# opensensor/thingino-accel

Hardware: AMD Instinct MI355X
Metric: images/sec yolov5s_int8 640x640 batch256 (higher is better)
Workload: dtype int8

## Files before the change

thingino-accel_amd/csrc/hip/conv_i8.hip:

```cpp
#include "conv_i8_common.hpp"

#ifndef I8M_ABL
#define I8M_ABL 0
#endif
template <int BPX, int BN, int STAGES, int KS = 1, int NW = 4>
__global__ __launch_bounds__(NW * 64) void conv_i8_mfma(const mhip_conv_i8_t p, const long total_pix, const int k64,
                                                         const int8_t *__restrict__ zeros, const unsigned noc,
                                                         const unsigned nblk, const int lg_inc, const unsigned kw_magic,
                                                         const fastdiv_t dhw, const fastdiv_t dow, const int bufmode,
                                                         const unsigned in_bytes) {
    ANAT_BEGIN();
    const bool POW2 = lg_inc >= 0;
    const bool masked = p.kh * p.kw <= 32;
    constexpr int SLICE = (BPX + BN) * BK;
    constexpr int STAGE = KS * SLICE;
    constexpr int NWN = BN == 128 ? 2 : 1;
    constexpr int NWM = NW / NWN;
    constexpr int WPX = BPX / NWM / 16;
    constexpr int WOC = BN / NWN / 16;
    constexpr int XROWS = BPX / NW;
    constexpr int XI = XROWS / 16;
    constexpr int LW = (BN / 16 + NW - 1) / NW;
    constexpr int L = XI + LW;
    static_assert(XI >= 1 && XROWS % 16 == 0, "every wave fetches whole 16-row pieces of the pixel tile");
// ... 240 lines not shown
    const int taps = p.kh * p.kw;
    const int nst = k128 / 128;
    auto issue = [&](int st, int buf) {
        int8_t *sb = lds + buf * STAGE;
        const int utap = (st * 128) >> lg_inc, urc = (st * 128) & ((1 << lg_inc) - 1);
        const int uky = (int)(((unsigned)utap * kw_magic) >> 16), ukx = utap - uky * p.kw;
        const int ukoff = (uky * p.in_w + ukx) * p.in_c + urc;
        const bool uvalid = utap < taps;
#pragma unroll
        for (int j = 0; j < XI; j++) {
            const bool ok = uvalid & (((tapmask[j] >> utap) & 1u) != 0u);
            blds16(xrs, ok ? xvoff[j] + ukoff : -1, 0, sb + (wv * XI + j) * 1024);
        }
#pragma unroll
        for (int j = 0; j < WI; j++) blds16(wrs, wvoff[j], st * 128, sb + BPX * 128 + (wv * WI + j) * 1024);
    };

    issue(0, 0);
    const int frow = lane & 15, fchunk = lane >> 4;
    for (int st = 0; st < nst; st++) {
        wait_vmcnt<0>();
        __builtin_amdgcn_s_barrier();
        asm volatile("" ::: "memory");
        const int8_t *xs = lds + (st & 1) * STAGE, *ws = xs + BPX * 128;
        v4i xb[2][WPX], wa[2][WOC];
#pragma unroll
        for (int h = 0; h < 2; h++) {
#pragma unroll
            for (int t = 0; t < WPX; t++) xb[h][t] = *(const v4i *)(xs + lds_off128(pxw + t * 16 + frow, h * 4 + fchunk));
#pragma unroll
            for (int q = 0; q < WOC; q++) wa[h][q] = *(const v4i *)(ws + lds_off128(ocw + q * 16 + frow, h * 4 + fchunk));
        }
        if (st + 1 < nst) issue(st + 1, (st + 1) & 1);
#pragma unroll
        for (int h = 0; h < 2; h++)
#pragma unroll
            for (int q = 0; q < WOC; q++)
#pragma unroll
                for (int t = 0; t < WPX; t++) acc[q][t] = __builtin_amdgcn_mfma_i32_16x16x64_i8(wa[h][q], xb[h][t], acc[q][t], 0, 0, 0);
    }
    __syncthreads();
    epilogue<BPX, BN, WPX, WOC, true>(p, acc, lds, slut, rowoff, oc0, pxw, ocw, hw);
}

template <int A, int B>
__device__ __forceinline__ void wait_vmcnt_at_most(int n) {
    constexpr int HI = A > B ? A : B, LO = A > B ? B : A;
    if (n >= A + B) wait_vmcnt<A + B>();
    else if (n >= HI) wait_vmcnt<HI>();
    else if (n >= LO) wait_vmcnt<LO>();
    else wait_vmcnt<0>();
}

struct conv_out_side_t {
    int8_t *out;
    size_t out_stride;
    const int8_t *w;
    const int32_t *bias;
    const uint8_t *lut, *lut2;
    int out_c, relu, out_pix_stride, out_ch_off;
    float cs;
    unsigned out_bytes;
};
template <int BPX, int BN, int STAGES, bool HAS_LUT, bool SEG = false, bool PAIR = false>
__global__ __launch_bounds__(NTHREADS) void conv_i8_persist(const mhip_conv_i8_t pin, const unsigned total_pix, const int k64,
                                                            const int8_t *__restrict__ zeros, const unsigned noc,
                                                            const unsigned npt, const unsigned ngrp, const int lg_inc,
                                                            const unsigned kw_magic, const fastdiv_t dhw, const fastdiv_t dow,
                                                            const unsigned out_bytes_first, const conv_out_side_t alt,
                                                            const unsigned noc0, const int bufmode, const unsigned in_bytes,
                                                            const int wres) {
    ANAT_BEGIN();
    const int STAGE = wres ? BPX * BK : (BPX + BN) * BK;
    constexpr int NWN = BN == 128 ? 2 : 1;
    constexpr int NWM = 4 / NWN;
    constexpr int WPX = BPX / NWM / 16;
    constexpr int WOC = BN / NWN / 16;
    constexpr int XI = BPX / 64;
    constexpr int LW = BN >= 128 ? 2 : 1;
    constexpr int L = XI + LW;
    constexpr int NST = WPX;
    extern __shared__ __attribute__((aligned(16))) int8_t dynlds[];
    uint8_t *slut = (uint8_t *)dynlds;
    int8_t *lds = dynlds + LUTB;
    lds_base_must_be_zero(dynlds);

    const int tid = threadIdx.x, lane = tid & 63;
    const int wv = __builtin_amdgcn_readfirstlane(tid >> 6);
    const unsigned id = xcd_remap(blockIdx.x, noc * ngrp);
    const unsigned grp = id / noc;
    unsigned ot = id - grp * noc;
    mhip_conv_i8_t p = pin;
    unsigned out_bytes = out_bytes_first;
    if (PAIR && ot >= noc0) {
        ot -= noc0;
        p.lut2 = alt.lut2;
        p.out = alt.out; p.out_stride = alt.out_stride; p.w = alt.w; p.bias = alt.bias; p.lut = alt.lut;
        p.out_c = alt.out_c; p.relu = alt.relu; p.out_pix_stride = alt.out_pix_stride; p.out_ch_off = alt.out_ch_off;
        p.cs = alt.cs;
        out_bytes = alt.out_bytes;
    }
    const int oc0 = (int)ot * BN;
    const unsigned t0 = (unsigned)(((unsigned long long)grp * npt) / ngrp);
    const unsigned t1 = (unsigned)(((unsigned long long)(grp + 1) * npt) / ngrp);
    if (t0 >= t1) return;
    const unsigned hw = (unsigned)(p.out_h * p.out_w);
    const int wm = wv % NWM, wn = wv / NWM;
    const int pxw = wm * (WPX * 16), ocw = wn * (WOC * 16);

    auto packed_row16 = [](int c) { return ((c >> 2) & 1) * 16 + (c >> 3) * 4 + (c & 3); };
    v4i bias[WOC];
#pragma unroll
    for (int s = 0; s < WOC; s++)
        bias[s] = p.bias ? *(const v4i *)(p.bias + (BN == 16 ? packed_row16((lane >> 4) * 4) : oc0 + ocw + s * 16 + (lane >> 4) * 4)) : (v4i){0, 0, 0, 0};
    if (HAS_LUT) {
        if (p.lut2) { if (tid < 128) ((uint32_t *)slut)[tid] = ((const uint32_t *)p.lut2)[tid]; }
        else if (tid < 64) ((uint32_t *)slut)[tid] = ((const uint32_t *)p.lut)[tid];
        __syncthreads();
    }
    const __amdgpu_buffer_rsrc_t orsrc = __builtin_amdgcn_make_buffer_rsrc(p.out, 0, (int)out_bytes, 0x00020000);

    const int schunk = (lane & 3) ^ (((lane >> 4) & 1) << 1);
    const int8_t *xwin[XI];
    unsigned tapmask[XI];
    unsigned rowf[SEG ? XI : 1], rowrem[SEG ? XI : 1];
    unsigned rowrem_up[SEG ? XI : 1];
    int xvoff[XI];
    auto setup_rows = [&](unsigned tile) {
#pragma unroll
        for (int j = 0; j < XI; j++) {
            const unsigned pix = tile * BPX + wv * (BPX / 4) + j * 16 + (lane >> 2);
            const bool valid = pix < total_pix;
            const unsigned f = valid ? fdiv(pix, dhw) : 0u;
            const unsigned rem = valid ? pix - f * hw : 0u;
            if (SEG) {
                rowf[j] = f;
                rowrem[j] = rem;
                const unsigned oy = fdiv(rem, dow), ox = rem - oy * (unsigned)p.out_w;
                rowrem_up[j] = (oy >> 1) * ((unsigned)p.out_w >> 1) + (ox >> 1);
                tapmask[j] = valid ? 1u : 0u;
                continue;
            }
            const int oy = (int)fdiv(rem, dow), ox = (int)(rem - (unsigned)oy * (unsigned)p.out_w);
            const int iy0 = oy * p.stride_h - p.pad_top, ix0 = ox * p.stride_w - p.pad_left;
            xwin[j] = p.in + (size_t)f * p.in_stride + ((long)iy0 * p.in_w + ix0) * p.in_c;
            xvoff[j] = (int)(f * (unsigned)p.in_stride) + (iy0 * p.in_w + ix0) * p.in_c + schunk * 16;
            const int kx_lo = ix0 < 0 ? -ix0 : 0, kx_hi = p.in_w - ix0 < p.kw ? p.in_w - ix0 : p.kw;
            const unsigned colbits = kx_hi > kx_lo ? ((kx_hi >= 32 ? ~0u : (1u << kx_hi) - 1u) & ~((1u << kx_lo) - 1u)) : 0u;
            unsigned m = 0;
            for (int r = 0; r < p.kh; r++) {
                const int iy = iy0 + r;
                if (iy >= 0 && iy < p.in_h) m |= colbits << (r * p.kw);
            }
            tapmask[j] = valid ? m : 0u;
        }
    };
    const int8_t *wsrc[LW];
    int wq[LW], wvoff[LW];
#pragma unroll
    for (int j = 0; j < LW; j++) {
        wq[j] = BN >= 64 ? wv * LW + j : (BN == 16 ? 0 : (wv & 1));
        const int wrow = BN == 16 ? packed_row16(lane >> 2) : oc0 + wq[j] * 16 + (lane >> 2);
        wsrc[j] = p.w + (size_t)wrow * k64 + schunk * 16;
        wvoff[j] = wrow * k64 + schunk * 16;
    }
    const __amdgpu_buffer_rsrc_t xrs = __builtin_amdgcn_make_buffer_rsrc((void *)p.in, 0, (int)in_bytes, 0x00020000);
    const __amdgpu_buffer_rsrc_t wrs = __builtin_amdgcn_make_buffer_rsrc((void *)p.w, 0, p.oc_pad * k64, 0x00020000);
    const int taps = p.kh * p.kw;
    const int nks = k64 / BK;

    auto issue = [&](int ks, int stage) {
        int8_t *sb = lds + stage * STAGE;
        const unsigned pos = (unsigned)(ks * BK + schunk * 16);
        if (SEG) {
            auto owner = [&](int c) { return (c >= p.seg_c0[1]) + (c >= p.seg_c0[2]) + (c >= p.seg_c0[3]); };
            const int sa = owner(ks * BK), sb2 = owner(ks * BK + 32);
            const bool hi = schunk >= 2;
            const int8_t *base = hi ? p.seg_in[sb2] : p.seg_in[sa];
            const unsigned fstride = (unsigned)(hi ? p.seg_stride[sb2] : p.seg_stride[sa]);
            const unsigned segc = (unsigned)(hi ? p.seg_c[sb2] : p.seg_c[sa]);
            const unsigned coff = pos - (unsigned)(hi ? p.seg_c0[sb2] : p.seg_c0[sa]);
            const bool up = ((p.seg_up >> (hi ? sb2 : sa)) & 1) != 0;
            const bool kvalid = (int)pos < p.in_c;
#pragma unroll
            for (int j = 0; j < XI; j++) {
                const bool ok = kvalid & (tapmask[j] != 0u);
                const int8_t *src = base + (size_t)rowf[j] * fstride + (size_t)(up ? rowrem_up[j] : rowrem[j]) * segc + coff;
                glds16(ok ? src : zeros, sb + (wv * (BPX / 4) + j * 16) * BK);
            }
        } else if (bufmode) {
            const int utap = (ks * BK) >> lg_inc, urc = (ks * BK) & ((1 << lg_inc) - 1);
            const int uky = (int)(((unsigned)utap * kw_magic) >> 16), ukx = utap - uky * p.kw;
            const int ukoff = (uky * p.in_w + ukx) * p.in_c + urc;
            const bool uvalid = utap < taps;
#pragma unroll
            for (int j = 0; j < XI; j++) {
                const bool ok = uvalid & (((tapmask[j] >> utap) & 1u) != 0u);
                blds16(xrs, ok ? xvoff[j] + ukoff : -1, 0, sb + (wv * (BPX / 4) + j * 16) * BK);
            }
            if (!wres)
#pragma unroll
                for (int j = 0; j < LW; j++) blds16(wrs, wvoff[j], ks * BK, sb + BPX * BK + wq[j] * 16 * BK);
            return;
        } else {
            const unsigned tap = pos >> lg_inc;
            const int rc = (int)(pos & ((1u << lg_inc) - 1u));
            const int ky = (int)((tap * kw_magic) >> 16);
            const int kx = (int)tap - ky * p.kw;
            const bool kvalid = (int)tap < taps;
            const long koff = ((long)ky * p.in_w + kx) * p.in_c + rc;
#pragma unroll
            for (int j = 0; j < XI; j++) {
                const bool ok = kvalid & ((tapmask[j] >> tap) & 1u);
                glds16(ok ? xwin[j] + koff : zeros, sb + (wv * (BPX / 4) + j * 16) * BK);
            }
        }
        if (!wres)
#pragma unroll
            for (int j = 0; j < LW; j++) glds16(wsrc[j] + ks * BK, sb + BPX * BK + wq[j] * 16 * BK);
    };

    int8_t *const wres_base = lds + STAGES * STAGE;
    if (wres)
        for (int ks = 0; ks < nks; ks++)
#pragma unroll
            for (int j = 0; j < LW; j++) glds16(wsrc[j] + ks * BK, wres_base + (ks * BN + wq[j] * 16) * BK);
    unsigned itile = t0;
    int iks = 0;
    int younger[STAGES - 1];
    setup_rows(t0);
    int nstage = 0;
#pragma unroll
    for (int s = 0; s < STAGES - 1; s++) {
        int n = 0;
        if (itile < t1) {
            issue(iks, nstage);
            n = wres ? XI : L;
            if (++iks == nks) {
                iks = 0;
                if (++itile < t1) setup_rows(itile);
            }
        }
#pragma unroll
        for (int i = 0; i < s; i++) younger[i] += n;
        younger[s] = 0;
        nstage++;
    }
    nstage = STAGES - 1;

    const int frow = lane & 15, fchunk = lane >> 4;
    const int chan = ocw + (lane >> 4) * (4 * WOC);
    const int pstride = p.out_pix_stride ? p.out_pix_stride : p.out_c;
    const int lo = p.relu ? 0 : -128;
    const uint8_t *lut128 = slut + 128;
    const bool ragged = (p.out_c % (WOC * 4)) != 0;
    int stage = 0;
    ANAT_NOW(1);
    for (unsigned tile = t0; tile < t1; tile++) {
        v4i acc[WOC][WPX];
        for (int ks = 0; ks < nks; ks++) {
            wait_vmcnt_at_most<(STAGES - 2) * L, NST>(younger[0]);
            __builtin_amdgcn_s_barrier();
            asm volatile("" ::: "memory");
            const int8_t *xs = lds + stage * STAGE, *ws = wres ? wres_base + ks * (BN * BK) : xs + BPX * BK;
            v4i xb[WPX], wa[WOC];
#pragma unroll
            for (int t = 0; t < WPX; t++) xb[t] = *(const v4i *)(xs + lds_off(pxw + t * 16 + frow, fchunk));
#pragma unroll
            for (int s = 0; s < WOC; s++) wa[s] = *(const v4i *)(ws + lds_off(ocw + s * 16 + frow, fchunk));
            int n = 0;
            if (itile < t1) {
                issue(iks, nstage);
                n = wres ? XI : L;
                if (++iks == nks) {
                    iks = 0;
                    if (++itile < t1) setup_rows(itile);
                }
            }
#pragma unroll
            for (int i = 0; i + 1 < STAGES - 1; i++) younger[i] = younger[i + 1] + n;
            younger[STAGES - 2] = 0;
            if (ks == 0) {
#pragma unroll
                for (int s = 0; s < WOC; s++)
#pragma unroll
                    for (int t = 0; t < WPX; t++) acc[s][t] = __builtin_amdgcn_mfma_i32_16x16x64_i8(wa[s], xb[t], bias[s], 0, 0, 0);
            } else {
#pragma unroll
                for (int s = 0; s < WOC; s++)
#pragma unroll
                    for (int t = 0; t < WPX; t++) acc[s][t] = __builtin_amdgcn_mfma_i32_16x16x64_i8(wa[s], xb[t], acc[s][t], 0, 0, 0);
            }
            stage = stage + 1 == STAGES ? 0 : stage + 1;
            nstage = nstage + 1 == STAGES ? 0 : nstage + 1;
        }
#ifdef ANATOMY
        if (tile + 1 == t1) ANAT_NOW(2);
#endif
#pragma unroll
        for (int t = 0; t < WPX; t++) {
            const unsigned pix = tile * BPX + pxw + t * 16 + (lane & 15);
            const unsigned f = fdiv(pix, dhw), rem = pix - f * hw;
            const unsigned off = f * (unsigned)p.out_stride + rem * (unsigned)pstride + (unsigned)(p.out_ch_off + oc0 + chan);
            const int nvalid = p.out_c - (oc0 + chan);
            const bool ok = pix < total_pix && nvalid >= WOC * 4;
            uint32_t pk[WOC];
            int a[WOC * 4];
#pragma unroll
            for (int s = 0; s < WOC; s++)
#pragma unroll
                for (int r = 0; r < 4; r++) a[s * 4 + r] = acc[s][t][r];
            if (HAS_LUT && p.lut2) requant_pack<WOC * 4, HAS_LUT, true, true, false, true>(a, p.cs, lo, lut128, pk);
            else requant_pack<WOC * 4, HAS_LUT, true, true>(a, p.cs, lo, lut128, pk);
            const int voff = ok ? (int)off : -1;
            if (WOC == 4)
                __builtin_amdgcn_raw_buffer_store_b128((v4i){(int)pk[0], (int)pk[1], (int)pk[2], (int)pk[3]}, orsrc, voff, 0, 0);
            else if (WOC == 2)
                __builtin_amdgcn_raw_buffer_store_b64((v2i){(int)pk[0], (int)pk[WOC > 1 ? 1 : 0]}, orsrc, voff, 0, 0);
            else
                __builtin_amdgcn_raw_buffer_store_b32((int)pk[0], orsrc, voff, 0, 0);
            if (ragged) {
                const bool part = pix < total_pix && nvalid > 0 && nvalid < WOC * 4;
                const int nv = part ? nvalid : 0;
                const int o4 = nv & 8, o2 = nv & 12, o1 = nv & 14;
                const uint32_t w4 = o4 ? pk[(WOC * 4 > 8) ? 2 : 0] : pk[0];
                const int i2 = o2 >> 2, i1 = o1 >> 2;
                uint32_t w2 = pk[0], w1 = pk[0];
#pragma unroll
                for (int q = 1; q < WOC; q++) {
                    w2 = i2 == q ? pk[q] : w2;
                    w1 = i1 == q ? pk[q] : w1;
                }
                w1 >>= (o1 & 2) * 8;
                if (WOC == 4)
                    __builtin_amdgcn_raw_buffer_store_b64((v2i){(int)pk[0], (int)pk[1]}, orsrc, (nv & 8) ? (int)off : -1, 0, 0);
                __builtin_amdgcn_raw_buffer_store_b32((int)w4, orsrc, (nv & 4) ? (int)off + o4 : -1, 0, 0);
                __builtin_amdgcn_raw_buffer_store_b16((short)w2, orsrc, (nv & 2) ? (int)off + o2 : -1, 0, 0);
                __builtin_amdgcn_raw_buffer_store_b8((char)w1, orsrc, (nv & 1) ? (int)off + o1 : -1, 0, 0);
            }
        }
#pragma unroll
        for (int i = 0; i < STAGES - 1; i++) younger[i] += ragged ? NST * (WOC == 4 ? 5 : 4) : NST;
    }
    ANAT_END(p);
}
ANAT_SETTER(mhip_anatomy_set_i8)
__device__ __forceinline__ bool mhip_small_c_dev(int in_c, int kw, int out_c) { return in_c <= 4 && kw <= 8 && out_c <= 64; }
template <int BN>
__global__ __launch_bounds__(NTHREADS) void conv_i8_generic(const mhip_conv_i8_t p, const long total_pix, const int k64,
                                                            const fastdiv_t dhw) {
    constexpr int STAGE = (BP + BN) * BK;
    constexpr int WPX = 2, WOC = BN / 16;
    constexpr int TILE_BYTES = BP * (BN + OPAD);
    constexpr int LDS_BYTES = (2 * STAGE > TILE_BYTES ? 2 * STAGE : TILE_BYTES) + 256;
    __shared__ __attribute__((aligned(16))) int8_t lds[LDS_BYTES];
    __shared__ long rowoff[BP];
    uint8_t *slut = (uint8_t *)lds + LDS_BYTES - 256;

    const int tid = threadIdx.x, lane = tid & 63, wv = tid >> 6;
    const long pix0 = (long)blockIdx.x * BP;
    const int oc0 = blockIdx.y * BN;
    const int hw = p.out_h * p.out_w;
    if (p.lut && tid < 64) ((uint32_t *)slut)[tid] = ((const uint32_t *)p.lut)[tid];
    fill_rowoff<BP>(p, rowoff, [=](int row) { long q = pix0 + row; return q < total_pix ? q : -1L; }, (unsigned)hw, dhw);

    const int cc = tid & 3;
    const int8_t *xbase[2];
    int iy0[2], ix0[2];
    bool rvalid[2];
#pragma unroll
    for (int j = 0; j < 2; j++) {
        long pix = pix0 + (tid >> 2) + j * 64;
        rvalid[j] = pix < total_pix;
        long f = rvalid[j] ? pix / hw : 0;
        int rem = rvalid[j] ? (int)(pix - f * hw) : 0;
        int oy = rem / p.out_w, ox = rem - oy * p.out_w;
        iy0[j] = oy * p.stride_h - p.pad_top;
        ix0[j] = ox * p.stride_w - p.pad_left;
        xbase[j] = p.in + (size_t)f * p.in_stride;
    }
    int ky = 0, rc = cc * 16;
    while (rc >= p.row_pad) { rc -= p.row_pad; ky++; }
    const int ceff = mhip_small_c_dev(p.in_c, p.kw, p.out_c) ? 4 : p.in_c;
    const int nks = k64 / BK;
    constexpr int WLOADS = (BN * 4 + NTHREADS - 1) / NTHREADS;
    v4i xreg[2], wreg[WLOADS];

    auto load_global = [&](int ks) {
#pragma unroll
        for (int j = 0; j < 2; j++) {
            v4i v = {0, 0, 0, 0};
            const int iy = iy0[j] + ky;
            if (rvalid[j] && ky < p.kh && iy >= 0 && iy < p.in_h) {
                const int8_t *rowp = xbase[j] + ((long)iy * p.in_w + ix0[j]) * p.in_c;
                int8_t b[16];
// ... 63 lines not shown
    return g * G + s * 16 + q * 4 + r;
}

extern "C" int mhip_conv_i8_is_safe(float cs) {
    return cs == cs && cs < 0.99f && cs > -0.99f;
}

extern "C" int mhip_conv_i8_lut2_ok(float cs) {
    if (!mhip_conv_i8_is_safe(cs)) return 0;
    const float a = cs < 0 ? -cs : cs;
    if (!(a >= 1e-6f)) return 0;
    const float quirk = 0.49999997f;
    const double a0 = (double)quirk / (double)a;
    for (int d = -3; d <= 3; d++) {
        const double c = (double)(long long)(a0 + 0.5) + d;
        if (c < 1.0 || c > 2147483647.0) continue;
        volatile float prod = (float)(int)c * a;
        if (prod == quirk) return 0;
    }
    return 1;
}

extern "C" int mhip_conv_i8_small_c(int in_c, int kw, int out_c) { return in_c <= 4 && kw <= 8 && out_c <= 64; }

extern "C" void mhip_conv_i8_pack_geom(int in_c, int kw, int out_c, int *row_pad, int *oc_pad, int *c_eff) {
    const int small = mhip_conv_i8_small_c(in_c, kw, out_c);
    if (row_pad) *row_pad = small ? 32 : (kw * in_c + 15) & ~15;
    if (oc_pad) *oc_pad = (out_c + 31) & ~31;
    if (c_eff) *c_eff = small ? 4 : in_c;
}

static tune_t g_tune;
static int env_int(const char *name, int dflt) {
    const char *e = getenv(name);
    return e ? atoi(e) : dflt;
}
const tune_t &conv_i8_tune_state() {
    if (!g_tune.init) {
        g_tune.persist = env_int("MARS_HIP_PERSIST", 1);
        g_tune.persist_stages = env_int("MARS_HIP_PSTAGES", 2);
        g_tune.persist_maxk = env_int("MARS_HIP_PERSIST_MAXK", 8);
        g_tune.persist_slots = env_int("MARS_HIP_PSLOTS", 0);
        g_tune.stages = env_int("MARS_HIP_STAGES", 0);
        g_tune.bpx = env_int("MARS_HIP_BPX", 0);
        g_tune.variant = env_int("MARS_HIP_VARIANT", 0);
        g_tune.bufmode = env_int("MARS_HIP_BUFMODE", 1);
        g_tune.wres = env_int("MARS_HIP_WRES", 3);
        g_tune.rgb_direct = env_int("MARS_HIP_RGB_DIRECT", 1);
        g_tune.small_batch = env_int("MARS_HIP_SMALL_BATCH", 1);
        g_tune.rows = env_int("MARS_HIP_ROWS", 1);
        g_tune.few_wgs = env_int("MARS_HIP_FEW_WGS", 256);
        g_tune.patch_ring = env_int("MARS_HIP_PATCH_RING", 0);
        g_tune.patch_lds_kb = env_int("MARS_HIP_PATCH_LDS_KB", 80);
        g_tune.init = 1;
    }
    return g_tune;
}
static inline const tune_t &tune() { return conv_i8_tune_state(); }
static int tune_access(const char *key, int value, int *get) {
    (void)conv_i8_tune_state();
    struct { const char *k; int *v; } tab[] = {{"persist", &g_tune.persist}, {"persist_stages", &g_tune.persist_stages},
                                               {"persist_maxk", &g_tune.persist_maxk}, {"persist_slots", &g_tune.persist_slots}, {"wres", &g_tune.wres}, {"rgb_direct", &g_tune.rgb_direct}, {"small_batch", &g_tune.small_batch},
                                               {"rows", &g_tune.rows}, {"few_wgs", &g_tune.few_wgs}, {"patch_ring", &g_tune.patch_ring}, {"patch_lds_kb", &g_tune.patch_lds_kb}, {"stages", &g_tune.stages}, {"bpx", &g_tune.bpx}, {"variant", &g_tune.variant}, {"bufmode", &g_tune.bufmode}};
    for (auto &e : tab)
        if (key && !strcmp(key, e.k)) {
            if (get) *get = *e.v;
            else *e.v = value;
            return 0;
        }
    return -1;
}
extern "C" int mhip_conv_i8_tune(const char *key, int value) { return tune_access(key, value, nullptr); }
extern "C" int mhip_conv_i8_tune_get(const char *key, int *value) { return value ? tune_access(key, 0, value) : -1; }

static int buf_mode(const mhip_conv_i8_t *p, int k64) {
    if (!tune().bufmode) return 0;
    return p->in_c >= 64 && (p->in_c & (p->in_c - 1)) == 0 && p->kh * p->kw <= 32 && (long)p->kh * p->kw * (p->kw - 1) < 65536 &&
           in_extent_bytes(p) <= 0x7fffffffL && (long)p->oc_pad * k64 <= 0x7fffffffL;
}

template <int BPX, int BN, int STAGES, int KS = 1, int NW = 4>
static int launch_mfma(const mhip_conv_i8_t *p, long total_pix, int k64) {
    const unsigned npt = (unsigned)((total_pix + BPX - 1) / BPX), noc = (unsigned)(p->oc_pad / BN);
    const unsigned nblk = npt * noc;
    const int nks = k64 / BK, nst = nks / KS, used = nst < STAGES ? nst : STAGES;
    if (KS > 1 && (nks % KS) != 0) return -1;
    size_t ring = (size_t)used * KS * (BPX + BN) * BK, tile = (size_t)BPX * (BN + OPAD);
    const size_t lds = BPX * 8 + LUTB + (ring > tile ? ring : tile);
    if (lds > 64 * 1024) {
        static bool attr = false;
        if (!attr && hipFuncSetAttribute((const void *)conv_i8_mfma<BPX, BN, STAGES, KS, NW>, hipFuncAttributeMaxDynamicSharedMemorySize,
                                         (int)(BPX * 8 + LUTB + (size_t)STAGES * KS * (BPX + BN) * BK)) != hipSuccess)
            return mhip_check(hipErrorUnknown, "conv_i8_mfma LDS attribute");
        attr = true;
    }
    int lg = -1;
    if ((p->in_c & (p->in_c - 1)) == 0 && (long)p->kh * p->kw * (p->kw - 1) < 65536) {
        lg = 0;
        while ((1 << lg) < p->in_c) lg++;
    }
    const unsigned magic = ((65536u + (unsigned)p->kw - 1u) / (unsigned)p->kw);
    hipLaunchKernelGGL((conv_i8_mfma<BPX, BN, STAGES, KS, NW>), dim3(nblk), dim3(NW * 64), lds, mhip_stream_native(), *p, total_pix,
                       k64, (const int8_t *)mhip_zero_page(), noc, nblk, lg, magic,
                       make_fastdiv((unsigned)(p->out_h * p->out_w)), make_fastdiv((unsigned)p->out_w),
                       lg >= 0 ? buf_mode(p, k64) : 0, (unsigned)in_extent_bytes(p));
    return mhip_check(hipGetLastError(), "conv_i8_mfma launch");
}


template <int BPX, int BN>
static size_t wres_lds(int k64) { return LUTB + 2 * (size_t)BPX * BK + (size_t)(k64 / BK) * BN * BK; }

template <int BPX, int BN, int STAGES, bool HAS_LUT, bool SEG = false, bool PAIR = false>
static int launch_persist_t(const mhip_conv_i8_t *p, long total_pix, int k64, int lg, unsigned magic,
                            const mhip_conv_i8_t *second = nullptr, int wres = 0) {
    if (BN == 16 && (p->out_c > 16 || p->oc_pad != 32 || (PAIR && (second->out_c > 16 || second->oc_pad != 32)))) return -1;
    const unsigned noc0 = BN == 16 ? 1u : (unsigned)(p->oc_pad / BN);
    const unsigned npt = (unsigned)((total_pix + BPX - 1) / BPX), noc = noc0 + (PAIR ? (BN == 16 ? 1u : (unsigned)(second->oc_pad / BN)) : 0u);
    conv_out_side_t alt;
    memset(&alt, 0, sizeof(alt));
    if (PAIR) {
        alt.out = second->out; alt.out_stride = second->out_stride; alt.w = second->w; alt.bias = second->bias;
        alt.lut = second->lut; alt.lut2 = second->lut2; alt.out_c = second->out_c; alt.relu = second->relu; alt.out_pix_stride = second->out_pix_stride;
        alt.out_ch_off = second->out_ch_off; alt.cs = second->cs;
    }
    if (PAIR) alt.out_bytes = (unsigned)persist_out_bytes(second);
    if (wres && STAGES != 2) return -1;
    const size_t lds = wres ? wres_lds<BPX, BN>(k64) : LUTB + (size_t)STAGES * (BPX + BN) * BK;
    if (wres) {
        static bool attr = false;
        if (!attr && hipFuncSetAttribute((const void *)conv_i8_persist<BPX, BN, STAGES, HAS_LUT, SEG, PAIR>,
                                         hipFuncAttributeMaxDynamicSharedMemorySize, 80 * 1024) != hipSuccess)
            return mhip_check(hipErrorUnknown, "conv_i8_persist LDS attribute");
        attr = true;
        int occ = 0, dev = 0;
        hipDeviceProp_t prop;
        if (hipOccupancyMaxActiveBlocksPerMultiprocessor(&occ, conv_i8_persist<BPX, BN, STAGES, HAS_LUT, SEG, PAIR>, NTHREADS, lds) != hipSuccess ||
            hipGetDevice(&dev) != hipSuccess || hipGetDeviceProperties(&prop, dev) != hipSuccess)
            return mhip_check(hipErrorUnknown, "conv_i8_persist occupancy query");
        unsigned g = (unsigned)((occ > 0 ? occ : 1) * prop.multiProcessorCount) / noc;
        if (tune().persist_slots > 0) g = (unsigned)tune().persist_slots / noc;
        if (g < 1) g = 1;
        if (g > npt) g = npt;
        hipLaunchKernelGGL((conv_i8_persist<BPX, BN, STAGES, HAS_LUT, SEG, PAIR>), dim3(noc * g), dim3(NTHREADS), lds,
                           mhip_stream_native(), *p, (unsigned)total_pix, k64, (const int8_t *)mhip_zero_page(), noc, npt, g, lg,
                           magic, make_fastdiv((unsigned)(p->out_h * p->out_w)), make_fastdiv((unsigned)p->out_w),
                           (unsigned)persist_out_bytes(p), alt, noc0, SEG ? 0 : buf_mode(p, k64), (unsigned)in_extent_bytes(p), 1);
        return mhip_check(hipGetLastError(), "conv_i8_persist (resident weights) launch");
    }
    static int slots = 0;
    if (!slots) {
        int occ = 0, dev = 0;
        hipDeviceProp_t prop;
        if (hipOccupancyMaxActiveBlocksPerMultiprocessor(&occ, conv_i8_persist<BPX, BN, STAGES, HAS_LUT, SEG, PAIR>, NTHREADS, lds) != hipSuccess ||
            hipGetDevice(&dev) != hipSuccess || hipGetDeviceProperties(&prop, dev) != hipSuccess)
            return mhip_check(hipErrorUnknown, "conv_i8_persist occupancy query");
        slots = (occ > 0 ? occ : 1) * prop.multiProcessorCount;
    }
    unsigned ngrp = (unsigned)(tune().persist_slots > 0 ? tune().persist_slots : 4 * slots) / noc;
    if (ngrp < 1) ngrp = 1;
    if (ngrp > npt) ngrp = npt;
    hipLaunchKernelGGL((conv_i8_persist<BPX, BN, STAGES, HAS_LUT, SEG, PAIR>), dim3(noc * ngrp), dim3(NTHREADS), lds,
                       mhip_stream_native(), *p, (unsigned)total_pix, k64, (const int8_t *)mhip_zero_page(), noc, npt, ngrp, lg,
                       magic, make_fastdiv((unsigned)(p->out_h * p->out_w)), make_fastdiv((unsigned)p->out_w),
                       (unsigned)persist_out_bytes(p), alt, noc0, SEG ? 0 : buf_mode(p, k64), (unsigned)in_extent_bytes(p), 0);
    return mhip_check(hipGetLastError(), "conv_i8_persist launch");
}

#define NVARIANTS 20
struct variant_t {
    int persist, bpx, stages, patch, ks2, w8, wres, r128, rows;
};
static int variant_code(const variant_t &v) {
    if (v.rows) return 20;
    if (v.r128) return 17 + v.r128;
    if (v.wres) return v.bpx == 256 ? 15 : 14;
    if (v.w8) return 13;
    if (v.ks2) return 12;
    if (v.patch) return v.patch == 16 ? 10 : (v.patch == 8 ? 9 : 11);
    return 1 + (v.persist ? 1 : 0) + (v.bpx == 256 ? 2 : 0) + (v.stages == 3 ? 4 : 0);
}
static variant_t variant_of(int code) {
    if (code == 20) return variant_t{0, 0, 0, 0, 0, 0, 0, 0, 1};
    if (code == 18 || code == 19) return variant_t{0, 0, 0, 0, 0, 0, 0, code - 17, 0};
    if (code == 14 || code == 15) return variant_t{1, code == 15 ? 256 : 128, 2, 0, 0, 0, 1, 0, 0};
    if (code == 13) return variant_t{0, 256, 3, 0, 0, 1, 0, 0, 0};
    if (code == 12) return variant_t{0, 128, 2, 0, 1, 0, 0, 0, 0};
    if (code >= 9 && code <= 11) return variant_t{0, 0, 0, code == 10 ? 16 : (code == 9 ? 8 : 4), 0, 0, 0, 0, 0};
    if (code > 8 || code == 6 || code == 8) return variant_t{-1, 0, 0, 0, 0, 0, 0, 0, 0};
    const int c = code - 1;
    return variant_t{c & 1, (c & 2) ? 256 : 128, (c & 4) ? 3 : 2, 0, 0, 0, 0, 0, 0};
}

static bool r128_ok(const mhip_conv_i8_t *p) {
    const int C = p->in_c;
    return C >= 128 && (C & (C - 1)) == 0 && p->oc_pad % 128 == 0 && p->kh * p->kw <= 32 && (long)p->kh * p->kw * (p->kw - 1) < 65536 &&
           p->row_pad == p->kw * C && p->nseg <= 1 && in_extent_bytes(p) <= 0x7fffffffL && (long)p->oc_pad * p->kh * p->row_pad <= 0x7fffffffL;
}
template <int BPX, int BN, int NW>
static int launch_r128_t(const mhip_conv_i8_t *p, long total_pix) {
    const int k128 = p->kh * p->row_pad;
    const unsigned npt = (unsigned)((total_pix + BPX - 1) / BPX), noc = (unsigned)(p->oc_pad / BN);
    size_t ring = 2 * (size_t)(BPX + BN) * 128, tile = (size_t)BPX * (BN + OPAD);
    const size_t lds = BPX * 8 + LUTB + (ring > tile ? ring : tile);
    static bool attr = false;
    if (!attr && hipFuncSetAttribute((const void *)conv_i8_r128<BPX, BN, NW>, hipFuncAttributeMaxDynamicSharedMemorySize, (int)lds) != hipSuccess)
        return mhip_check(hipErrorUnknown, "conv_i8_r128 LDS attribute");
    attr = true;
    int lg = 0;
    while ((1 << lg) < p->in_c) lg++;
    const unsigned magic = ((65536u + (unsigned)p->kw - 1u) / (unsigned)p->kw);
    hipLaunchKernelGGL((conv_i8_r128<BPX, BN, NW>), dim3(npt * noc), dim3(NW * 64), lds, mhip_stream_native(), *p, total_pix, k128, noc,
                       npt * noc, lg, magic, make_fastdiv((unsigned)(p->out_h * p->out_w)), make_fastdiv((unsigned)p->out_w),
                       (unsigned)in_extent_bytes(p));
    return mhip_check(hipGetLastError(), "conv_i8_r128 launch");
}
static int launch_r128(const mhip_conv_i8_t *p, long total_pix, int form) {
    if (!r128_ok(p)) return -1;
// ... 129 lines not shown
        if (b16) return launch_variant_t<256, 16>(p, total_pix, k64, v);
        return launch_variant_t<256, 32>(p, total_pix, k64, v);
    }
    if (bn == 128) return launch_variant_t<128, 128>(p, total_pix, k64, v);
    if (bn == 64) return launch_variant_t<128, 64>(p, total_pix, k64, v);
    if (b16) return launch_variant_t<128, 16>(p, total_pix, k64, v);
    return launch_variant_t<128, 32>(p, total_pix, k64, v);
}

template <int BPX, int BN>
static int launch_pair_t(const mhip_conv_i8_t *a, const mhip_conv_i8_t *b, long total_pix, int k64, int lg, unsigned magic,
                         int wres) {
    if (a->nseg > 1) return -2;
    return launch_persist_t<BPX, BN, 2, true, false, true>(a, total_pix, k64, lg, magic, b, wres);
}
extern "C" int mhip_conv_i8_pair(const mhip_conv_i8_t *a, const mhip_conv_i8_t *b) {
    if (!a || !b || !tune().persist || tune().variant) return -2;
    if (a->in != b->in || a->in_stride != b->in_stride || a->frames != b->frames || a->in_h != b->in_h || a->in_w != b->in_w ||
        a->in_c != b->in_c || a->out_h != b->out_h || a->out_w != b->out_w || a->kh != b->kh || a->kw != b->kw ||
        a->stride_h != b->stride_h || a->stride_w != b->stride_w || a->pad_top != b->pad_top || a->pad_left != b->pad_left ||
        a->row_pad != b->row_pad || a->nseg != b->nseg || a->seg_up != b->seg_up || !a->lut || !b->lut || a->add || b->add ||
        a->out_nchw || b->out_nchw)
        return -2;
    for (int i = 0; i < a->nseg; i++)
        if (a->seg_in[i] != b->seg_in[i] || a->seg_c[i] != b->seg_c[i] || a->seg_stride[i] != b->seg_stride[i]) return -2;
    if ((a->in_c % 16) != 0 || mhip_conv_i8_small_c(a->in_c, a->kw, a->out_c) || mhip_conv_i8_small_c(b->in_c, b->kw, b->out_c))
        return -2;
    if (a->nseg > 1 && (!seg_valid(a) || !seg_valid(b))) return -2;
    if (!persist_eligible(a) || !persist_eligible(b)) return -2;
    const int bn = a->oc_pad % 128 == 0 ? 128 : (a->oc_pad % 64 == 0 ? 64 : 32);
    const int bnb = b->oc_pad % 128 == 0 ? 128 : (b->oc_pad % 64 == 0 ? 64 : 32);
    if (bn != bnb || !mhip_zero_page()) return -2;
    const long total_pix = (long)a->frames * a->out_h * a->out_w;
    const int k64 = (a->kh * a->row_pad + BK - 1) / BK * BK, nks = k64 / BK;
    if (total_pix <= 0 || total_pix > 0x7fffffffL) return -2;
    int lg = 0;
    while ((1 << lg) < a->in_c) lg++;
    const unsigned magic = ((65536u + (unsigned)a->kw - 1u) / (unsigned)a->kw);
    const variant_t dv = default_variant(a, nks);
    const int bpx = dv.bpx ? dv.bpx : 128, wres = dv.persist && dv.wres && (tune().wres & 2);
    const bool b16 = bn16_ok(a) && bn16_ok(b);
    if (bpx == 256) {
        if (bn == 128) return launch_pair_t<256, 128>(a, b, total_pix, k64, lg, magic, wres);
        if (bn == 64) return launch_pair_t<256, 64>(a, b, total_pix, k64, lg, magic, wres);
        if (b16) return launch_pair_t<256, 16>(a, b, total_pix, k64, lg, magic, wres);
        return launch_pair_t<256, 32>(a, b, total_pix, k64, lg, magic, wres);
    }
    if (bn == 128) return launch_pair_t<128, 128>(a, b, total_pix, k64, lg, magic, wres);
    if (bn == 64) return launch_pair_t<128, 64>(a, b, total_pix, k64, lg, magic, wres);
    if (b16) return launch_pair_t<128, 16>(a, b, total_pix, k64, lg, magic, wres);
    return launch_pair_t<128, 32>(a, b, total_pix, k64, lg, magic, wres);
}

extern "C" int mhip_conv_i8_seg_ok(const mhip_conv_i8_t *p) {
    return p && (p->in_c % 16) == 0 && !mhip_conv_i8_small_c(p->in_c, p->kw, p->out_c) && seg_valid(p) && persist_eligible(p);
}

extern "C" int mhip_conv_i8_variants(const mhip_conv_i8_t *p, int *codes, int max) {
    if (!p || (p->in_c % 16) != 0 || mhip_conv_i8_small_c(p->in_c, p->kw, p->out_c)) return 0;
    const int k64 = (p->kh * p->row_pad + BK - 1) / BK * BK, nks = k64 / BK;
    int n = 0;
    if (p->pre_w) {
        const int first = conv_i8_pre_tile_rows(p);
        for (int th : {first, 16, 8, 4})
            if (th && n < max && conv_i8_patch_ok(p, th, nullptr)) {
                const int code = th == 16 ? 10 : (th == 8 ? 9 : 11);
                bool seen = false;
                for (int i = 0; i < n; i++) seen |= codes[i] == code;
                if (!seen) codes[n++] = code;
            }
        return n;
    }
    if (p->post_w) {
        for (int th : {16, 8, 4})
            if (n < max && conv_i8_patch_ok(p, th, nullptr)) codes[n++] = th == 16 ? 10 : (th == 8 ? 9 : 11);
        return n;
    }
    if (p->split_w) {
        for (int th : {16, 8, 4})
            if (n < max && conv_i8_patch_ok(p, th, nullptr)) codes[n++] = th == 16 ? 10 : (th == 8 ? 9 : 11);
        return n;
    }
    if (p->nseg > 1) {
        const int bn = p->oc_pad % 128 == 0 ? 128 : (p->oc_pad % 64 == 0 ? 64 : 32);
        const variant_t dv = default_variant(p, nks);
        const int dflt = dv.persist && dv.wres ? (dv.bpx == 256 ? 15 : 14) : (dv.bpx == 256 ? 4 : 2);
        if (n < max) codes[n++] = dflt;
        if (n < max && dflt != 2) codes[n++] = 2;
        if (n < max && dflt != 4) codes[n++] = 4;
        if (n < max && dflt != 14 && LUTB + 2 * (size_t)128 * BK + (size_t)nks * bn * BK <= 80 * 1024) codes[n++] = 14;
        if (n < max && dflt != 15 && LUTB + 2 * (size_t)256 * BK + (size_t)nks * bn * BK <= 80 * 1024) codes[n++] = 15;
        return n;
    }
    const int dflt = variant_code(default_variant(p, nks));
    if (n < max) codes[n++] = dflt;
    for (int code = 1; code <= NVARIANTS; code++) {
        const variant_t v = variant_of(code);
        if (code == dflt) continue;
        if (v.patch && !conv_i8_patch_ok(p, v.patch, nullptr)) continue;
        if (v.persist && !persist_eligible(p)) continue;
        if (v.ks2 && ((nks & 1) || nks < 4 || p->oc_pad % 64 != 0)) continue;
        if (v.w8 && (p->oc_pad % 128 != 0 || nks < 3)) continue;
        if (v.persist < 0) continue;
        if (v.r128 && !r128_ok(p)) continue;
        if (v.rows && !conv_i8_rows_ok(p)) continue;
        if (v.wres) {
// ... 123 lines not shown
```

thingino-accel_amd/csrc/hip/conv_i8_common.hpp:

```cpp
#pragma once
#include <hip/hip_runtime.h>
#include <stdint.h>
#include <stdlib.h>
#include <string.h>
#include <type_traits>

#include "../mhip.h"

extern "C" hipStream_t mhip_stream_native(void);
extern "C" int mhip_check(hipError_t e, const char *what);
extern "C" const void *mhip_zero_page(void);

typedef int v4i __attribute__((ext_vector_type(4)));
typedef int v2i __attribute__((ext_vector_type(2)));

#ifdef ANATOMY
struct anat_rec_t {
    unsigned key, wg, hwid, xcc;
    unsigned long long t[4];
};
static __device__ anat_rec_t *g_anat_buf;
static __device__ unsigned g_anat_cap;
#define ANAT_SETTER(NAME)                                                                                                    \
    extern "C" int NAME(void *buf, unsigned cap) {                                                                          \
// ... 64 lines not shown
    asm("v_med3_i32 %0, %1, %2, %3" : "=v"(m) : "v"(r), "v"(lo), "v"(hi));
    return m;
}
template <int NV>
__device__ __forceinline__ void wait_lds_values(int (&v)[NV]) {
    static_assert(NV == 4 || NV == 8 || NV == 16, "values per lane");
    if constexpr (NV == 16)
        asm volatile("s_waitcnt lgkmcnt(0)"
                     : "+v"(v[0]), "+v"(v[1]), "+v"(v[2]), "+v"(v[3]), "+v"(v[4]), "+v"(v[5]), "+v"(v[6]), "+v"(v[7]), "+v"(v[8]), "+v"(v[9]),
                       "+v"(v[10]), "+v"(v[11]), "+v"(v[12]), "+v"(v[13]), "+v"(v[14]), "+v"(v[15]));
    else if constexpr (NV == 8)
        asm volatile("s_waitcnt lgkmcnt(0)" : "+v"(v[0]), "+v"(v[1]), "+v"(v[2]), "+v"(v[3]), "+v"(v[4]), "+v"(v[5]), "+v"(v[6]), "+v"(v[7]));
    else
        asm volatile("s_waitcnt lgkmcnt(0)" : "+v"(v[0]), "+v"(v[1]), "+v"(v[2]), "+v"(v[3]));
}

__device__ __forceinline__ uint32_t pack4(int q0, int q1, int q2, int q3) {
    const uint32_t a = __builtin_amdgcn_perm((uint32_t)q1, (uint32_t)q0, 0x0c0c0400u);
    const uint32_t b = __builtin_amdgcn_perm((uint32_t)q3, (uint32_t)q2, 0x0c0c0400u);
    return (b << 16) | a;
}
__device__ __forceinline__ void lut4_at0(int q0, int q1, int q2, int q3, int &v0, int &v1, int &v2, int &v3) {
    asm volatile("ds_read_i8 %0, %4 offset:128\n\tds_read_i8 %1, %5 offset:128\n\t"
                 "ds_read_i8 %2, %6 offset:128\n\tds_read_i8 %3, %7 offset:128"
                 : "=&v"(v0), "=&v"(v1), "=&v"(v2), "=&v"(v3)
                 : "v"(q0), "v"(q1), "v"(q2), "v"(q3)
                 : "memory");
}
__device__ __forceinline__ void lds_base_must_be_zero(const void *dynamic_lds) {
    __builtin_amdgcn_s_setprio(3);
    unsigned a = (unsigned)(size_t)(const __attribute__((address_space(3))) void *)dynamic_lds;
    asm volatile("" : "+s"(a));
    if (a != 0u) __builtin_trap();
}
struct add_args_t {
    float s_conv, s_other, inv;
};
__device__ __forceinline__ int add_one(int v, uint32_t xword, int k, const add_args_t &g, int lo8, int hi8) {
    const int x = __builtin_amdgcn_sbfe((int)xword, 8 * k, 8);
    const float y = (float)v * g.s_conv + (float)x * g.s_other;
    const float t = y * g.inv;
    const int r = (int)(t + 0.5f);
    int m;
    asm("v_med3_i32 %0, %1, %2, %3" : "=v"(m) : "v"(r), "v"(lo8), "v"(hi8));
    return m;
}
__device__ __forceinline__ void lut4_fast(int q0, int q1, int q2, int q3, int &v0, int &v1, int &v2, int &v3) {
    asm volatile("ds_read_i8 %0, %4 offset:256\n\tds_read_i8 %1, %5 offset:256\n\t"
                 "ds_read_i8 %2, %6 offset:256\n\tds_read_i8 %3, %7 offset:256"
                 : "=&v"(v0), "=&v"(v1), "=&v"(v2), "=&v"(v3)
                 : "v"(q0), "v"(q1), "v"(q2), "v"(q3)
                 : "memory");
}
template <int NV>
__device__ __forceinline__ void requant_pack_pre(const int (&a)[NV], float cs, uint32_t (&pk)[NV / 4]) {
    const float cs2 = cs * 2.0f;
    const int klo = -256, khi = 255;
    int q[NV], v[NV];
#pragma unroll
    for (int i = 0; i < NV; i++) {
        const int k = (int)((float)a[i] * cs2);
        asm("v_med3_i32 %0, %1, %2, %3" : "=v"(q[i]) : "v"(k), "v"(klo), "v"(khi));
    }
#pragma unroll
    for (int g = 0; g < NV / 4; g++)
        asm volatile("ds_read_i8 %0, %4 offset:768\n\tds_read_i8 %1, %5 offset:768\n\t"
                     "ds_read_i8 %2, %6 offset:768\n\tds_read_i8 %3, %7 offset:768"
                     : "=&v"(v[4 * g]), "=&v"(v[4 * g + 1]), "=&v"(v[4 * g + 2]), "=&v"(v[4 * g + 3])
                     : "v"(q[4 * g]), "v"(q[4 * g + 1]), "v"(q[4 * g + 2]), "v"(q[4 * g + 3])
                     : "memory");
    wait_lds_values<NV>(v);
#pragma unroll
    for (int g = 0; g < NV / 4; g++) pk[g] = pack4(v[4 * g], v[4 * g + 1], v[4 * g + 2], v[4 * g + 3]);
}
__device__ __forceinline__ void requant_pack_two(const int (&a)[16], float cs0, float cs1, uint32_t (&pk)[4]) {
    const float c0 = cs0 * 2.0f, c1 = cs1 * 2.0f;
    const int klo = -256, khi = 255;
    int q[16], v[16];
#pragma unroll
    for (int i = 0; i < 16; i++) {
        const int k = (int)((float)a[i] * (i < 8 ? c0 : c1));
        asm("v_med3_i32 %0, %1, %2, %3" : "=v"(q[i]) : "v"(k), "v"(klo), "v"(khi));
    }
#pragma unroll
    for (int g = 0; g < 2; g++)
        asm volatile("ds_read_i8 %0, %4 offset:768\n\tds_read_i8 %1, %5 offset:768\n\t"
                     "ds_read_i8 %2, %6 offset:768\n\tds_read_i8 %3, %7 offset:768"
                     : "=&v"(v[4 * g]), "=&v"(v[4 * g + 1]), "=&v"(v[4 * g + 2]), "=&v"(v[4 * g + 3])
                     : "v"(q[4 * g]), "v"(q[4 * g + 1]), "v"(q[4 * g + 2]), "v"(q[4 * g + 3])
                     : "memory");
#pragma unroll
    for (int g = 2; g < 4; g++)
        asm volatile("ds_read_i8 %0, %4 offset:1280\n\tds_read_i8 %1, %5 offset:1280\n\t"
                     "ds_read_i8 %2, %6 offset:1280\n\tds_read_i8 %3, %7 offset:1280"
                     : "=&v"(v[4 * g]), "=&v"(v[4 * g + 1]), "=&v"(v[4 * g + 2]), "=&v"(v[4 * g + 3])
                     : "v"(q[4 * g]), "v"(q[4 * g + 1]), "v"(q[4 * g + 2]), "v"(q[4 * g + 3])
                     : "memory");
    wait_lds_values<16>(v);
#pragma unroll
    for (int g = 0; g < 4; g++) pk[g] = pack4(v[4 * g], v[4 * g + 1], v[4 * g + 2], v[4 * g + 3]);
}
__device__ __forceinline__ void requant_pack_chain(const int (&a)[8], float cs, uint32_t (&pk)[2]) {
    const float cs2 = cs * 2.0f;
    const int klo = -256, khi = 255;
    int q[8], v[8];
#pragma unroll
    for (int i = 0; i < 8; i++) {
        const int k = (int)((float)a[i] * cs2);
        asm("v_med3_i32 %0, %1, %2, %3" : "=v"(q[i]) : "v"(k), "v"(klo), "v"(khi));
    }
#pragma unroll
    for (int g = 0; g < 2; g++)
        asm volatile("ds_read_i8 %0, %4 offset:1792\n\tds_read_i8 %1, %5 offset:1792\n\t"
                     "ds_read_i8 %2, %6 offset:1792\n\tds_read_i8 %3, %7 offset:1792"
                     : "=&v"(v[4 * g]), "=&v"(v[4 * g + 1]), "=&v"(v[4 * g + 2]), "=&v"(v[4 * g + 3])
                     : "v"(q[4 * g]), "v"(q[4 * g + 1]), "v"(q[4 * g + 2]), "v"(q[4 * g + 3])
                     : "memory");
    wait_lds_values<8>(v);
#pragma unroll
    for (int g = 0; g < 2; g++) pk[g] = pack4(v[4 * g], v[4 * g + 1], v[4 * g + 2], v[4 * g + 3]);
}
template <int NV, bool HAS_LUT, bool SAFE, bool LUT0, bool ADD = false, bool FAST = false>
__device__ __forceinline__ void requant_pack(const int (&a)[NV], float cs, int lo, const uint8_t *lut128, uint32_t (&pk)[NV / 4],
                                             const uint32_t *xw = nullptr, const add_args_t *ga = nullptr) {
    int q[NV];
    const int hi = 127;
    if (FAST && HAS_LUT && LUT0 && SAFE) {
        const float cs2 = cs * 2.0f;
        const int klo = -256, khi = 255;
        int v[NV];
#pragma unroll
        for (int i = 0; i < NV; i++) {
            const int k = (int)((float)a[i] * cs2);
            asm("v_med3_i32 %0, %1, %2, %3" : "=v"(q[i]) : "v"(k), "v"(klo), "v"(khi));
        }
#pragma unroll
        for (int g = 0; g < NV / 4; g++)
            lut4_fast(q[4 * g], q[4 * g + 1], q[4 * g + 2], q[4 * g + 3], v[4 * g], v[4 * g + 1], v[4 * g + 2], v[4 * g + 3]);
        wait_lds_values<NV>(v);
        if (ADD) {
            const int lo8 = -128;
#pragma unroll
            for (int i = 0; i < NV; i++) v[i] = add_one(v[i], xw[i >> 2], i & 3, *ga, lo8, hi);
        }
#pragma unroll
        for (int g = 0; g < NV / 4; g++) pk[g] = pack4(v[4 * g], v[4 * g + 1], v[4 * g + 2], v[4 * g + 3]);
        return;
    }
#pragma unroll
    for (int i = 0; i < NV; i++) q[i] = SAFE ? requant_safe(a[i], cs, lo, hi) : requant<false>(a[i], cs, lo);
    if (HAS_LUT && LUT0) {
        int v[NV];
#pragma unroll
        for (int g = 0; g < NV / 4; g++)
            lut4_at0(q[4 * g], q[4 * g + 1], q[4 * g + 2], q[4 * g + 3], v[4 * g], v[4 * g + 1], v[4 * g + 2], v[4 * g + 3]);
        wait_lds_values<NV>(v);
        if (ADD) {
            const int lo8 = -128;
#pragma unroll
            for (int i = 0; i < NV; i++) v[i] = add_one(v[i], xw[i >> 2], i & 3, *ga, lo8, hi);
        }
#pragma unroll
        for (int g = 0; g < NV / 4; g++) pk[g] = pack4(v[4 * g], v[4 * g + 1], v[4 * g + 2], v[4 * g + 3]);
    } else {
        if (HAS_LUT) {
#pragma unroll
            for (int i = 0; i < NV; i++) q[i] = (int8_t)lut128[q[i]];
        }
        if (ADD) {
            const int lo8 = -128;
#pragma unroll
            for (int i = 0; i < NV; i++) q[i] = add_one(q[i], xw[i >> 2], i & 3, *ga, lo8, hi);
        }
#pragma unroll
// ... 138 lines not shown
        for (int id = tid; id < BPX * BN; id += (int)blockDim.x) {
            const int c = id / BPX, row = id - c * BPX;
            const long off = rowoff[row];
            if (off < 0 || c >= ncols) continue;
            p.out[off + (size_t)(oc0 + c) * hw] = tile[row * ROW + c];
        }
    }
}

template <int BPX, int BN, int WPX, int WOC, bool LUT0 = false>
__device__ __forceinline__ void epilogue(const mhip_conv_i8_t &p, v4i (&acc)[WOC][WPX], int8_t *tile, const uint8_t *slut,
                                         const long *rowoff, int oc0, int pxw, int ocw, int hw) {
    const bool direct = !p.out_nchw && ((p.out_c | p.out_pix_stride | p.out_ch_off) & 15) == 0;
#define EPI(L, S, D) epilogue_t<BPX, BN, WPX, WOC, L, S, D, LUT0>(p, acc, tile, slut, rowoff, oc0, pxw, ocw, hw)
    if (direct) {
        if (p.lut) { if (p.safe) EPI(true, true, true); else EPI(true, false, true); }
        else { if (p.safe) EPI(false, true, true); else EPI(false, false, true); }
    } else {
        if (p.lut) { if (p.safe) EPI(true, true, false); else EPI(true, false, false); }
        else { if (p.safe) EPI(false, true, false); else EPI(false, false, false); }
    }
#undef EPI
}

template <int WPX, int WOC>
__device__ __forceinline__ void init_acc(const mhip_conv_i8_t &p, v4i (&acc)[WOC][WPX], int ocbase) {
    const int lane = threadIdx.x & 63;
#pragma unroll
    for (int s = 0; s < WOC; s++) {
        const v4i b = p.bias ? *(const v4i *)(p.bias + ocbase + s * 16 + (lane >> 4) * 4) : (v4i){0, 0, 0, 0};
#pragma unroll
        for (int t = 0; t < WPX; t++) acc[s][t] = b;
    }
}


struct tune_t {
    int init;
    int persist;
    int persist_stages;
    int persist_maxk;
    int persist_slots;
    int stages;
    int bpx;
    int variant;
    int bufmode;
    int small_batch;
    int rgb_direct;
    int wres;
    int few_wgs;
    int rows;
    int patch_ring;
    int patch_lds_kb;
};
const tune_t &conv_i8_tune_state();

extern "C" int mhip_conv_i8_small_c(int in_c, int kw, int out_c);

static inline long in_extent_bytes(const mhip_conv_i8_t *p) {
    return (long)(p->frames - 1) * (long)p->in_stride + (long)p->in_h * p->in_w * p->in_c;
}
static inline long persist_out_bytes(const mhip_conv_i8_t *p) {
    const long pstride = p->out_pix_stride ? p->out_pix_stride : p->out_c;
    return (long)(p->frames - 1) * (long)p->out_stride + (long)p->out_h * p->out_w * pstride;
}
static inline bool conv_i8_direct_rows(const mhip_conv_i8_t *p) {
    return !p->out_nchw && ((p->out_c | p->out_pix_stride | p->out_ch_off) & 15) == 0;
}

bool conv_i8_patch_ok(const mhip_conv_i8_t *p, int th, int *ring);
int conv_i8_launch_patch(const mhip_conv_i8_t *p, int k64, int th);
int conv_i8_pre_tile_rows(const mhip_conv_i8_t *p);
int conv_i8_post_tile_rows(const mhip_conv_i8_t *p);
int conv_i8_split_tile_rows(const mhip_conv_i8_t *p);
bool conv_i8_rows_ok(const mhip_conv_i8_t *p);
int conv_i8_launch_rows(const mhip_conv_i8_t *p);
int conv_i8_try_rgb(const mhip_conv_i8_t *p, int k64);
int conv_i8_try_smallc(const mhip_conv_i8_t *p, int k64);
```

thingino-accel_amd/csrc/host/mars_internal.h:

```cpp
#ifndef MARS_INTERNAL_H
#define MARS_INTERNAL_H

#include <stddef.h>
#include <stdint.h>

#include "../mhip.h"
#include "mars_hip.h"
#include "mars_runtime.h"

enum {
    OP_CONV_I8 = 0,
    OP_CONV_F32,
    OP_RELU_BYTES,
    OP_LUT_I8,
    OP_BINARY_I8,
    OP_SIGMOID_F32,
    OP_BINARY_F32,
    OP_RELU_F32,
    OP_BN,
    OP_MAXPOOL,
    OP_CONCAT_SLICE,
    OP_UPSAMPLE,
    OP_UPSAMPLE_Q, OP_MAXPOOL_Q,
    OP_CONCAT_Q,
    OP_CONV_F32_VHEAD,
    OP_FAIL,
};

#define NO_OFF ((size_t)-1)
#define MARS_MAX_IO 4
#define MARS_MAX_MODEL_TUNE 16

typedef struct {
    size_t bytes;
    size_t extent;
    size_t stride;
    uint8_t *dev;
    int is_weight;
    int needed;
    int io_in, io_out;
    uint8_t *host;
    uint8_t *dense_dev;
    int pix_c, pix_stride;
    int rec_c, rec_hw;
    int nhwc_c, nhwc_hw;
    size_t zero_from;
    int partial;
    int nhwc_pitch;
    int tail_read;
} mtensor_t;

typedef struct {
    int kind, layer, err;
    int t_in[4], n_in, t_out;
    int in_h, in_w, in_c, out_h, out_w, out_c, kh, kw, sh, sw, pt, pl;
    int nchw, relu, is_mul, is_f32, leaky, safe;
    size_t in_byte_off, out_byte_off;
    int k_limit;
    int vc_n, vc_t[3], vc_run, vc_shift;
    int rows_only;
    int out_nchw;
    int silu_f32;
    int f32_exact;
    int variant;
    int add_t; float add_s_conv, add_s_other, add_inv;
    int nseg, seg_t[4], seg_c[4], seg_up;
    int chain_n, chain_out[3];
    int pair_next;
    int row_pad, oc_pad, c_pad;
    int ch_off, scale_h, scale_w, bn_n;
    int out_pix_stride, out_ch_off;
    int store_c;
    float cs, f0, f1, f2;
    size_t n;
    size_t w_off, b_off, lut_off, s_off;
    int pre;
    size_t pre_w_off, pre_b_off, pre_lut2_off;
    float pre_cs;
    int post_next;
    size_t post_w_off;
    int split_next;
    size_t split_w_off;
    int split_chain;
    size_t chain_w_off;
    size_t w2_off;
    int w2_rows;
    int w2_planes;
    size_t w3_off;
    int w3_stem;
    int in_rec, out_rec;
    size_t lut2_off;
    size_t w_blob_off[2];
    double macs, bytes;
    int prof_kind;
    float last_ms;
    void *ev0, *ev1;
    int prof_rec;
    void *ev_start;
} mars_op_t;

typedef struct {
    int fusion;
    unsigned no_fuse_lut : 1, no_nhwc_internal : 1, no_vconcat_q : 1, no_pair_f32 : 1, no_rec : 1, no_zero_tail : 1, no_vconcat_f32 : 1,
        no_rowpad : 1, no_post : 1, no_split : 1, no_chain : 1;
    size_t rec_limit;
    size_t vconcat_limit;
    size_t bottleneck_limit;
} plan_switches_t;

typedef struct mars_model_ext {
    mars_model_t pub;
    plan_switches_t sw;
    int batch, profiling, deferred;
    int plan_err;
    int no_vconcat;
    int no_download;
    int no_bottleneck;
    int no_post;
    int no_split;
    int no_chain;
    int rec_frames;
    int rec_skipped;
    size_t rec_max_frames;
    mtensor_t *mt;
    mars_op_t *ops;
    int n_ops, cap_ops;
    uint8_t *arena_host;
    size_t arena_size, arena_cap;
    uint8_t *arena_dev;
    size_t blob_mirror_bytes;
    uint8_t *act_dev;
    size_t act_bytes;
    uint8_t *scratch_dev;
    size_t scratch_per_frame;
    int scratch_t, scratch_cpad, scratch_f0, scratch_n;
    void *det_dev;
    int *det_counts_dev;
    float *det_lut_dev;
    int det_cap;
    float det_lut_scale[4];
    int det_lut_n;
    int det_lut_mono[4];
    float *heads_lut_dev;
    float heads_lut_scale[4];
    int heads_lut_n;
    float *dfl_lut_dev;
    float dfl_lut_scale[4][2];
    int dfl_lut_n;
    void *ev_graph_done, *ev_tail_done;
    int tail_pending;
    int frame0, run_frames;
    void *ev_fork, *ev_join[3];
    void *ev_chunk[2][8];
    void *graph_exec;
    unsigned graph_gen;
    int ran_plain;
    void *pipe;
    struct { char key[28]; int value, saved; } tune[MARS_MAX_MODEL_TUNE];
    int n_tune, tune_depth;
    int plan_f32_mode;
    unsigned char *layer_noop;
    void *roi_dev;
    int roi_cap_slots, roi_cap_frames;
    int roi_slots;
    struct mars_model_ext *roi_from;
    void *cls_dev;
    size_t cls_bytes, cls_sums_off, cls_top_off;
    int cls_frames, cls_c, cls_top_k;
    void *ev_label_done;
    int label_pending;
    void *label_dev;
    int label_cap, label_frames;
    void *match_dev;
// ... 4 lines not shown
    void *track_dev;
    int track_cap, track_frames;
    void *seg_dev;
    size_t seg_bytes, seg_rec_off, seg_word_off;
    int seg_frames, seg_max, seg_ph, seg_pw;
    void *ev_seg[2];
    void *pose_dev;
    size_t pose_bytes, pose_rec_off, pose_kpt_off;
    int pose_frames, pose_max, pose_k;
    float pose_lut_scale[4];
    int pose_lut_n;
    void *ev_pose[2];
    void *obb_dev;
    size_t obb_bytes, obb_cnt_off, obb_out_off;
    int obb_frames;
    float obb_lut_scale[4];
    int obb_lut_n;
    void *ev_obb[2];
    int det_mapped;
    void *tile_roi_dev;
    int tile_roi_cap;
    void *tile_dev;
    int tile_cap, tile_cams;
    void *ev_tile[2];
    struct mars_model_ext *live_next;
} mars_model_ext_t;


#define MARS_INTERNAL __attribute__((visibility("hidden")))
#define ALIGN_UP(x, a) (((x) + (size_t)(a) - 1) & ~((size_t)(a) - 1))
#define NO_TENSOR 0xFFFFFFFFu
#define MAX_DIM_PRODUCT ((size_t)1 << 40)
#define ARENA_MAX ((size_t)1 << 40)
#define MAX_CHANNELS 65536
MARS_INTERNAL int mars_verbose(void);
#define VLOG(...) do { if (mars_verbose()) fprintf(stderr, "Mars: " __VA_ARGS__); } while (0)
MARS_INTERNAL void drop_graph(mars_model_ext_t *m);
MARS_INTERNAL mars_model_ext_t *mars_live_models(void);
MARS_INTERNAL void plan_switches_read(plan_switches_t *sw, int at_load);
MARS_INTERNAL mars_error_t build_plan(mars_model_ext_t *m);
MARS_INTERNAL mars_error_t upload_params(mars_model_ext_t *m);
MARS_INTERNAL mars_error_t alloc_batch(mars_model_ext_t *m, int n);
MARS_INTERNAL size_t elem_size(uint32_t dtype);
MARS_INTERNAL size_t shape_numel(const mars_tensor_t *d);
MARS_INTERNAL size_t reference_buffer_size(const mars_model_ext_t *m);
MARS_INTERNAL size_t arena_reserve(mars_model_ext_t *m, size_t bytes);
MARS_INTERNAL void blob_read(const mars_model_ext_t *m, size_t off, size_t n, void *dst);
MARS_INTERNAL int op_reads(const mars_op_t *o, int t);
MARS_INTERNAL int op_writes(const mars_op_t *o, int t);
MARS_INTERNAL size_t planned_stride(const mtensor_t *t);
MARS_INTERNAL void conv_i8_geometry(const mars_op_t *op, int frames, mhip_conv_i8_t *p);
MARS_INTERNAL int conv_i8_pre_fits(const mars_op_t *op, int frames, size_t in_stride, size_t out_stride);
MARS_INTERNAL int conv_i8_post_fits(const mars_model_ext_t *m, const mars_op_t *a, const mars_op_t *b, int frames);
MARS_INTERNAL int conv_i8_split_fits(const mars_model_ext_t *m, const mars_op_t *a, const mars_op_t *b, const mars_op_t *c, int frames);
MARS_INTERNAL int conv_i8_chain_fits(const mars_model_ext_t *m, const mars_op_t *a, const mars_op_t *b, const mars_op_t *c, const mars_op_t *d, int side, int frames);
MARS_INTERNAL void plan_layer(mars_model_ext_t *m, int li);
MARS_INTERNAL void fold_silu(mars_model_ext_t *m, int f32);
MARS_INTERNAL void fuse_lut(mars_model_ext_t *m);
MARS_INTERNAL void nhwc_internal(mars_model_ext_t *m);
MARS_INTERNAL void fold_add(mars_model_ext_t *m, int f32);
MARS_INTERNAL void virtual_concat(mars_model_ext_t *m);
MARS_INTERNAL void elide_concat(mars_model_ext_t *m);
MARS_INTERNAL void trim_concat(mars_model_ext_t *m);
MARS_INTERNAL void fuse_pool_chains(mars_model_ext_t *m);
MARS_INTERNAL void pair_convs(mars_model_ext_t *m);
MARS_INTERNAL void fuse_bottleneck(mars_model_ext_t *m);
MARS_INTERNAL void fuse_post(mars_model_ext_t *m);
MARS_INTERNAL void fuse_split(mars_model_ext_t *m);
MARS_INTERNAL void fuse_split_chain(mars_model_ext_t *m);
MARS_INTERNAL void pad_output_rows(mars_model_ext_t *m);
MARS_INTERNAL void virtual_concat_q(mars_model_ext_t *m);
MARS_INTERNAL void f32_policy(mars_model_ext_t *m);
MARS_INTERNAL void zero_tail_f32(mars_model_ext_t *m);
MARS_INTERNAL void pair_convs_f32(mars_model_ext_t *m);
MARS_INTERNAL void rec_pairs(mars_model_ext_t *m);
MARS_INTERNAL void virtual_concat_f32(mars_model_ext_t *m);
MARS_INTERNAL void plan_check(mars_model_ext_t *m);
MARS_INTERNAL void conv_i8_params(const mars_model_ext_t *m, const mars_op_t *op, mhip_conv_i8_t *p);
MARS_INTERNAL int mars_preproc_prepare(int w, int h, int tw, int th);
MARS_INTERNAL int mars_preproc_prepare_nv12(int w, int h, int tw, int th, int frames);

MARS_INTERNAL void mars_roi_release(mars_model_ext_t *m);

MARS_INTERNAL void mars_cls_release(mars_model_ext_t *m);

MARS_INTERNAL void mars_match_release(mars_model_ext_t *m);

MARS_INTERNAL void mars_track_release(mars_model_ext_t *m);

MARS_INTERNAL void mars_seg_release(mars_model_ext_t *m);

MARS_INTERNAL void mars_pose_release(mars_model_ext_t *m);

MARS_INTERNAL void mars_obb_release(mars_model_ext_t *m);

MARS_INTERNAL void mars_tile_release(mars_model_ext_t *m);

MARS_INTERNAL int mars_tensor_chw(const mars_tensor_t *d, int *c, int *h, int *w);
MARS_INTERNAL int mars_locate_i8(const mars_model_ext_t *m, int T, int ch, int hh, int ww, int any_writer, int *buf, int *off, int *pix_step, int *ch_step);
MARS_INTERNAL mars_error_t mars_own_det_buffers(mars_model_ext_t *m);
MARS_INTERNAL mars_error_t mars_tail_on_aux(mars_model_ext_t *m, int (*launch)(struct mars_model_ext *, const void *, void *, int *), const void *cfg);

mars_error_t mars_detect_prepare(mars_model_ext_t *m, const int *output_indices, int n_outputs);
int mars_detect_launch(mars_model_ext_t *m, const int *output_indices, int n_outputs, float nms_thresh, void *dets_dev,
                       int *counts_dev);

// ... 36 lines not shown
```

thingino-accel_amd/csrc/host/mars_model.c:

```c
#include <math.h>
#include <stdio.h>
#include <stdlib.h>
#include <string.h>
#include <sys/types.h>
#include <time.h>

#include "mars_internal.h"
#include "nna.h"


int mars_verbose(void) {
    static int v = -1;
    if (v < 0) v = getenv("MARS_VERBOSE") ? 1 : 0;
    return v;
}

void plan_switches_read(plan_switches_t *sw, int at_load) {
    const char *e;
    if (at_load) sw->fusion = (e = getenv("MARS_HIP_FUSION")) ? atoi(e) : 1;
    sw->no_fuse_lut = getenv("MARS_HIP_NO_FUSE_LUT") != NULL;
    sw->no_nhwc_internal = getenv("MARS_HIP_NO_NHWC_INTERNAL") != NULL;
    sw->no_vconcat_q = getenv("MARS_HIP_NO_VCONCAT_Q") != NULL;
    sw->no_pair_f32 = getenv("MARS_HIP_NO_PAIR_F32") != NULL;
    sw->no_rec = getenv("MARS_HIP_NO_REC") != NULL;
    sw->no_zero_tail = getenv("MARS_HIP_NO_ZERO_TAIL") != NULL;
    sw->no_vconcat_f32 = getenv("MARS_HIP_NO_VCONCAT_F32") != NULL;
    sw->no_rowpad = getenv("MARS_HIP_NO_ROWPAD") != NULL;
    sw->no_post = getenv("MARS_HIP_NO_POST") != NULL;
    sw->no_split = getenv("MARS_HIP_NO_SPLIT") != NULL;
    sw->no_chain = getenv("MARS_HIP_NO_CHAIN") != NULL;
    sw->rec_limit = (e = getenv("MARS_HIP_REC_LIMIT")) ? (size_t)strtoull(e, NULL, 0) : (size_t)0xfffffff0u;
    sw->vconcat_limit = (e = getenv("MARS_HIP_VCONCAT_LIMIT")) ? (size_t)strtoull(e, NULL, 0) : (size_t)0x7fffffffu;
    sw->bottleneck_limit = (e = getenv("MARS_HIP_BOTTLENECK_LIMIT")) ? (size_t)strtoull(e, NULL, 0) : 0;
}

void drop_graph(mars_model_ext_t *m) {
    if (m->graph_exec) {
        mhip_sync();
        mhip_graph_destroy(m->graph_exec);
    }
    m->graph_exec = NULL;
    m->ran_plain = 0;
}

static const char *const k_err[] = {
    "OK", "Invalid magic number", "Version mismatch", "Memory allocation failed",
    "Invalid file format", "NNA initialization failed", "Layer execution failed",
    "Invalid tensor", "Invalid layer",
};

const char *mars_get_error_string(mars_error_t err) {
    int i = -(int)err;
    if (i >= 0 && i < (int)(sizeof(k_err) / sizeof(k_err[0]))) return k_err[i];
    return "Unknown error";
}

static void free_device_state(mars_model_ext_t *m) {
    drop_graph(m);
    if (m->act_dev) mhip_free(m->act_dev);
    if (m->scratch_dev) mhip_free(m->scratch_dev);
    m->act_dev = m->scratch_dev = NULL;
    for (uint32_t i = 0; m->mt && i < m->pub.header.num_tensors; i++) {
        if (m->mt[i].host) mhip_host_free(m->mt[i].host);
        m->mt[i].host = NULL;
        if (m->mt[i].dense_dev) mhip_free(m->mt[i].dense_dev);
        m->mt[i].dense_dev = NULL;
        if (!m->mt[i].is_weight) m->mt[i].dev = NULL;
    }
    if (m->det_dev) mhip_free(m->det_dev);
    if (m->det_counts_dev) mhip_free(m->det_counts_dev);
    m->det_dev = NULL;
    m->det_counts_dev = NULL;
    m->det_cap = 0;
    m->tail_pending = 0;
    mars_roi_release(m);
    mars_cls_release(m);
    mars_track_release(m);
    mars_seg_release(m);
    mars_pose_release(m);
    mars_obb_release(m);
    mars_tile_release(m);
}

// ... 33 lines not shown
    for (int k = 0; k < 3; k++)
        if (m->ev_join[k]) mhip_event_destroy(m->ev_join[k]);
    for (int k = 0; k < 2; k++)
        for (int c = 0; c < 8; c++)
            if (m->ev_chunk[k][c]) mhip_event_destroy(m->ev_chunk[k][c]);
    free(m->arena_host);
    free(m->layer_noop);
    free(m->mt);
    free(m->pub.weights);
    free(m->pub.layers);
    free(m->pub.tensors);
    free(m);
}

mars_error_t build_plan(mars_model_ext_t *m) {
    const uint32_t nt = m->pub.header.num_tensors, nl = m->pub.header.num_layers;
    plan_switches_read(&m->sw, 0);
    free_ops(m);
    m->arena_size = 0;
    if (m->arena_host) memset(m->arena_host, 0, m->arena_cap);
    m->scratch_per_frame = 0;
    m->plan_err = MARS_OK;
    m->plan_f32_mode = mhip_conv_f32_mode(-1);
    m->blob_mirror_bytes = m->pub.weights_size;
    for (uint32_t i = 0; i < nt; i++) {
        m->mt[i].extent = m->mt[i].bytes;
        m->mt[i].pix_c = m->mt[i].pix_stride = 0;
        m->mt[i].needed = (m->mt[i].io_in || m->mt[i].io_out) ? 1 : 0;
    }
    for (uint32_t i = 0; i < nl && m->plan_err == MARS_OK; i++) {
        const int n0 = m->n_ops;
        plan_layer(m, (int)i);
        m->layer_noop[i] = m->n_ops == n0;
    }
    if (m->plan_err != MARS_OK) return (mars_error_t)m->plan_err;
    if (m->sw.fusion >= 1) {
        fold_silu(m, 0);
        fuse_lut(m);
        fold_silu(m, 1);
        nhwc_internal(m);
        fold_add(m, 0);
        fold_add(m, 1);
        if (!m->no_vconcat) virtual_concat(m);
        elide_concat(m);
        trim_concat(m);
        fuse_pool_chains(m);
        pair_convs(m);
        if (m->sw.fusion >= 2 && !m->no_bottleneck) fuse_bottleneck(m);
        fuse_post(m);
        fuse_split(m);
        fuse_split_chain(m);
        pad_output_rows(m);
        virtual_concat_q(m);
    } else {
        nhwc_internal(m);
    }
    f32_policy(m);
    zero_tail_f32(m);
    if (m->sw.fusion >= 1) pair_convs_f32(m);
    rec_pairs(m);
    virtual_concat_f32(m);
    if (m->plan_err == MARS_OK) plan_check(m);
    return (mars_error_t)m->plan_err;
}

mars_error_t upload_params(mars_model_ext_t *m) {
    size_t mirror_off = arena_reserve(m, m->blob_mirror_bytes + 64);
    if (mirror_off == NO_OFF) return MARS_ERR_ALLOC_FAILED;
    if (!m->deferred) blob_read(m, 0, m->blob_mirror_bytes, m->arena_host + mirror_off);
    if (m->arena_dev) mhip_free(m->arena_dev);
    m->arena_dev = (uint8_t *)mhip_malloc(m->arena_size);
    if (!m->arena_dev) return MARS_ERR_ALLOC_FAILED;
    if (mhip_h2d_async(m->arena_dev, m->arena_host, m->arena_size) || mhip_sync()) return MARS_ERR_NNA_INIT_FAILED;
    for (uint32_t i = 0; i < m->pub.header.num_tensors; i++) {
        if (!m->mt[i].is_weight) continue;
        m->mt[i].dev = m->arena_dev + mirror_off + (size_t)m->pub.tensors[i].desc.data_offset;
        m->mt[i].stride = 0;
        m->pub.tensors[i].paddr = m->mt[i].dev;
    }
    m->pub.ddr_paddr = m->arena_dev;
    m->pub.ddr_size = m->arena_size;
    return MARS_OK;
}

mars_error_t alloc_batch(mars_model_ext_t *m, int n) {
    const uint32_t nt = m->pub.header.num_tensors;
    if (m->pipe) mars_hip_pipe_close(&m->pub);
    if (mhip_sync()) return MARS_ERR_LAYER_FAILED;
    plan_switches_read(&m->sw, 0);
    const size_t vlim = m->sw.vconcat_limit, blim = m->sw.bottleneck_limit;
    const int rec_replan = (size_t)n > m->rec_max_frames || (m->rec_skipped && n < m->rec_frames);
    m->rec_frames = n;
    if (m->no_vconcat || m->no_bottleneck || m->no_post || m->no_split || m->no_chain || rec_replan) {
        m->no_vconcat = m->no_bottleneck = m->no_post = m->no_split = m->no_chain = 0;
        mars_error_t e = build_plan(m);
        if (e == MARS_OK) e = upload_params(m);
        if (e != MARS_OK) return e;
    }
    if (!m->no_vconcat)
        for (int i = 0; i < m->n_ops; i++) {
            const mars_op_t *op = &m->ops[i];
            if (op->kind != OP_CONV_I8 || op->nseg < 2 || op->t_out < 0) continue;
            if (planned_stride(&m->mt[op->t_out]) * (size_t)n > vlim) {
                m->no_vconcat = 1;
                mars_error_t e = build_plan(m);
                if (e == MARS_OK) e = upload_params(m);
                if (e != MARS_OK) return e;
                break;
            }
        }
    if (m->sw.fusion >= 2 && !m->no_bottleneck)
        for (int i = 0; i < m->n_ops; i++) {
            const mars_op_t *op = &m->ops[i];
            if (op->kind != OP_CONV_I8 || !op->pre || op->t_out < 0) continue;
            const size_t in_stride = op->t_in[0] >= 0 ? planned_stride(&m->mt[op->t_in[0]]) : 0;
            if (!conv_i8_pre_fits(op, n, in_stride, planned_stride(&m->mt[op->t_out])) || (blim && (size_t)n > blim)) {
                m->no_bottleneck = 1;
                mars_error_t e = build_plan(m);
                if (e == MARS_OK) e = upload_params(m);
                if (e != MARS_OK) return e;
                break;
            }
        }
    if (!m->no_post)
        for (int i = 0; i + 1 < m->n_ops; i++) {
            const mars_op_t *op = &m->ops[i];
            if (op->kind != OP_CONV_I8 || !op->post_next) continue;
            if (!conv_i8_post_fits(m, op, op + 1, n)) {
                m->no_post = 1;
                mars_error_t e = build_plan(m);
                if (e == MARS_OK) e = upload_params(m);
                if (e != MARS_OK) return e;
                break;
            }
        }
    if (!m->no_chain)
        for (int i = 0; i + 3 < m->n_ops; i++) {
            const mars_op_t *op = &m->ops[i];
            if (op->kind != OP_CONV_I8 || !op->split_next || !op->split_chain) continue;
            if (!conv_i8_chain_fits(m, op, op + 1, op + 2, op + 3, op->split_chain, n)) {
                m->no_chain = 1;
                mars_error_t e = build_plan(m);
                if (e == MARS_OK) e = upload_params(m);
                if (e != MARS_OK) return e;
                break;
            }
        }
    if (!m->no_split)
        for (int i = 0; i + 2 < m->n_ops; i++) {
            const mars_op_t *op = &m->ops[i];
            if (op->kind != OP_CONV_I8 || !op->split_next) continue;
            if (!conv_i8_split_fits(m, op, op + 1, op + 2, n)) {
                m->no_split = 1;
                mars_error_t e = build_plan(m);
                if (e == MARS_OK) e = upload_params(m);
                if (e != MARS_OK) return e;
                break;
            }
        }
    free_device_state(m);
    size_t per_frame = 0;
    for (uint32_t i = 0; i < nt; i++) {
        mtensor_t *t = &m->mt[i];
        if (t->is_weight || !t->needed) continue;
        t->stride = planned_stride(t);
        per_frame += t->stride;
    }
    m->act_bytes = per_frame * (size_t)n;
    m->act_dev = (uint8_t *)mhip_malloc(m->act_bytes + 512);
    if (!m->act_dev) return MARS_ERR_ALLOC_FAILED;
    if (mhip_memset_async(m->act_dev, 0, m->act_bytes + 256)) return MARS_ERR_ALLOC_FAILED;
    size_t off = 256;
    for (uint32_t i = 0; i < nt; i++) {
        mtensor_t *t = &m->mt[i];
        mars_runtime_tensor_t *rt = &m->pub.tensors[i];
        if (t->is_weight) continue;
        rt->vaddr = NULL; rt->paddr = NULL; rt->alloc_size = 0;
        if (!t->needed) continue;
        t->dev = m->act_dev + off;
        off += t->stride * (size_t)n;
        rt->paddr = t->dev;
        rt->alloc_size = t->stride * (size_t)n;
        if (t->io_in || t->io_out) {
            const size_t hb = t->bytes * (size_t)n, ref = reference_buffer_size(m);
            size_t cap = hb > ref ? hb : ref;
            if (ref > ((size_t)8 << 20)) cap = hb;
            t->host = (uint8_t *)mhip_host_alloc(cap ? cap : 64);
            if (!t->host) return MARS_ERR_ALLOC_FAILED;
            memset(t->host, 0, cap);
            rt->vaddr = t->host;
            rt->alloc_size = n == 1 && cap >= ref ? ref : hb;
        }
        if (t->pix_stride) {
            t->dense_dev = (uint8_t *)mhip_malloc(t->bytes * (size_t)n);
            if (!t->dense_dev) return MARS_ERR_ALLOC_FAILED;
        }
    }
    if (m->scratch_per_frame) {
        m->scratch_dev = (uint8_t *)mhip_malloc(ALIGN_UP(m->scratch_per_frame, 256) * (size_t)n + 256);
        if (!m->scratch_dev) return MARS_ERR_ALLOC_FAILED;
    }
    m->batch = n;
    m->frame0 = 0;
    m->run_frames = n;
    return mhip_sync() ? MARS_ERR_ALLOC_FAILED : MARS_OK;
}
// ... 56 lines not shown
        uint32_t id = h.output_tensor_ids[i];
        if (id < h.num_tensors && !m->mt[id].is_weight) m->mt[id].io_out = (int)i + 1;
    }

    mars_error_t err = build_plan(m);
    if (err != MARS_OK) { mars_free(&m->pub); return err; }
    VLOG("%u layers -> %d launches, parameter arena %zu bytes\n", h.num_layers, m->n_ops, m->arena_size);
    *out_m = m;
    return MARS_OK;
}

mars_error_t mars_hip_load_memory_ex(const void *data, size_t size, unsigned flags, mars_model_t **out_model) {
    if (!out_model) return MARS_ERR_INVALID_FILE;
    mars_model_ext_t *m = NULL;
    mars_error_t err = load_host(data, size, flags, &m);
    if (err != MARS_OK) return err;
    if (!nna_is_ready() || !mhip_ready()) {
        fprintf(stderr, "Mars: no initialised MI355X device (call nna_init first); refusing to load\n");
        mars_free(&m->pub);
        return MARS_ERR_NNA_INIT_FAILED;
    }
    err = upload_params(m);
    if (err == MARS_OK) err = alloc_batch(m, 1);
    if (err != MARS_OK) { mars_free(&m->pub); return err; }
    m->live_next = g_live_models;
    g_live_models = m;
    *out_model = &m->pub;
    return MARS_OK;
}

static int describe_op_full(const mars_op_t *o, char *line, size_t cap, int k) {
#define ADD(...) k += snprintf(line + k, cap - (size_t)k, __VA_ARGS__)
    ADD(" | err %d in %dx%dx%d out %dx%dx%d k %dx%d s %dx%d p %d,%d", o->err, o->in_h, o->in_w, o->in_c, o->out_h, o->out_w, o->out_c, o->kh, o->kw, o->sh, o->sw, o->pt, o->pl);
    ADD(" nchw %d out_nchw %d relu %d is_mul %d is_f32 %d leaky %d safe %d silu %d f32_exact %d variant %d", o->nchw, o->out_nchw, o->relu, o->is_mul, o->is_f32, o->leaky,
        o->safe, o->silu_f32, o->f32_exact, o->variant);
    ADD(" row_pad %d oc_pad %d c_pad %d store_c %d ch_off %d out_ch_off %d out_pix_stride %d in_byte_off %zu out_byte_off %zu scale %dx%d bn_n %d n %zu", o->row_pad,
        o->oc_pad, o->c_pad, o->store_c, o->ch_off, o->out_ch_off, o->out_pix_stride, o->in_byte_off, o->out_byte_off, o->scale_h, o->scale_w, o->bn_n, o->n);
    ADD(" k_limit %d rows_only %d pair_next %d in_rec %d out_rec %d vc %d,%d,%d:", o->k_limit, o->rows_only, o->pair_next, o->in_rec, o->out_rec, o->vc_n, o->vc_run, o->vc_shift);
    for (int q = 0; q < o->vc_n && q < 3; q++) ADD(" %d", o->vc_t[q]);
    ADD(" add %d %a %a %a seg %d up %d:", o->add_t, (double)o->add_s_conv, (double)o->add_s_other, (double)o->add_inv, o->nseg, o->seg_up);
    for (int q = 0; q < o->nseg && q < 4; q++) ADD(" %d/%d", o->seg_t[q], o->seg_c[q]);
    ADD(" chain %d:", o->chain_n);
    for (int q = 0; q < o->chain_n && q < 3; q++) ADD(" %d", o->chain_out[q]);
    ADD(" cs %a f %a %a %a", (double)o->cs, (double)o->f0, (double)o->f1, (double)o->f2);
    ADD(" w_off %zd b_off %zd lut_off %zd lut2_off %zd s_off %zd w2_off %zd rows %d planes %d w3_off %zd stem %d blob %zd %zd", (ssize_t)o->w_off, (ssize_t)o->b_off,
        (ssize_t)o->lut_off, (ssize_t)o->lut2_off, (ssize_t)o->s_off, (ssize_t)o->w2_off, o->w2_rows, o->w2_planes, (ssize_t)o->w3_off, o->w3_stem, (ssize_t)o->w_blob_off[0],
        (ssize_t)o->w_blob_off[1]);
    ADD(" post_next %d", o->post_next);
    if (o->post_next) ADD(" %zd", (ssize_t)o->post_w_off);
    ADD(" split_next %d", o->split_next);
    if (o->split_next) ADD(" %zd", (ssize_t)o->split_w_off);
    ADD(" split_chain %d", o->split_chain);
    if (o->split_chain) ADD(" %zd", (ssize_t)o->chain_w_off);
    ADD(" pre %d", o->pre);
    if (o->pre) ADD(" %zd %zd %zd %a", (ssize_t)o->pre_w_off, (ssize_t)o->pre_b_off, (ssize_t)o->pre_lut2_off, (double)o->pre_cs);
    ADD(" macs %a bytes %a prof_kind %d", o->macs, o->bytes, o->prof_kind);
#undef ADD
    return k;
}

size_t mars_hip_describe_plan(const void *data, size_t size, unsigned flags, char *out, size_t cap) {
    static const char *const kinds[] = {"conv_i8", "conv_f32", "relu_bytes", "lut_i8", "binary_i8", "sigmoid_f32", "binary_f32", "relu_f32", "bn",
                                        "maxpool", "concat_slice", "upsample", "upsample_q", "maxpool_q", "concat_q", "conv_f32_vhead", "fail"};
    mars_model_ext_t *m = NULL;
    const int full = (flags & MARS_HIP_DESCRIBE_FULL) != 0;
    if (load_host(data, size, flags & ~MARS_HIP_DESCRIBE_FULL, &m) != MARS_OK) return 0;
    size_t n = 0;
    char line[4096];
#define EMIT() do { const size_t l = strlen(line); if (out && n < cap) memcpy(out + n, line, n + l <= cap ? l : cap - n); n += l; } while (0)
    for (int i = 0; i < m->n_ops; i++) {
        const mars_op_t *o = &m->ops[i];
        int k = snprintf(line, sizeof line, "op %d layer %d %s in", i, o->layer, o->kind >= 0 && o->kind <= OP_FAIL ? kinds[o->kind] : "?");
        for (int q = 0; q < o->n_in && q < 4; q++) k += snprintf(line + k, sizeof line - (size_t)k, " %d", o->t_in[q]);
        k += snprintf(line + k, sizeof line - (size_t)k, " out %d", o->t_out);
#define FLAG(cond, ...) if (cond) k += snprintf(line + k, sizeof line - (size_t)k, __VA_ARGS__)
        FLAG(o->kind == OP_CONV_I8 || o->kind == OP_CONV_F32 || o->kind == OP_CONV_F32_VHEAD, " k%dx%d s%d c%d->%d", o->kh, o->kw, o->sw, o->in_c, o->out_c);
        FLAG(o->nchw, " relayout"); FLAG(o->out_nchw, " planar_store"); FLAG(o->lut_off != NO_OFF, " lut"); FLAG(o->add_t, " add=%d", o->add_t - 1);
        FLAG(o->nseg, " seg=%d", o->nseg); FLAG(o->pair_next, " pair_next"); FLAG(o->post_next, " post_next"); FLAG(o->split_next, " split_next"); FLAG(o->pre, " pre"); FLAG(o->silu_f32, " silu");
        FLAG(o->k_limit, " k_limit=%d", o->k_limit); FLAG(o->in_rec, " in_rec=%d", o->in_rec); FLAG(o->out_rec, " out_rec");
        FLAG(o->vc_shift, " view=-%d", o->vc_shift); FLAG(o->vc_n, " vcat=%dx%d", o->vc_n, o->vc_run);
        FLAG(o->rows_only, " rows_only=%d", o->rows_only); FLAG(o->out_byte_off, " out_off=%zu", o->out_byte_off); FLAG(o->chain_n, " chain=%d", o->chain_n);
        FLAG(o->out_pix_stride, " pix_stride=%d", o->out_pix_stride); FLAG(o->kind == OP_FAIL, " err=%d", o->err);
#undef FLAG
        if (full) k = describe_op_full(o, line, sizeof line, k);
        snprintf(line + k, sizeof line - (size_t)k, "\n");
        EMIT();
    }
    for (uint32_t t = 0; t < m->pub.header.num_tensors; t++) {
        const mtensor_t *mt = &m->mt[t];
        const int listed = mt->nhwc_c || mt->partial || mt->zero_from || mt->rec_c || mt->pix_stride;
        if (!listed && !(full && mt->needed)) continue;
        int k = listed ? snprintf(line, sizeof line, "tensor %u nhwc_c %d pitch %d partial %d zero_from %zu rec_c %d pix_stride %d", t, mt->nhwc_c, mt->nhwc_pitch,
                                  mt->partial, mt->zero_from, mt->rec_c, mt->pix_stride)
                       : snprintf(line, sizeof line, "+tensor %u", t);
        if (full)
            k += snprintf(line + k, sizeof line - (size_t)k, " | bytes %zu extent %zu needed %d tail_read %d weight %d io %d,%d pix_c %d rec_hw %d nhwc_hw %d", mt->bytes,
                          mt->extent, mt->needed, mt->tail_read, mt->is_weight, mt->io_in, mt->io_out, mt->pix_c, mt->rec_hw, mt->nhwc_hw);
        snprintf(line + k, sizeof line - (size_t)k, "\n");
        EMIT();
    }
    if (full) {
        const plan_switches_t *w = &m->sw;
        snprintf(line, sizeof line, "+plan n_ops %d arena_size %zu scratch_per_frame %zu blob_mirror_bytes %zu rec_max_frames %zu rec_skipped %d f32_mode %d | fusion %d"
                 " no_fuse_lut %d no_nhwc_internal %d no_vconcat_q %d no_pair_f32 %d no_rec %d no_zero_tail %d no_vconcat_f32 %d no_rowpad %d no_post %d no_split %d no_chain %d rec_limit %zu"
                 " vconcat_limit %zu bottleneck_limit %zu\n", m->n_ops, m->arena_size, m->scratch_per_frame, m->blob_mirror_bytes, m->rec_max_frames, m->rec_skipped,
                 m->plan_f32_mode, w->fusion, w->no_fuse_lut, w->no_nhwc_internal, w->no_vconcat_q, w->no_pair_f32, w->no_rec, w->no_zero_tail, w->no_vconcat_f32,
                 w->no_rowpad, w->no_post, w->no_split, w->no_chain, w->rec_limit, w->vconcat_limit, w->bottleneck_limit);
        EMIT();
    }
#undef EMIT
    if (out && cap) out[n < cap ? n : cap - 1] = 0;
    mars_free(&m->pub);
    return n;
}

int mars_yolo_find_heads(const void *data, size_t size, int *tensor_ids, int *strides, int *num_classes, int cap) {
    mars_model_ext_t *m = NULL;
    if (load_host(data, size, 0, &m) != MARS_OK) return -1;
    const int n = mars_find_heads(m, tensor_ids, strides, num_classes, cap);
    mars_free(&m->pub);
    return n;
}

int mars_yolo_find_dfl_heads(const void *data, size_t size, int *box_ids, int *cls_ids, int *strides, int *num_classes, int *reg_max, int cap) {
    mars_model_ext_t *m = NULL;
    if (load_host(data, size, 0, &m) != MARS_OK) return -1;
    const int n = mars_find_dfl_heads(m, box_ids, cls_ids, strides, num_classes, reg_max, cap);
    mars_free(&m->pub);
    return n;
}

mars_error_t mars_load_memory(const void *data, size_t size, mars_model_t **model) {
    return mars_hip_load_memory_ex(data, size, 0, model);
}

mars_error_t mars_load_file(const char *path, mars_model_t **model) {
    if (!path || !model) return MARS_ERR_INVALID_FILE;
    FILE *fp = fopen(path, "rb");
    if (!fp) {
        fprintf(stderr, "Mars: Cannot open %s\n", path);
        return MARS_ERR_INVALID_FILE;
    }
    fseek(fp, 0, SEEK_END);
    long size = ftell(fp);
    fseek(fp, 0, SEEK_SET);
    if (size <= 0) { fclose(fp); return MARS_ERR_INVALID_FILE; }
    void *buf = malloc((size_t)size);
    if (!buf) { fclose(fp); return MARS_ERR_ALLOC_FAILED; }
    if (fread(buf, 1, (size_t)size, fp) != (size_t)size) { free(buf); fclose(fp); return MARS_ERR_INVALID_FILE; }
    fclose(fp);
    mars_error_t err = mars_load_memory(buf, (size_t)size, model);
    free(buf);
    return err;
}

mars_runtime_tensor_t *mars_get_input(mars_model_t *model, int index) {
    if (!model || index < 0 || (uint32_t)index >= model->header.num_inputs) return NULL;
    uint32_t tid = model->header.input_tensor_ids[index];
    if (tid >= model->header.num_tensors) return NULL;
    return &model->tensors[tid];
// ... 26 lines not shown
```

thingino-accel_amd/csrc/host/mars_plan.c:

```c
#include <math.h>
#include <stdio.h>
#include <stdlib.h>
#include <string.h>
#include <time.h>

#include "mars_internal.h"
#include "nna.h"

int32_t mars_trunc_x86(float x) {
    if (x >= -2147483648.0f && x < 2147483648.0f) return (int32_t)x;
    return INT32_MIN;
}
static int sat8(int32_t v) { return v > 127 ? 127 : (v < -128 ? -128 : v); }
static int q_half_up(float v) { return sat8(mars_trunc_x86(v + 0.5f)); }

size_t elem_size(uint32_t dtype) {
    switch (dtype) {
        case MARS_DTYPE_FLOAT32: case MARS_DTYPE_INT32: return 4;
        case MARS_DTYPE_INT16: return 2;
        default: return 1;
    }
}

size_t shape_numel(const mars_tensor_t *d) {
// ... 554 lines not shown
    int w = 0;
    for (int i = 0; i < m->n_ops; i++)
        if (m->ops[i].kind != -1) m->ops[w++] = m->ops[i];
    m->n_ops = w;
}

size_t planned_stride(const mtensor_t *t) {
    size_t s = ALIGN_UP(t->extent > t->bytes ? t->extent : t->bytes, 256);
    return s ? s : 256;
}

static void lut2_from_lut(mars_model_ext_t *m, mars_op_t *c, const int8_t *tab) {
    if (!mhip_conv_i8_lut2_ok(c->cs)) return;
    int8_t tab2[512];
    for (int k = -256; k < 256; k++) {
        int r = k >= 0 ? (k + 1) >> 1 : -((1 - k) >> 1);
        const int lo = c->relu ? 0 : -128;
        r = r < lo ? lo : (r > 127 ? 127 : r);
        tab2[k + 256] = tab[r + 128];
    }
    c->lut2_off = arena_reserve(m, 512);
    if (c->lut2_off != NO_OFF) memcpy(m->arena_host + c->lut2_off, tab2, 512);
}

void conv_i8_geometry(const mars_op_t *op, int frames, mhip_conv_i8_t *p) {
    memset(p, 0, sizeof(*p));
    p->frames = frames;
    p->in_c = op->in_c; p->in_h = op->in_h; p->in_w = op->in_w;
    p->out_h = op->out_h; p->out_w = op->out_w; p->out_c = op->store_c ? op->store_c : op->out_c;
    p->kh = op->kh; p->kw = op->kw; p->stride_h = op->sh; p->stride_w = op->sw; p->pad_top = op->pt; p->pad_left = op->pl;
    p->row_pad = op->row_pad; p->oc_pad = op->oc_pad; p->safe = op->safe;
    p->out_pix_stride = op->out_pix_stride; p->out_ch_off = op->out_ch_off;
}
int conv_i8_pre_fits(const mars_op_t *op, int frames, size_t in_stride, size_t out_stride) {
    mhip_conv_i8_t p;
    conv_i8_geometry(op, frames, &p);
    p.in_stride = in_stride; p.out_stride = out_stride;
    p.pre_w = (const int8_t *)op; p.pre_bias = (const int32_t *)op; p.pre_lut2 = (const uint8_t *)op; p.lut2 = (const uint8_t *)op;
    p.lut = (const uint8_t *)op;
    return mhip_conv_i8_pre_ok(&p);
}

int conv_i8_post_fits(const mars_model_ext_t *m, const mars_op_t *a, const mars_op_t *b, int frames) {
    mhip_conv_i8_t p;
    if (a->t_in[0] < 0 || a->t_out < 0 || b->t_out < 0) return 0;
    conv_i8_geometry(a, frames, &p);
    p.in_stride = planned_stride(&m->mt[a->t_in[0]]); p.out_stride = planned_stride(&m->mt[a->t_out]);
    p.lut = p.lut2 = p.post_lut2 = (const uint8_t *)a;
    p.post_w = p.post_in = (const int8_t *)a; p.post_out = (int8_t *)m;
    if (a->add_t) p.add = (const int8_t *)a;
    p.post_out_stride = planned_stride(&m->mt[b->t_out]);
    p.post_out_pix_stride = b->out_pix_stride; p.post_out_ch_off = b->out_ch_off;
    return mhip_conv_i8_post_ok(&p);
}

int conv_i8_split_fits(const mars_model_ext_t *m, const mars_op_t *a, const mars_op_t *b, const mars_op_t *c, int frames) {
    mhip_conv_i8_t p;
    if (a->t_in[0] < 0 || a->t_out < 0 || b->t_out < 0 || c->t_out < 0) return 0;
    conv_i8_geometry(a, frames, &p);
    p.in_stride = planned_stride(&m->mt[a->t_in[0]]); p.out_stride = planned_stride(&m->mt[a->t_out]);
    p.lut = p.lut2 = p.split_lut2[0] = p.split_lut2[1] = (const uint8_t *)a;
    p.split_w = (const int8_t *)a; p.split_out[0] = p.split_out[1] = (int8_t *)m;
    p.split_out_stride[0] = planned_stride(&m->mt[b->t_out]); p.split_out_stride[1] = planned_stride(&m->mt[c->t_out]);
    return mhip_conv_i8_split_ok(&p);
}

int conv_i8_chain_fits(const mars_model_ext_t *m, const mars_op_t *a, const mars_op_t *b, const mars_op_t *c, const mars_op_t *d, int side, int frames) {
    mhip_conv_i8_t p;
    if (a->t_in[0] < 0 || a->t_out < 0 || b->t_out < 0 || c->t_out < 0 || d->t_out < 0 || (side != 1 && side != 2)) return 0;
    conv_i8_geometry(a, frames, &p);
    p.in_stride = planned_stride(&m->mt[a->t_in[0]]); p.out_stride = planned_stride(&m->mt[a->t_out]);
    p.lut = p.lut2 = p.split_lut2[0] = p.split_lut2[1] = p.chain_lut2 = (const uint8_t *)a;
    p.split_w = p.chain_w = (const int8_t *)a;
    p.split_out[0] = (int8_t *)m; p.split_out[1] = (int8_t *)m + 1; p.chain_out = (int8_t *)m + 2;
    p.split_out_stride[0] = planned_stride(&m->mt[b->t_out]); p.split_out_stride[1] = planned_stride(&m->mt[c->t_out]);
    p.chain_side = side; p.chain_out_stride = planned_stride(&m->mt[d->t_out]);
    return mhip_conv_i8_split_ok(&p);
}

static int match_silu(const mars_model_ext_t *m, int i, int f32, const int *readers, const int *writers, int q[3], int *fwd) {
    const mars_op_t *c = &m->ops[i], *s = c + 1, *mu = c + 2;
    if (c->kind != (f32 ? OP_CONV_F32 : OP_CONV_I8) || s->kind != (f32 ? OP_SIGMOID_F32 : OP_LUT_I8) || mu->kind != (f32 ? OP_BINARY_F32 : OP_BINARY_I8) || !mu->is_mul)
        return 0;
    if (!f32 && m->pub.layers[s->layer].desc.type != MARS_LAYER_SIGMOID) return 0;
    const int q1 = q[0] = c->t_out, q2 = q[1] = s->t_out, q3 = q[2] = mu->t_out;
    if (s->t_in[0] != q1 || q1 == q2 || q2 == q3 || q1 == q3) return 0;
    *fwd = mu->t_in[0] == q1 && mu->t_in[1] == q2;
    if (!*fwd && !(mu->t_in[0] == q2 && mu->t_in[1] == q1)) return 0;
    if (f32 ? q3 == c->t_in[0] || m->mt[q3].is_weight : op_reads(c, q3)) return 0;
    if (readers[q1] != 2 || readers[q2] != 1 || writers[q1] != 1 || writers[q2] != 1 || writers[q3] != 1) return 0;
    if (m->mt[q1].io_out || m->mt[q2].io_out || m->mt[q1].io_in || m->mt[q2].io_in) return 0;
    const size_t n1 = (size_t)c->out_h * c->out_w * c->out_c;
    return s->n == n1 && mu->n == n1;
}

void fold_silu(mars_model_ext_t *m, int f32) {
    int *readers, *writers;
    if (!use_counts(m, &readers, &writers)) return;
    for (int i = 0; i + 2 < m->n_ops; i++) {
        mars_op_t *c = &m->ops[i];
        int q[3], fwd;
        if (!match_silu(m, i, f32, readers, writers, q, &fwd)) continue;
        const size_t n1 = (size_t)c->out_h * c->out_w * c->out_c;
        if (f32) {
            c->silu_f32 = 1;
        } else {
// ... 476 lines not shown
                                (int8_t *)(m->arena_host + off));
        a->split_next = 1;
        a->split_w_off = off;
        m->mt[T].needed = 0;
        i += 2;
    }
    free(readers);
}

static int chain_mate_ok(const mars_op_t *d, const mars_op_t *a) {
    return d->kind == OP_CONV_I8 && d->kh == 1 && d->kw == 1 && d->sh == 1 && d->sw == 1 && !d->pt && !d->pl && d->safe && !d->nchw && !d->out_nchw && !d->add_t &&
           !d->chain_n && !d->store_c && !d->in_byte_off && !d->out_byte_off && !d->out_pix_stride && !d->out_ch_off && d->lut_off != NO_OFF &&
           d->lut2_off != NO_OFF && !d->nseg && !d->pre && !d->pair_next && !d->post_next && !d->split_next && d->n_in == 1 && d->in_c == 32 && d->out_c == 32 &&
           d->oc_pad == 32 && d->row_pad == 32 && d->in_h == a->out_h && d->in_w == a->out_w && d->out_h == a->out_h && d->out_w == a->out_w;
}
void fuse_split_chain(mars_model_ext_t *m) {
    if (m->sw.no_chain || m->no_chain || m->sw.no_split || m->no_split) return;
    int *readers, *writers;
    if (!use_counts(m, &readers, &writers)) return;
    for (int i = 0; i + 3 < m->n_ops; i++) {
        mars_op_t *a = &m->ops[i];
        if (a->kind != OP_CONV_I8 || !a->split_next || a->split_chain) continue;
        const int O0 = a[1].t_out, O1 = a[2].t_out;
        for (int j = i + 3; j < m->n_ops && j <= i + 48; j++) {
            const mars_op_t *d = &m->ops[j];
            if (!chain_mate_ok(d, a) || m->ops[j - 1].pair_next || m->ops[j - 1].post_next || m->ops[j - 1].split_next ||
                (j >= 2 && m->ops[j - 2].split_next))
                continue;
            const int side = d->t_in[0] == O0 ? 1 : (d->t_in[0] == O1 ? 2 : 0), O = d->t_out;
            if (!side || O < 0 || O == O0 || O == O1 || O == a->t_out || writers[O] != 1 || m->mt[O].io_in || m->mt[O].is_weight || m->mt[O].pix_stride ||
                op_reads(a, O) || op_reads(d, O))
                continue;
            if (touched_between(m, i + 3, j, O, USE_READ | USE_WRITE) || touched_between(m, i + 3, j, d->t_in[0], USE_WRITE)) continue;
            if (!conv_i8_chain_fits(m, a, a + 1, a + 2, d, side, 1)) continue;
            const size_t bytes = mhip_conv_i8_chain_pack(NULL, NULL, NULL);
            const size_t off = arena_reserve(m, bytes);
            if (off == NO_OFF) { free(readers); return; }
            mhip_conv_i8_chain_pack((const int8_t *)(m->arena_host + d->w_off), d->b_off != NO_OFF ? (const int32_t *)(m->arena_host + d->b_off) : NULL,
                                    (int8_t *)(m->arena_host + off));
            if (j > i + 3) {
                const mars_op_t moved = *d;
                memmove(&m->ops[i + 4], &m->ops[i + 3], sizeof(mars_op_t) * (size_t)(j - i - 3));
                m->ops[i + 3] = moved;
            }
            a->split_chain = side;
            a->chain_w_off = off;
            break;
        }
        i += 2;
    }
    free(readers);
}

void pad_output_rows(mars_model_ext_t *m) {
    for (uint32_t i = 0; i < m->pub.header.num_tensors; i++) m->mt[i].pix_c = m->mt[i].pix_stride = 0;
    if (m->sw.no_rowpad) return;
    for (int i = 0; i < m->n_ops; i++) {
        mars_op_t *o = &m->ops[i];
        if (o->kind != OP_CONV_I8 || o->out_nchw || o->out_pix_stride || o->out_ch_off || o->add_t || o->t_out < 0 ||
            (o->out_c & 15) == 0 || (o->in_c & 15) != 0)
            continue;
        mtensor_t *t = &m->mt[o->t_out];
        const int P = (o->out_c + 15) & ~15;
        const size_t px = (size_t)o->out_h * o->out_w;
        if (!t->io_out || t->io_in || P > o->oc_pad || t->bytes != px * (size_t)o->out_c || (px * P) % 256 != 0) continue;
        if (touched_by_other(m, o->t_out, i, i)) continue;
        o->out_pix_stride = P;
        o->store_c = P;
        t->pix_c = o->out_c;
        t->pix_stride = P;
        if (px * P > t->extent) t->extent = px * P;
    }
}

void virtual_concat(mars_model_ext_t *m) {
    const int nt = (int)m->pub.header.num_tensors;
    for (int T = 0; T < nt; T++) {
        const mtensor_t *mt = &m->mt[T];
        if (mt->is_weight || mt->io_in || mt->io_out) continue;
        int sl[4], ns = 0, bad = 0, first_reader = -1, last_reader = -1, last_slice = -1;
        for (int i = 0; i < m->n_ops && !bad; i++) {
            const mars_op_t *o = &m->ops[i];
            if (o->t_out == T) {
                if (o->kind != OP_CONCAT_SLICE || ns >= 4) bad = 1;
                else { sl[ns++] = i; last_slice = i; }
            }
            for (int k = 0; k < o->n_in; k++)
                if (o->t_in[k] == T) {
                    if (o->kind != OP_CONV_I8 || k != 0 || o->n_in != 1 || o->nchw || o->kh != 1 || o->kw != 1 || o->sh != 1 ||
                        o->sw != 1 || o->pt || o->pl || !o->safe || o->nseg || (o->out_c & 15) || o->in_h != o->out_h ||
                        o->in_w != o->out_w || (o->in_c & (o->in_c - 1)) != 0 || o->add_t)
                        bad = 1;
                    if (first_reader < 0) first_reader = i;
                    last_reader = i;
                }
        }
        if (bad || ns < 2 || first_reader < 0 || last_slice > first_reader) continue;
        for (int a = 0; a < ns; a++)
            for (int b = a + 1; b < ns; b++)
                if (m->ops[sl[b]].ch_off < m->ops[sl[a]].ch_off) { int t = sl[a]; sl[a] = sl[b]; sl[b] = t; }
        int c = 0;
        const mars_op_t *s0 = &m->ops[sl[0]];
        for (int a = 0; a < ns && !bad; a++) {
            const mars_op_t *o = &m->ops[sl[a]];
            if (o->ch_off != c || (o->in_c & 31) || o->out_h != s0->out_h || o->out_w != s0->out_w || o->out_c != s0->out_c ||
                o->t_in[0] == T || o->t_in[0] < 0)
// ... 19 lines not shown
                o->seg_c[a] = m->ops[sl[a]].in_c;
            }
        }
        for (int a = 0; a < ns; a++) m->ops[sl[a]].kind = -1;
        m->mt[T].needed = 0;
        for (int a = 0; a < ns; a++) {
            const int S = m->ops[sl[a]].t_in[0];
            int up = -1, nread = 0, nwrite = 0, ok = 1;
            for (int i = 0; i < m->n_ops; i++) {
                const mars_op_t *o = &m->ops[i];
                if (o->kind == -1) continue;
                if (o->t_out == S) { nwrite++; up = i; }
                for (int k = 0; k < o->n_in; k++)
                    if (o->t_in[k] == S && !(o->kind == OP_CONV_I8 && o->nseg == ns && o->seg_t[a] == S)) nread++;
            }
            if (nwrite != 1 || nread != 0 || up < 0 || m->mt[S].io_out || m->mt[S].io_in || m->mt[S].is_weight) continue;
            const mars_op_t *u = &m->ops[up];
            if (u->kind != OP_UPSAMPLE || u->out_pix_stride || u->scale_h != 2 || u->scale_w != 2 || u->out_h != 2 * u->in_h ||
                u->out_w != 2 * u->in_w || u->in_c != m->ops[sl[a]].in_c || u->out_h != s0->out_h || u->out_w != s0->out_w)
                continue;
            const int U = u->t_in[0];
            if (U < 0 || U == S) continue;
            int last = -1;
            for (int i = 0; i < m->n_ops; i++)
                if (m->ops[i].kind == OP_CONV_I8 && m->ops[i].nseg == ns && m->ops[i].seg_t[a] == S) last = i;
            for (int i = up; i <= last && ok; i++)
                if (m->ops[i].kind != -1 && m->ops[i].t_out == U) ok = 0;
            if (!ok) continue;
            for (int i = 0; i < m->n_ops; i++) {
                mars_op_t *o = &m->ops[i];
                if (o->kind == OP_CONV_I8 && o->nseg == ns && o->seg_t[a] == S) {
                    o->seg_t[a] = o->t_in[a] = U;
                    o->seg_up |= 1 << a;
                }
            }
            m->ops[up].kind = -1;
            m->mt[S].needed = 0;
        }
    }
    drop_dead_ops(m);
}

static int same_conv_input(const mars_op_t *a, const mars_op_t *b) {
    if (a->n_in != b->n_in || a->nseg != b->nseg || a->seg_up != b->seg_up) return 0;
    for (int k = 0; k < a->n_in; k++)
        if (a->t_in[k] != b->t_in[k]) return 0;
    for (int k = 0; k < a->nseg; k++)
        if (a->seg_t[k] != b->seg_t[k] || a->seg_c[k] != b->seg_c[k]) return 0;
    return a->in_h == b->in_h && a->in_w == b->in_w && a->in_c == b->in_c && a->out_h == b->out_h && a->out_w == b->out_w &&
           a->kh == b->kh && a->kw == b->kw && a->sh == b->sh && a->sw == b->sw && a->pt == b->pt && a->pl == b->pl &&
           a->row_pad == b->row_pad && a->oc_pad == b->oc_pad;
}
static int pairable(const mars_op_t *o) {
    return o->kind == OP_CONV_I8 && !o->nchw && !o->out_nchw && !o->add_t && !o->nseg && o->safe && o->lut_off != NO_OFF && !o->pair_next &&
           (o->in_c & 15) == 0 && o->in_c > 4 && (o->out_c & 15) == 0 && !o->out_pix_stride;
}
static int pair_up(mars_model_ext_t *m, int i, int j) {
    const mars_op_t *b = &m->ops[j];
    if (touched_between(m, i + 1, j, b->t_out, USE_READ | USE_WRITE)) return 0;
    for (int k = 0; k < b->n_in; k++)
        if (touched_between(m, i + 1, j, b->t_in[k], USE_WRITE)) return 0;
    const mars_op_t moved = *b;
    memmove(&m->ops[i + 2], &m->ops[i + 1], sizeof(mars_op_t) * (size_t)(j - i - 1));
    m->ops[i + 1] = moved;
    m->ops[i].pair_next = 1;
    return 1;
}
void pair_convs(mars_model_ext_t *m) {
    for (int i = 0; i + 1 < m->n_ops; i++) {
        mars_op_t *a = &m->ops[i];
        if (!pairable(a) || (i > 0 && m->ops[i - 1].pair_next)) continue;
        for (int j = i + 1; j < m->n_ops && j <= i + 48; j++) {
            mars_op_t *b = &m->ops[j];
            if (!pairable(b) || !same_conv_input(a, b) || b->t_out == a->t_out) continue;
            if (op_reads(b, b->t_out) || op_reads(b, a->t_out)) continue;
            if (pair_up(m, i, j)) break;
        }
    }
}

static int pairable_f32(const mars_op_t *o) {
    return o->kind == OP_CONV_F32 && !o->add_t && o->n_in == 1 && o->w2_off != NO_OFF && o->w3_off == NO_OFF && !o->pair_next && !o->in_rec && !o->out_rec &&
           o->kh == 1 && o->kw == 1;
}
void pair_convs_f32(mars_model_ext_t *m) {
    if (m->sw.no_pair_f32) return;
    for (int i = 0; i + 1 < m->n_ops; i++) {
        mars_op_t *a = &m->ops[i];
        if (!pairable_f32(a) || (i > 0 && m->ops[i - 1].pair_next)) continue;
        for (int j = i + 1; j < m->n_ops && j <= i + 48; j++) {
            mars_op_t *b = &m->ops[j];
            if (!pairable_f32(b) || b->t_in[0] != a->t_in[0] || b->t_out == a->t_out || b->t_out < 0 || a->t_out < 0) continue;
            if (a->in_h != b->in_h || a->in_w != b->in_w || a->in_c != b->in_c || a->out_h != b->out_h || a->out_w != b->out_w || a->out_c != b->out_c ||
                a->sh != b->sh || a->sw != b->sw || a->pt != b->pt || a->pl != b->pl || a->silu_f32 != b->silu_f32 || a->f32_exact != b->f32_exact)
                continue;
            if (planned_stride(&m->mt[a->t_out]) != planned_stride(&m->mt[b->t_out])) continue;
            if (a->w2_planes != b->w2_planes) continue;
            int ok = b->t_in[0] != b->t_out && b->t_in[0] != a->t_out;
            for (int q = i + 1; q < j && ok; q++)
                if (m->ops[q].pair_next) ok = 0;
            if (ok && pair_up(m, i, j)) break;
        }
    }
}

void fuse_pool_chains(mars_model_ext_t *m) {
    for (int i = 0; i + 1 < m->n_ops; i++) {
        mars_op_t *a = &m->ops[i];
        if (a->kind != OP_MAXPOOL || a->chain_n || a->sh != 1 || a->sw != 1 || a->out_pix_stride || (a->in_c & 15) ||
            a->out_h != a->in_h || a->out_w != a->in_w || a->kh <= 0 || a->kw <= 0 || (size_t)a->in_h * a->in_w * 64 > 60 * 1024 ||
            a->t_out < 0 || m->mt[a->t_out].io_out)
            continue;
        int n = 1;
        a->chain_out[0] = a->t_out;
        while (n < 3 && i + n < m->n_ops) {
            const mars_op_t *b = &m->ops[i + n];
            if (b->kind != OP_MAXPOOL || b->t_in[0] != a->chain_out[n - 1] || b->sh != 1 || b->sw != 1 || b->out_pix_stride ||
                b->in_c != a->in_c || b->in_h != a->in_h || b->in_w != a->in_w || b->out_h != a->in_h || b->out_w != a->in_w ||
                b->kh != a->kh || b->kw != a->kw || b->t_out < 0 || m->mt[b->t_out].io_out || b->t_out == a->t_in[0])
                break;
            a->chain_out[n] = b->t_out;
            n++;
        }
        if (n < 2) continue;
        a->chain_n = n;
        for (int k = 1; k < n; k++) {
            a->bytes += m->ops[i + k].bytes - (double)a->in_h * a->in_w * a->in_c;
            m->ops[i + k].kind = -1;
        }
// ... 214 lines not shown
            h->vc_n = N - 1; h->vc_run = Wb / 4;
            h->n_in = N;
            for (int k = 0; k < N - 1; k++) { h->vc_t[k] = firsts[k]; h->t_in[1 + k] = firsts[k]; }
            h->macs = (double)(sB / 4) * x->out_c * (double)(km + 1);
            h->bytes = ((double)(sB / 4) * (double)(km + 1) + (double)(sB / 4) * x->out_c) * 4.0;
            h->variant = 0;
            h->w3_off = wt_off[q]; h->w3_stem = 0;
            h->w2_off = NO_OFF; h->w2_planes = 0;
        }
        memmove(&m->ops[first_op], &m->ops[e + 1], sizeof(mars_op_t) * (size_t)(m->n_ops - e - 1));
        m->n_ops -= N;
        m->mt[T].needed = 0;
        m->mt[T].partial = 1;
        m->mt[T].zero_from = 0;
        i = first_op - 1;
    }
}

void f32_policy(mars_model_ext_t *m) {
    const int nt = (int)m->pub.header.num_tensors;
    unsigned char *hot = (unsigned char *)calloc((size_t)nt + 1, 1);
    if (!hot) {
        for (int i = 0; i < m->n_ops; i++) m->ops[i].f32_exact = 1;
        return;
    }
    for (int i = m->n_ops - 1; i >= 0; i--) {
        mars_op_t *o = &m->ops[i];
        int reach = 0;
        if (o->kind == OP_MAXPOOL && o->t_in[0] >= 0 && m->pub.tensors[o->t_in[0]].desc.dtype == MARS_DTYPE_FLOAT32) reach = 1;
        if (o->kind == OP_RELU_BYTES && o->t_out >= 0) {
            hot[o->t_out] = 1;
            continue;
        }
        if (o->t_out >= 0 && hot[o->t_out]) reach = 1;
        for (int k = 0; k < o->chain_n; k++)
            if (o->chain_out[k] >= 0 && hot[o->chain_out[k]]) reach = 1;
        if (!reach) continue;
        for (int k = 0; k < o->n_in; k++)
            if (o->t_in[k] >= 0) hot[o->t_in[k]] = 1;
        if (o->kind == OP_CONV_F32) o->f32_exact = 1;
    }
    free(hot);
}

void plan_check(mars_model_ext_t *m) {
    for (int i = 0; i < m->n_ops; i++) {
        const mars_op_t *o = &m->ops[i];
        const char *why = NULL;
        if (o->kind == -1) why = "a dead op is left";
        else if (o->n_in < 0 || o->n_in > 4 || o->nseg < 0 || o->nseg > 4 || o->chain_n < 0 || o->chain_n > 3 || o->vc_n < 0 || o->vc_n > 3) why = "an operand count is out of range";
        else if (o->add_t && !op_reads(o, o->add_t - 1)) why = "add_t is not among t_in";
        else if (o->chain_n && o->t_out != o->chain_out[o->chain_n - 1]) why = "t_out is not the chain's last stage";
        else if (o->pair_next && (i + 1 >= m->n_ops || m->ops[i + 1].kind != o->kind)) why = "pair_next without a mate of its kind";
        else if (o->post_next && (o->kind != OP_CONV_I8 || i + 1 >= m->n_ops || m->ops[i + 1].kind != OP_CONV_I8 || m->ops[i + 1].nseg != 2 ||
                                  m->ops[i + 1].seg_t[0] != o->t_out || !op_reads(o, m->ops[i + 1].seg_t[1])))
            why = "post_next without its 1x1 behind it, or y2 is not among t_in";
        else if (o->split_next && (o->kind != OP_CONV_I8 || i + 2 >= m->n_ops || m->ops[i + 1].kind != OP_CONV_I8 || m->ops[i + 2].kind != OP_CONV_I8 ||
                                   !m->ops[i + 1].pair_next || m->ops[i + 2].pair_next || m->ops[i + 1].n_in != 1 || m->ops[i + 2].n_in != 1 ||
                                   m->ops[i + 1].t_in[0] != o->t_out || m->ops[i + 2].t_in[0] != o->t_out || o->post_next || o->pair_next || o->pre || o->add_t))
            why = "split_next without its pair of 1x1s behind it";
        else if (o->split_chain && (!o->split_next || i + 3 >= m->n_ops || !chain_mate_ok(&m->ops[i + 3], o) || (o->split_chain != 1 && o->split_chain != 2) ||
                                    m->ops[i + 3].t_in[0] != m->ops[i + o->split_chain].t_out || m->ops[i + 3].t_out < 0 ||
                                    m->ops[i + 3].t_out == m->ops[i + 1].t_out || m->ops[i + 3].t_out == m->ops[i + 2].t_out || m->ops[i + 3].t_out == o->t_out ||
                                    m->mt[m->ops[i + 3].t_out].pix_stride || o->chain_w_off == NO_OFF))
            why = "split_chain without its 1x1 behind the pair";
        for (int k = 0; !why && k < o->nseg; k++)
            if (!op_reads(o, o->seg_t[k])) why = "a seg_t is not among t_in";
        for (int k = 0; !why && k < o->vc_n; k++)
            if (!op_reads(o, o->vc_t[k])) why = "a vc_t is not among t_in";
        if (!why) continue;
        VLOG("plan_check: op %d (layer %d, kind %d): %s\n", i, o->layer, o->kind, why);
        m->plan_err = MARS_ERR_LAYER_FAILED;
        return;
    }
}
```

thingino-accel_amd/csrc/host/mars_run.c:

```c
#include <math.h>
#include <stdio.h>
#include <stdlib.h>
#include <string.h>
#include <time.h>

#include "mars_internal.h"
#include "nna.h"

static int g_graph_max_batch = 8;
static unsigned g_tune_gen = 1;
static int g_dual_min_batch = 64;
static int g_dual_ways = 2;
static uint8_t *tdev(const mars_model_ext_t *m, int ti) {
    if (ti < 0 || !m->mt[ti].dev) return NULL;
    return m->mt[ti].dev + (m->mt[ti].is_weight ? 0 : (size_t)m->frame0 * m->mt[ti].stride);
}
static size_t tstride(const mars_model_ext_t *m, int ti) { return ti >= 0 ? m->mt[ti].stride : 0; }

void conv_i8_params(const mars_model_ext_t *m, const mars_op_t *op, mhip_conv_i8_t *p) {
    uint8_t *A = m->arena_dev;
    conv_i8_geometry(op, m->run_frames, p);
    p->in = (const int8_t *)tdev(m, op->t_in[0]); p->in_stride = tstride(m, op->t_in[0]);
    p->out = (int8_t *)tdev(m, op->t_out); p->out_stride = tstride(m, op->t_out);
    if (p->in) p->in += op->in_byte_off;
// ... 261 lines not shown
    if (!m->act_dev || !m->arena_dev) return MARS_ERR_NNA_INIT_FAILED;
    int graphable = g_graph_max_batch > 0 && m->batch <= g_graph_max_batch && !m->profiling && !m->pipe;
    for (int i = 0; i < m->n_ops && graphable; i++)
        if (m->ops[i].kind == OP_FAIL) graphable = 0;
    if (!graphable) return enqueue_plan(model);
    if (m->graph_exec && m->graph_gen != g_tune_gen) {
        drop_graph(m);
        m->ran_plain = 0;
    }
    if (!m->graph_exec) {
        if (!m->ran_plain) {
            mars_error_t e = enqueue_plan(model);
            if (e == MARS_OK) m->ran_plain = 1;
            return e;
        }
        if (m->tail_pending) {
            mhip_select_stream(0);
            if (mhip_stream_wait(0, m->ev_tail_done)) return MARS_ERR_LAYER_FAILED;
            m->tail_pending = 0;
        }
        if (mhip_graph_begin() == 0) {
            mars_error_t e = enqueue_plan(model);
            m->graph_exec = mhip_graph_end(e == MARS_OK);
            m->graph_gen = g_tune_gen;
            if (e != MARS_OK) { m->graph_exec = NULL; return e; }
        }
        VLOG("plan of %d launches at batch %d %s\n", m->n_ops, m->batch, m->graph_exec ? "captured into a HIP graph" : "could not be captured");
        if (!m->graph_exec) {
            g_graph_max_batch = 0;
            return enqueue_plan(model);
        }
    }
    if (m->tail_pending) {
        mhip_select_stream(0);
        if (mhip_stream_wait(0, m->ev_tail_done)) return MARS_ERR_LAYER_FAILED;
        m->tail_pending = 0;
    }
    if (mhip_graph_launch(m->graph_exec)) return MARS_ERR_LAYER_FAILED;
    for (uint32_t i = 0; i < model->header.num_layers; i++) model->layers[i].is_executed = true;
    return MARS_OK;
}

static mars_error_t enqueue_range(mars_model_ext_t *m, int sid, int wait_tail) {
    void *prof_last = NULL;
    mhip_select_stream(sid);
    m->scratch_t = -1;
    for (int i = 0; i < m->n_ops; i++) {
        mars_op_t *op = &m->ops[i];
        if (op->kind == OP_FAIL) {
            fprintf(stderr, "Mars: Layer %d execution failed\n", op->layer);
            return (mars_error_t)op->err;
        }
        mars_op_t *mate = (op->pair_next || op->post_next || op->split_next) && i + 1 < m->n_ops ? &m->ops[i + 1] : NULL;
        mars_op_t *mate2 = op->split_next && i + 2 < m->n_ops ? &m->ops[i + 2] : NULL;
        mars_op_t *mate3 = op->split_next && op->split_chain && i + 3 < m->n_ops ? &m->ops[i + 3] : NULL;
        if (wait_tail && ((op->t_out >= 0 && (m->mt[op->t_out].io_out || m->mt[op->t_out].tail_read)) ||
                          (mate && mate->t_out >= 0 && (m->mt[mate->t_out].io_out || m->mt[mate->t_out].tail_read)) ||
                          (mate2 && mate2->t_out >= 0 && (m->mt[mate2->t_out].io_out || m->mt[mate2->t_out].tail_read)) ||
                          (mate3 && mate3->t_out >= 0 && (m->mt[mate3->t_out].io_out || m->mt[mate3->t_out].tail_read)))) {
            mhip_stream_wait(sid, m->ev_tail_done);
            wait_tail = 0;
        }
        if (m->profiling) {
            if (!op->ev1) op->ev1 = mhip_event_create();
            if (!prof_last) {
                if (!op->ev0) op->ev0 = mhip_event_create();
                mhip_event_record(op->ev0);
                prof_last = op->ev0;
            }
            op->ev_start = prof_last;
        }
        int rc;
        if (op->split_next) {
            mhip_conv_i8_t pa;
            rc = -1;
            if (mate && mate2 && (mate3 || !op->split_chain)) {
                conv_i8_split_params(m, op, mate, mate2, &pa);
                if (mate3) conv_i8_chain_params(m, op, mate3, &pa);
                rc = mhip_conv_i8(&pa);
            }
            i += mate3 ? 3 : 2;
        } else if (mate && op->post_next) {
            mhip_conv_i8_t pa;
            conv_i8_post_params(m, op, mate, &pa);
            rc = mhip_conv_i8(&pa);
            i++;
        } else if (mate && op->kind == OP_CONV_F32) {
            mhip_conv_f32_t pa, pb;
            conv_f32_params(m, op, &pa);
            conv_f32_params(m, mate, &pb);
            rc = mhip_conv_f32_pair(&pa, &pb);
            if (rc == -2) {
                rc = launch_op(m, op);
                if (!rc) rc = launch_op(m, mate);
            }
            i++;
        } else if (mate) {
            mhip_conv_i8_t pa, pb;
            conv_i8_params(m, op, &pa);
            conv_i8_params(m, mate, &pb);
            rc = mhip_conv_i8_pair(&pa, &pb);
            if (rc == -2) {
                rc = launch_op(m, op);
                if (!rc) rc = launch_op(m, mate);
            }
            i++;
        } else {
            rc = launch_op(m, op);
        }
        {
            const mars_op_t *w2[4] = {op, mate, mate2, mate3};
            for (int q = 0; q < 4; q++)
                if (w2[q] && op_writes(w2[q], m->scratch_t)) m->scratch_t = -1;
        }
        if (m->profiling) {
            const int nx = i + 1;
            const int end = m->profiling != 2 || nx >= m->n_ops || m->ops[nx].prof_kind != op->prof_kind;
            op->prof_rec = end;
            if (end) {
                mhip_event_record(op->ev1);
                prof_last = op->ev1;
            }
        }
        if (rc != 0) {
            fprintf(stderr, "Mars: Layer %d launch failed: %s\n", op->layer, mhip_last_error());
            return MARS_ERR_LAYER_FAILED;
        }
    }
    return MARS_OK;
}

static mars_error_t enqueue_plan(mars_model_t *model) {
    mars_model_ext_t *m = (mars_model_ext_t *)model;
    for (uint32_t i = 0; i < model->header.num_layers; i++) model->layers[i].is_executed = false;
    const int B = m->batch;
    int dual = g_dual_min_batch > 0 && B >= g_dual_min_batch && B >= 2 && !m->profiling &&
               !(g_graph_max_batch > 0 && B <= g_graph_max_batch);
    if (dual) {
        if (!m->ev_fork) m->ev_fork = mhip_event_create_sync();
        for (int k = 0; k < 3; k++) {
            if (!m->ev_join[k]) m->ev_join[k] = mhip_event_create_sync();
            if (!m->ev_join[k]) dual = 0;
        }
        if (!m->ev_fork) dual = 0;
    }
    mars_error_t e;
    if (!dual) {
        m->frame0 = 0; m->run_frames = B;
        e = enqueue_range(m, 0, m->tail_pending);
    } else {
        const int ways = g_dual_ways < B ? g_dual_ways : B;
        mhip_select_stream(0);
        int rc = mhip_event_record(m->ev_fork);
        for (int k = 1; k < ways && !rc; k++) rc = mhip_stream_wait(3 + k, m->ev_fork);
// ... 247 lines not shown

int mars_hip_get_tuning(const char *key, int *value) { return value ? tune_raw(key, 0, value) : -1; }

int mars_hip_model_set_tuning(mars_model_t *model, const char *key, int value) {
    mars_model_ext_t *m = (mars_model_ext_t *)model;
    int cur;
    if (!m || !key || strlen(key) >= sizeof m->tune[0].key || tune_raw(key, 0, &cur)) return -1;
    if (tune_raw(key, value, NULL)) return -1;
    tune_raw(key, cur, NULL);
    int i = 0;
    while (i < m->n_tune && strcmp(m->tune[i].key, key)) i++;
    if (i == m->n_tune) {
        if (m->n_tune == MARS_MAX_MODEL_TUNE) return -1;
        strcpy(m->tune[m->n_tune++].key, key);
    }
    m->tune[i].value = value;
    drop_graph(m);
    if (!strcmp(key, "f32_mfma") && replan_for_f32_mode(m) != MARS_OK) return -1;
    return 0;
}

int mars_hip_model_get_tuning(mars_model_t *model, const char *key, int *value) {
    mars_model_ext_t *m = (mars_model_ext_t *)model;
    if (!m || !key || !value) return -1;
    for (int i = 0; i < m->n_tune; i++)
        if (!strcmp(m->tune[i].key, key)) { *value = m->tune[i].value; return 0; }
    return tune_raw(key, 0, value);
}

static mars_error_t autotune_model(mars_model_t *model, int reps);
mars_error_t mars_hip_autotune(mars_model_t *model, int reps) {
    if (!model) return MARS_ERR_INVALID_FILE;
    tune_push((mars_model_ext_t *)model);
    mars_error_t e = autotune_model(model, reps);
    tune_pop((mars_model_ext_t *)model);
    return e;
}
static mars_error_t autotune_model(mars_model_t *model, int reps) {
    mars_model_ext_t *m = (mars_model_ext_t *)model;
    if (!m->act_dev || !m->arena_dev) return MARS_ERR_NNA_INIT_FAILED;
    drop_graph(m);
    if (reps <= 0) reps = 3;
    void *e0 = mhip_event_create(), *e1 = mhip_event_create();
    if (!e0 || !e1) return MARS_ERR_ALLOC_FAILED;
    mars_error_t err = MARS_OK;
    if (mhip_sync()) err = MARS_ERR_LAYER_FAILED;
    for (int i = 0; i < m->n_ops && err == MARS_OK; i++) {
        mars_op_t *op = &m->ops[i];
        if (op->kind != OP_CONV_I8 || op->nchw) continue;
        if (op->pair_next || (i > 0 && m->ops[i - 1].pair_next)) continue;
        if (op->post_next || (i > 0 && m->ops[i - 1].post_next)) continue;
        if (op->split_next) continue;
        if (i >= 3 && m->ops[i - 3].split_chain) continue;
        mhip_conv_i8_t p;
        conv_i8_params(m, op, &p);
        int codes[32];
        const int n = mhip_conv_i8_variants(&p, codes, 32);
        if (getenv("MARS_VERBOSE") && atoi(getenv("MARS_VERBOSE")) > 1)
            fprintf(stderr, "Mars: autotune layer %d: %dx%dx%d -> %dx%dx%d k%dx%d s%d pixstride %d choff %d lut %d safe %d\n", op->layer,
                    p.in_h, p.in_w, p.in_c, p.out_h, p.out_w, p.out_c, p.kh, p.kw, p.stride_w, p.out_pix_stride, p.out_ch_off,
                    p.lut != NULL, p.safe);
        float best = 0.0f;
        int best_code = 0;
        for (int k = 0; k < n && err == MARS_OK; k++) {
            p.variant = codes[k];
            int rc = mhip_conv_i8(&p);
            if (!rc) rc = mhip_event_record(e0);
            for (int r = 0; r < reps && !rc; r++) rc = mhip_conv_i8(&p);
            if (!rc) rc = mhip_event_record(e1);
            if (rc || mhip_sync()) { err = MARS_ERR_LAYER_FAILED; break; }
            const float ms = mhip_event_elapsed_ms(e0, e1);
            if (getenv("MARS_VERBOSE") && atoi(getenv("MARS_VERBOSE")) > 1)
                fprintf(stderr, "Mars: autotune layer %d: candidate %d: %.1f us\n", op->layer, codes[k], ms * 1000.0f / reps);
            if (best_code == 0 || ms < best) { best = ms; best_code = codes[k]; }
        }
        if (err == MARS_OK && best_code) {
            if (getenv("MARS_VERBOSE"))
                fprintf(stderr, "Mars: autotune layer %d: variant %d (%.1f us) of %d candidates, default %d\n", op->layer,
                        best_code, best * 1000.0f / reps, n, n ? codes[0] : 0);
            op->variant = best_code;
        }
    }
    mhip_event_destroy(e0);
    mhip_event_destroy(e1);
    return err;
}

void *mars_hip_tensor_device(mars_model_t *model, int ti, size_t *frame_stride) {
    if (!model || ti < 0 || (uint32_t)ti >= model->header.num_tensors) return NULL;
    mars_model_ext_t *m = (mars_model_ext_t *)model;
    if (frame_stride) *frame_stride = m->mt[ti].stride;
    return m->mt[ti].dev;
}

size_t mars_hip_tensor_frame_bytes(const mars_model_t *model, int ti) {
    if (!model || ti < 0 || (uint32_t)ti >= model->header.num_tensors) return 0;
    return ((const mars_model_ext_t *)model)->mt[ti].bytes;
}

int mars_hip_tensor_row_pitch(mars_model_t *model, int ti, int *row_bytes) {
    if (!model || ti < 0 || (uint32_t)ti >= model->header.num_tensors) return 0;
    const mtensor_t *t = &((mars_model_ext_t *)model)->mt[ti];
    if (row_bytes) *row_bytes = t->pix_stride ? t->pix_c : 0;
    return t->pix_stride;
}

// ... 150 lines not shown
```

thingino-accel_amd/csrc/mhip.h:

```cpp
#ifndef MHIP_H
#define MHIP_H

#include <stddef.h>
#include <stdint.h>

#ifdef __cplusplus
extern "C" {
#endif

int mhip_init(int device_hint);
void mhip_shutdown(void);
int mhip_ready(void);
int mhip_device_info(int *cu_count, int *lds_bytes, int *gfx_version, size_t *hbm_bytes);
void *mhip_stream(void);
int mhip_sync(void);
void mhip_select_aux(int on);
void mhip_select_stream(int which);
int mhip_stream_wait(int which, void *ev);
int mhip_event_sync(void *ev);
void *mhip_malloc(size_t bytes);
void mhip_free(void *p);
void *mhip_host_alloc(size_t bytes);
void mhip_host_free(void *p);
int mhip_memset_async(void *dst, int value, size_t bytes);
// ... 36 lines not shown
    int relu;
    int out_nchw;
    int in_planar;
    int safe;
    int out_pix_stride;
    int out_ch_off;
    int variant;
    const int8_t *add;
    float add_s_conv, add_s_other, add_inv;
    int nseg;
    const int8_t *seg_in[4];
    size_t seg_stride[4];
    int seg_c[4], seg_c0[4];
    int seg_up;
    const int8_t *post_w;
    const uint8_t *post_lut2;
    float post_cs;
    const int8_t *post_in;  size_t post_in_stride;
    int8_t *post_out;       size_t post_out_stride;
    int post_out_pix_stride, post_out_ch_off;
    const int8_t *split_w;
    const uint8_t *split_lut2[2];
    float split_cs[2];
    int8_t *split_out[2];   size_t split_out_stride[2];
    int chain_side;
    const int8_t *chain_w;
    const uint8_t *chain_lut2;
    float chain_cs;
    int8_t *chain_out;      size_t chain_out_stride;
} mhip_conv_i8_t;
int mhip_conv_i8_split_ok(const mhip_conv_i8_t *p);
size_t mhip_conv_i8_split_pack(const int8_t *packed0, const int32_t *bias0, const int8_t *packed1, const int32_t *bias1, int8_t *out);
int mhip_conv_i8_split_row(int side, int oc);
size_t mhip_conv_i8_chain_pack(const int8_t *packed, const int32_t *bias, int8_t *out);
int mhip_conv_i8_chain_k(int c);
int mhip_conv_i8_post_ok(const mhip_conv_i8_t *p);
size_t mhip_conv_i8_post_pack(int c, const int8_t *packed, const int32_t *bias, int8_t *out);
int mhip_conv_i8_post_k(int c, int k);
int mhip_conv_i8_post_row(int c, int oc);
int mhip_conv_i8_oc_row(int oc, int oc_pad);
int mhip_conv_i8_pre_ok(const mhip_conv_i8_t *p);
size_t mhip_conv_i8_rgb_pack(int in_c, int kh, int kw, int stride_h, int stride_w, int pad_left, int oc_pad, int k64,
                             const int8_t *packed, int8_t *out);
size_t mhip_conv_i8_rows_pack(int in_c, int kh, int kw, int stride_h, int stride_w, int oc_pad, int k64, int out_w,
                              const int8_t *packed, int8_t *out);
unsigned long mhip_conv_i8_rows_launches(void);
int mhip_conv_i8_is_safe(float cs);
int mhip_conv_i8_lut2_ok(float cs);
int mhip_conv_i8_tune(const char *key, int value);
int mhip_conv_i8_tune_get(const char *key, int *value);
int mhip_conv_i8_variants(const mhip_conv_i8_t *p, int *codes, int max);
int mhip_conv_i8_seg_ok(const mhip_conv_i8_t *p);
int mhip_conv_i8_pair(const mhip_conv_i8_t *a, const mhip_conv_i8_t *b);
int mhip_conv_i8_small_c(int in_c, int kw, int out_c);
void mhip_conv_i8_pack_geom(int in_c, int kw, int out_c, int *row_pad, int *oc_pad, int *c_eff);
int mhip_conv_i8(const mhip_conv_i8_t *p);

typedef struct {
    const float *in;  size_t in_stride;
    float *out;       size_t out_stride;
    const float *w;   const float *bias;
    const void *w_split;
    const void *w_patch;
    int frames;
    int in_h, in_w, in_c, out_h, out_w, out_c;
    int kh, kw, stride_h, stride_w, pad_top, pad_left;
    int silu;
    const float *add; size_t add_stride;
    int use_mfma;
    int k_limit;
    int k_limit_required;
    int in_rec, out_rec;
} mhip_conv_f32_t;
int mhip_conv_f32(const mhip_conv_f32_t *p);
size_t mhip_conv_f32_vcat_pack(int out_c, int in_c, int planes, const float *w, float *out);
int mhip_conv_f32_vcat_head(const mhip_conv_f32_t *p, const float *w_t, const float *const *first, const size_t *first_strides, int n_first, int run_floats);
int mhip_conv_f32_pair(const mhip_conv_f32_t *a, const mhip_conv_f32_t *b);
unsigned long mhip_conv_f32_pair_launches(void);
size_t mhip_conv_f32_split_pack(int out_c, int in_c, int kh, int kw, int stride_w, int planes, const float *w, void *out);
unsigned long mhip_conv_f32_split_launches(void);
int mhip_conv_f32_split_takes(int out_c, int in_c, int kh, int kw, int stride_h, int stride_w, int pad_left, int in_w, int out_w);
size_t mhip_conv_f32_patch_pack(int out_c, int in_c, int kh, int kw, int stride, int pad, int in_h, int in_w, int out_h, int out_w,
                                const float *w, void *out);
size_t mhip_conv_f32_patch_pack2(int out_c, int in_c, int kh, int kw, int stride, int pad, int in_h, int in_w, int out_h, int out_w,
                                 int rec, const float *w, void *out);
int mhip_conv_f32_patch_geom2(int out_c, int in_c, int kh, int kw, int stride, int pad, int in_h, int in_w, int out_h, int out_w,
                              int rec, int *outv, int cap);
unsigned long mhip_conv_f32_prec_launches(void);
unsigned long mhip_conv_f32_recin_launches(void);
int mhip_conv_f32_patch_rec_form(int out_c, int in_c, int kh, int kw, int stride, int pad, int in_h, int in_w, int out_h, int out_w);
int mhip_conv_f32_patch_geom(int out_c, int in_c, int kh, int kw, int stride, int pad, int in_h, int in_w, int out_h, int out_w,
                             int *outv, int cap);
unsigned long mhip_conv_f32_patch_launches(void);
size_t mhip_conv_f32_stem_pack(int out_c, int in_c, int kh, int kw, int stride, int pad, int in_h, int in_w, int out_h, int out_w,
                               const float *w, void *out);
unsigned long mhip_conv_f32_stem_launches(void);
int mhip_conv_f32_mode(int set);

int mhip_lut_i8(const int8_t *in, size_t in_stride, int8_t *out, size_t out_stride, int frames,
                size_t n, const uint8_t *lut_dev);
int mhip_relu_bytes(int8_t *buf, size_t stride, int frames, size_t n);
int mhip_binary_i8(int is_mul, const int8_t *a, size_t a_stride, const int8_t *b, size_t b_stride,
                   int8_t *out, size_t out_stride, int frames, size_t n, float sa, float sb, float inv_so,
                   int out_run, int out_pix_stride, int out_ch_off);
int mhip_sigmoid_f32(const float *in, size_t in_stride, float *out, size_t out_stride, int frames, size_t n);
int mhip_binary_f32(int op , const float *a, size_t a_stride, const float *b,
// ... 269 lines not shown
```

Baseline: 60470.

## Fuse paired convs into one tile and chain a trailing 1x1 conv

Adds a BOTH mode to the persistent int8 conv kernel. Two convs that read the same input are computed side by side in one 128- or 256-row output tile, so the input tile is loaded once for both instead of once per side. Adds a CHAIN mode that runs a following 64-channel 1x1 conv on one side's requantized output directly in the epilogue using MFMA. When that intermediate tensor has no other reader, its store is skipped. This needs more LDS for the extra lookup tables and chain weights, more register pressure from 256-row tiles, and a more complex host-side pass that reorders ops.

```diff
diff --git a/thingino-accel_amd/csrc/hip/conv_i8.hip b/thingino-accel_amd/csrc/hip/conv_i8.hip
--- a/thingino-accel_amd/csrc/hip/conv_i8.hip
+++ b/thingino-accel_amd/csrc/hip/conv_i8.hip
@@ -316,6 +316,19 @@
     else wait_vmcnt<0>();
 }
 
+struct conv_chain_t {
+    const int8_t *w;
+    const int32_t *bias;
+    const uint8_t *lut2;
+    int8_t *out;
+    size_t out_stride;
+    unsigned out_bytes;
+    float cs;
+    int side, elide;
+};
+#define CHAIN_W_OFF (3 * LUTB)
+#define CHAIN_B_OFF (CHAIN_W_OFF + 4096)
+#define CHAIN_LDS (LUTB + 4096 + 256)
 struct conv_out_side_t {
     int8_t *out;
     size_t out_stride;
@@ -326,27 +339,31 @@
     float cs;
     unsigned out_bytes;
 };
-template <int BPX, int BN, int STAGES, bool HAS_LUT, bool SEG = false, bool PAIR = false>
+template <int BPX, int BN, int STAGES, bool HAS_LUT, bool SEG = false, bool PAIR = false, bool BOTH = false, bool CHAIN = false>
 __global__ __launch_bounds__(NTHREADS) void conv_i8_persist(const mhip_conv_i8_t pin, const unsigned total_pix, const int k64,
                                                             const int8_t *__restrict__ zeros, const unsigned noc,
                                                             const unsigned npt, const unsigned ngrp, const int lg_inc,
                                                             const unsigned kw_magic, const fastdiv_t dhw, const fastdiv_t dow,
                                                             const unsigned out_bytes_first, const conv_out_side_t alt,
                                                             const unsigned noc0, const int bufmode, const unsigned in_bytes,
-                                                            const int wres) {
+                                                            const int wres, const conv_chain_t ch) {
     ANAT_BEGIN();
     const int STAGE = wres ? BPX * BK : (BPX + BN) * BK;
-    constexpr int NWN = BN == 128 ? 2 : 1;
+    constexpr int NWN = BN >= 128 ? 2 : 1;
     constexpr int NWM = 4 / NWN;
     constexpr int WPX = BPX / NWM / 16;
     constexpr int WOC = BN / NWN / 16;
     constexpr int XI = BPX / 64;
-    constexpr int LW = BN >= 128 ? 2 : 1;
+    constexpr int LW = BN >= 128 ? BN / 64 : 1;
     constexpr int L = XI + LW;
-    constexpr int NST = WPX;
+    constexpr int NST = WPX * (WOC == 8 ? 2 : 1);
+    static_assert(!BOTH || ((BN == 128 || BN == 256) && HAS_LUT && !PAIR), "BOTH: two sides of 64 (128) channels with half-step tables in one 128 (256) row tile");
+    static_assert(BOTH || BN <= 128, "the 256-row tile exists for two sides of 128 channels only");
+    static_assert(!CHAIN || BN == 128, "CHAIN: sides of 64 channels");
+    static_assert(!CHAIN || BOTH, "CHAIN: a 1x1 behind one side of a one-tile pair");
     extern __shared__ __attribute__((aligned(16))) int8_t dynlds[];
     uint8_t *slut = (uint8_t *)dynlds;
-    int8_t *lds = dynlds + LUTB;
+    int8_t *lds = dynlds + (BOTH ? 2 : 1) * LUTB + (CHAIN ? CHAIN_LDS : 0);
     lds_base_must_be_zero(dynlds);
 
     const int tid = threadIdx.x, lane = tid & 63;
@@ -356,8 +373,9 @@
     unsigned ot = id - grp * noc;
     mhip_conv_i8_t p = pin;
     unsigned out_bytes = out_bytes_first;
-    if (PAIR && ot >= noc0) {
-        ot -= noc0;
+    const bool second = BOTH ? wv >= NWM : (PAIR && ot >= noc0);
+    if (PAIR && second) ot -= noc0;
+    if (second) {
         p.lut2 = alt.lut2;
         p.out = alt.out; p.out_stride = alt.out_stride; p.w = alt.w; p.bias = alt.bias; p.lut = alt.lut;
         p.out_c = alt.out_c; p.relu = alt.relu; p.out_pix_stride = alt.out_pix_stride; p.out_ch_off = alt.out_ch_off;
@@ -371,18 +389,30 @@
     const unsigned hw = (unsigned)(p.out_h * p.out_w);
     const int wm = wv % NWM, wn = wv / NWM;
     const int pxw = wm * (WPX * 16), ocw = wn * (WOC * 16);
+    const int ocs = BOTH ? 0 : ocw;
 
     auto packed_row16 = [](int c) { return ((c >> 2) & 1) * 16 + (c >> 3) * 4 + (c & 3); };
     v4i bias[WOC];
 #pragma unroll
     for (int s = 0; s < WOC; s++)
-        bias[s] = p.bias ? *(const v4i *)(p.bias + (BN == 16 ? packed_row16((lane >> 4) * 4) : oc0 + ocw + s * 16 + (lane >> 4) * 4)) : (v4i){0, 0, 0, 0};
+        bias[s] = p.bias ? *(const v4i *)(p.bias + (BN == 16 ? packed_row16((lane >> 4) * 4) : oc0 + ocs + s * 16 + (lane >> 4) * 4)) : (v4i){0, 0, 0, 0};
     if (HAS_LUT) {
-        if (p.lut2) { if (tid < 128) ((uint32_t *)slut)[tid] = ((const uint32_t *)p.lut2)[tid]; }
+        if (BOTH) {
+            if (tid < 128) {
+                ((uint32_t *)slut)[tid] = ((const uint32_t *)pin.lut2)[tid];
+                ((uint32_t *)slut)[128 + tid] = ((const uint32_t *)alt.lut2)[tid];
+                if (CHAIN) ((uint32_t *)slut)[256 + tid] = ((const uint32_t *)ch.lut2)[tid];
+            }
+            if (CHAIN && tid < 64) ((int32_t *)(dynlds + CHAIN_B_OFF))[tid] = ch.bias ? ch.bias[tid] : 0;
+        } else if (p.lut2) { if (tid < 128) ((uint32_t *)slut)[tid] = ((const uint32_t *)p.lut2)[tid]; }
         else if (tid < 64) ((uint32_t *)slut)[tid] = ((const uint32_t *)p.lut)[tid];
         __syncthreads();
     }
     const __amdgpu_buffer_rsrc_t orsrc = __builtin_amdgcn_make_buffer_rsrc(p.out, 0, (int)out_bytes, 0x00020000);
+    const bool chw = CHAIN && wn == ch.side - 1;
+    const bool store_own = !(chw && ch.elide);
+    const __amdgpu_buffer_rsrc_t drsrc = __builtin_amdgcn_make_buffer_rsrc(ch.out, 0, CHAIN ? (int)ch.out_bytes : 0, 0x00020000);
+    const int nstw = NST * ((store_own ? 1 : 0) + (chw ? 1 : 0));
 
     const int schunk = (lane & 3) ^ (((lane >> 4) & 1) << 1);
     const int8_t *xwin[XI];
@@ -424,7 +454,7 @@
 #pragma unroll
     for (int j = 0; j < LW; j++) {
         wq[j] = BN >= 64 ? wv * LW + j : (BN == 16 ? 0 : (wv & 1));
-        const int wrow = BN == 16 ? packed_row16(lane >> 2) : oc0 + wq[j] * 16 + (lane >> 2);
+        const int wrow = BN == 16 ? packed_row16(lane >> 2) : oc0 + (BOTH ? wq[j] & (BN / 32 - 1) : wq[j]) * 16 + (lane >> 2);
         wsrc[j] = p.w + (size_t)wrow * k64 + schunk * 16;
         wvoff[j] = wrow * k64 + schunk * 16;
     }
@@ -437,14 +467,14 @@
         int8_t *sb = lds + stage * STAGE;
         const unsigned pos = (unsigned)(ks * BK + schunk * 16);
         if (SEG) {
-            auto owner = [&](int c) { return (c >= p.seg_c0[1]) + (c >= p.seg_c0[2]) + (c >= p.seg_c0[3]); };
+            auto owner = [&](int c) { return (c >= pin.seg_c0[1]) + (c >= pin.seg_c0[2]) + (c >= pin.seg_c0[3]); };
             const int sa = owner(ks * BK), sb2 = owner(ks * BK + 32);
             const bool hi = schunk >= 2;
-            const int8_t *base = hi ? p.seg_in[sb2] : p.seg_in[sa];
-            const unsigned fstride = (unsigned)(hi ? p.seg_stride[sb2] : p.seg_stride[sa]);
-            const unsigned segc = (unsigned)(hi ? p.seg_c[sb2] : p.seg_c[sa]);
-            const unsigned coff = pos - (unsigned)(hi ? p.seg_c0[sb2] : p.seg_c0[sa]);
-            const bool up = ((p.seg_up >> (hi ? sb2 : sa)) & 1) != 0;
+            const int8_t *base = hi ? pin.seg_in[sb2] : pin.seg_in[sa];
+            const unsigned fstride = (unsigned)(hi ? pin.seg_stride[sb2] : pin.seg_stride[sa]);
+            const unsigned segc = (unsigned)(hi ? pin.seg_c[sb2] : pin.seg_c[sa]);
+            const unsigned coff = pos - (unsigned)(hi ? pin.seg_c0[sb2] : pin.seg_c0[sa]);
+            const bool up = ((pin.seg_up >> (hi ? sb2 : sa)) & 1) != 0;
             const bool kvalid = (int)pos < p.in_c;
 #pragma unroll
             for (int j = 0; j < XI; j++) {
@@ -485,6 +515,7 @@
     };
 
     int8_t *const wres_base = lds + STAGES * STAGE;
+    if (CHAIN) glds16(ch.w + (size_t)(wv * 16 + (lane >> 2)) * BK + schunk * 16, dynlds + CHAIN_W_OFF + wv * 16 * BK);
     if (wres)
         for (int ks = 0; ks < nks; ks++)
 #pragma unroll
@@ -513,7 +544,7 @@
     nstage = STAGES - 1;
 
     const int frow = lane & 15, fchunk = lane >> 4;
-    const int chan = ocw + (lane >> 4) * (4 * WOC);
+    const int chan = ocs + (lane >> 4) * (4 * WOC);
     const int pstride = p.out_pix_stride ? p.out_pix_stride : p.out_c;
     const int lo = p.relu ? 0 : -128;
     const uint8_t *lut128 = slut + 128;
@@ -523,7 +554,8 @@
     for (unsigned tile = t0; tile < t1; tile++) {
         v4i acc[WOC][WPX];
         for (int ks = 0; ks < nks; ks++) {
-            wait_vmcnt_at_most<(STAGES - 2) * L, NST>(younger[0]);
+            if (CHAIN && younger[0] >= 2 * NST + (STAGES - 2) * L) wait_vmcnt<2 * NST + (STAGES - 2) * L>();
+            else wait_vmcnt_at_most<(STAGES - 2) * L, NST>(younger[0]);
             __builtin_amdgcn_s_barrier();
             asm volatile("" ::: "memory");
             const int8_t *xs = lds + stage * STAGE, *ws = wres ? wres_base + ks * (BN * BK) : xs + BPX * BK;
@@ -561,6 +593,14 @@
 #ifdef ANATOMY
         if (tile + 1 == t1) ANAT_NOW(2);
 #endif
+        v4i wd[CHAIN ? 4 : 1], bd[CHAIN ? 4 : 1];
+        if (CHAIN && chw) {
+#pragma unroll
+            for (int s = 0; s < 4; s++) {
+                wd[CHAIN ? s : 0] = *(const v4i *)(dynlds + CHAIN_W_OFF + lds_off(s * 16 + frow, fchunk));
+                bd[CHAIN ? s : 0] = *(const v4i *)(dynlds + CHAIN_B_OFF + (s * 16 + (lane >> 4) * 4) * 4);
+            }
+        }
 #pragma unroll
         for (int t = 0; t < WPX; t++) {
             const unsigned pix = tile * BPX + pxw + t * 16 + (lane & 15);
@@ -574,10 +614,42 @@
             for (int s = 0; s < WOC; s++)
 #pragma unroll
                 for (int r = 0; r < 4; r++) a[s * 4 + r] = acc[s][t][r];
-            if (HAS_LUT && p.lut2) requant_pack<WOC * 4, HAS_LUT, true, true, false, true>(a, p.cs, lo, lut128, pk);
+            if constexpr (BOTH && WOC == 8) {
+#pragma unroll
+                for (int h = 0; h < 2; h++) {
+                    int ah[16];
+                    uint32_t ph[4];
+#pragma unroll
+                    for (int q = 0; q < 16; q++) ah[q] = a[h * 16 + q];
+                    if (second) requant_pack_at<16, LUTB>(ah, p.cs, ph);
+                    else requant_pack_at<16, 0>(ah, p.cs, ph);
+                    const int vo = pix < total_pix ? (int)(f * (unsigned)p.out_stride + rem * (unsigned)pstride) + h * 64 + (lane >> 4) * 16 : -1;
+                    __builtin_amdgcn_raw_buffer_store_b128((v4i){(int)ph[0], (int)ph[1], (int)ph[2], (int)ph[3]}, orsrc, vo, 0, 0);
+                }
+                continue;
+            } else if constexpr (BOTH) {
+                if (second) requant_pack_at<WOC * 4, LUTB>(a, p.cs, pk);
+                else requant_pack<WOC * 4, HAS_LUT, true, true, false, true>(a, p.cs, lo, lut128, pk);
+            } else if (HAS_LUT && p.lut2) requant_pack<WOC * 4, HAS_LUT, true, true, false, true>(a, p.cs, lo, lut128, pk);
             else requant_pack<WOC * 4, HAS_LUT, true, true>(a, p.cs, lo, lut128, pk);
             const int voff = ok ? (int)off : -1;
-            if (WOC == 4)
+            if constexpr (CHAIN) {
+                if (store_own) __builtin_amdgcn_raw_buffer_store_b128((v4i){(int)pk[0], (int)pk[1], (int)pk[2], (int)pk[3]}, orsrc, voff, 0, 0);
+                if (chw) {
+                    const v4i xd = {(int)pk[0], (int)pk[1], (int)pk[2], (int)pk[3]};
+                    int ad[16];
+#pragma unroll
+                    for (int s = 0; s < 4; s++) {
+                        const v4i r = __builtin_amdgcn_mfma_i32_16x16x64_i8(wd[s], xd, bd[s], 0, 0, 0);
+#pragma unroll
+                        for (int e = 0; e < 4; e++) ad[s * 4 + e] = r[e];
+                    }
+                    uint32_t pd[4];
+                    requant_pack_at<16, 2 * LUTB>(ad, ch.cs, pd);
+                    const unsigned offd = f * (unsigned)ch.out_stride + rem * 64u + (unsigned)chan;
+                    __builtin_amdgcn_raw_buffer_store_b128((v4i){(int)pd[0], (int)pd[1], (int)pd[2], (int)pd[3]}, drsrc, pix < total_pix ? (int)offd : -1, 0, 0);
+                }
+            } else if (WOC == 4)
                 __builtin_amdgcn_raw_buffer_store_b128((v4i){(int)pk[0], (int)pk[1], (int)pk[2], (int)pk[3]}, orsrc, voff, 0, 0);
             else if (WOC == 2)
                 __builtin_amdgcn_raw_buffer_store_b64((v2i){(int)pk[0], (int)pk[WOC > 1 ? 1 : 0]}, orsrc, voff, 0, 0);
@@ -604,7 +676,7 @@
             }
         }
 #pragma unroll
-        for (int i = 0; i < STAGES - 1; i++) younger[i] += ragged ? NST * (WOC == 4 ? 5 : 4) : NST;
+        for (int i = 0; i < STAGES - 1; i++) younger[i] += CHAIN ? nstw : (ragged ? NST * (WOC == 4 ? 5 : 4) : NST);
     }
     ANAT_END(p);
 }
@@ -774,6 +846,8 @@
         g_tune.few_wgs = env_int("MARS_HIP_FEW_WGS", 256);
         g_tune.patch_ring = env_int("MARS_HIP_PATCH_RING", 0);
         g_tune.patch_lds_kb = env_int("MARS_HIP_PATCH_LDS_KB", 80);
+        g_tune.both_bpx = env_int("MARS_HIP_BOTH_BPX", 0);
+        g_tune.both_wide = env_int("MARS_HIP_BOTH_WIDE", 0);
         g_tune.init = 1;
     }
     return g_tune;
@@ -783,7 +857,7 @@
     (void)conv_i8_tune_state();
     struct { const char *k; int *v; } tab[] = {{"persist", &g_tune.persist}, {"persist_stages", &g_tune.persist_stages},
                                                {"persist_maxk", &g_tune.persist_maxk}, {"persist_slots", &g_tune.persist_slots}, {"wres", &g_tune.wres}, {"rgb_direct", &g_tune.rgb_direct}, {"small_batch", &g_tune.small_batch},
-                                               {"rows", &g_tune.rows}, {"few_wgs", &g_tune.few_wgs}, {"patch_ring", &g_tune.patch_ring}, {"patch_lds_kb", &g_tune.patch_lds_kb}, {"stages", &g_tune.stages}, {"bpx", &g_tune.bpx}, {"variant", &g_tune.variant}, {"bufmode", &g_tune.bufmode}};
+                                               {"rows", &g_tune.rows}, {"few_wgs", &g_tune.few_wgs}, {"patch_ring", &g_tune.patch_ring}, {"patch_lds_kb", &g_tune.patch_lds_kb}, {"both_bpx", &g_tune.both_bpx}, {"both_wide", &g_tune.both_wide}, {"stages", &g_tune.stages}, {"bpx", &g_tune.bpx}, {"variant", &g_tune.variant}, {"bufmode", &g_tune.bufmode}};
     for (auto &e : tab)
         if (key && !strcmp(key, e.k)) {
             if (get) *get = *e.v;
@@ -833,48 +907,51 @@
 template <int BPX, int BN>
 static size_t wres_lds(int k64) { return LUTB + 2 * (size_t)BPX * BK + (size_t)(k64 / BK) * BN * BK; }
 
-template <int BPX, int BN, int STAGES, bool HAS_LUT, bool SEG = false, bool PAIR = false>
+template <int BPX, int BN, int STAGES, bool HAS_LUT, bool SEG = false, bool PAIR = false, bool BOTH = false, bool CHAIN = false>
 static int launch_persist_t(const mhip_conv_i8_t *p, long total_pix, int k64, int lg, unsigned magic,
-                            const mhip_conv_i8_t *second = nullptr, int wres = 0) {
+                            const mhip_conv_i8_t *second = nullptr, int wres = 0, const conv_chain_t *chain = nullptr) {
     if (BN == 16 && (p->out_c > 16 || p->oc_pad != 32 || (PAIR && (second->out_c > 16 || second->oc_pad != 32)))) return -1;
-    const unsigned noc0 = BN == 16 ? 1u : (unsigned)(p->oc_pad / BN);
+    const unsigned noc0 = BN == 16 || BOTH ? 1u : (unsigned)(p->oc_pad / BN);
     const unsigned npt = (unsigned)((total_pix + BPX - 1) / BPX), noc = noc0 + (PAIR ? (BN == 16 ? 1u : (unsigned)(second->oc_pad / BN)) : 0u);
     conv_out_side_t alt;
     memset(&alt, 0, sizeof(alt));
-    if (PAIR) {
+    if (PAIR || BOTH) {
         alt.out = second->out; alt.out_stride = second->out_stride; alt.w = second->w; alt.bias = second->bias;
         alt.lut = second->lut; alt.lut2 = second->lut2; alt.out_c = second->out_c; alt.relu = second->relu; alt.out_pix_stride = second->out_pix_stride;
         alt.out_ch_off = second->out_ch_off; alt.cs = second->cs;
     }
-    if (PAIR) alt.out_bytes = (unsigned)persist_out_bytes(second);
+    if (PAIR || BOTH) alt.out_bytes = (unsigned)persist_out_bytes(second);
     if (wres && STAGES != 2) return -1;
-    const size_t lds = wres ? wres_lds<BPX, BN>(k64) : LUTB + (size_t)STAGES * (BPX + BN) * BK;
+    conv_chain_t ch;
+    memset(&ch, 0, sizeof(ch));
+    if (CHAIN) ch = *chain;
+    const size_t lds = (BOTH ? LUTB : 0) + (CHAIN ? CHAIN_LDS : 0) + (wres ? wres_lds<BPX, BN>(k64) : LUTB + (size_t)STAGES * (BPX + BN) * BK);
     if (wres) {
         static bool attr = false;
-        if (!attr && hipFuncSetAttribute((const void *)conv_i8_persist<BPX, BN, STAGES, HAS_LUT, SEG, PAIR>,
+        if (!attr && hipFuncSetAttribute((const void *)conv_i8_persist<BPX, BN, STAGES, HAS_LUT, SEG, PAIR, BOTH, CHAIN>,
                                          hipFuncAttributeMaxDynamicSharedMemorySize, 80 * 1024) != hipSuccess)
             return mhip_check(hipErrorUnknown, "conv_i8_persist LDS attribute");
         attr = true;
         int occ = 0, dev = 0;
         hipDeviceProp_t prop;
-        if (hipOccupancyMaxActiveBlocksPerMultiprocessor(&occ, conv_i8_persist<BPX, BN, STAGES, HAS_LUT, SEG, PAIR>, NTHREADS, lds) != hipSuccess ||
+        if (hipOccupancyMaxActiveBlocksPerMultiprocessor(&occ, conv_i8_persist<BPX, BN, STAGES, HAS_LUT, SEG, PAIR, BOTH, CHAIN>, NTHREADS, lds) != hipSuccess ||
             hipGetDevice(&dev) != hipSuccess || hipGetDeviceProperties(&prop, dev) != hipSuccess)
             return mhip_check(hipErrorUnknown, "conv_i8_persist occupancy query");
         unsigned g = (unsigned)((occ > 0 ? occ : 1) * prop.multiProcessorCount) / noc;
         if (tune().persist_slots > 0) g = (unsigned)tune().persist_slots / noc;
         if (g < 1) g = 1;
         if (g > npt) g = npt;
-        hipLaunchKernelGGL((conv_i8_persist<BPX, BN, STAGES, HAS_LUT, SEG, PAIR>), dim3(noc * g), dim3(NTHREADS), lds,
+        hipLaunchKernelGGL((conv_i8_persist<BPX, BN, STAGES, HAS_LUT, SEG, PAIR, BOTH, CHAIN>), dim3(noc * g), dim3(NTHREADS), lds,
                            mhip_stream_native(), *p, (unsigned)total_pix, k64, (const int8_t *)mhip_zero_page(), noc, npt, g, lg,
                            magic, make_fastdiv((unsigned)(p->out_h * p->out_w)), make_fastdiv((unsigned)p->out_w),
-                           (unsigned)persist_out_bytes(p), alt, noc0, SEG ? 0 : buf_mode(p, k64), (unsigned)in_extent_bytes(p), 1);
+                           (unsigned)persist_out_bytes(p), alt, noc0, SEG ? 0 : buf_mode(p, k64), (unsigned)in_extent_bytes(p), 1, ch);
         return mhip_check(hipGetLastError(), "conv_i8_persist (resident weights) launch");
     }
     static int slots = 0;
     if (!slots) {
         int occ = 0, dev = 0;
         hipDeviceProp_t prop;
-        if (hipOccupancyMaxActiveBlocksPerMultiprocessor(&occ, conv_i8_persist<BPX, BN, STAGES, HAS_LUT, SEG, PAIR>, NTHREADS, lds) != hipSuccess ||
+        if (hipOccupancyMaxActiveBlocksPerMultiprocessor(&occ, conv_i8_persist<BPX, BN, STAGES, HAS_LUT, SEG, PAIR, BOTH, CHAIN>, NTHREADS, lds) != hipSuccess ||
             hipGetDevice(&dev) != hipSuccess || hipGetDeviceProperties(&prop, dev) != hipSuccess)
             return mhip_check(hipErrorUnknown, "conv_i8_persist occupancy query");
         slots = (occ > 0 ? occ : 1) * prop.multiProcessorCount;
@@ -882,10 +959,10 @@
     unsigned ngrp = (unsigned)(tune().persist_slots > 0 ? tune().persist_slots : 4 * slots) / noc;
     if (ngrp < 1) ngrp = 1;
     if (ngrp > npt) ngrp = npt;
-    hipLaunchKernelGGL((conv_i8_persist<BPX, BN, STAGES, HAS_LUT, SEG, PAIR>), dim3(noc * ngrp), dim3(NTHREADS), lds,
+    hipLaunchKernelGGL((conv_i8_persist<BPX, BN, STAGES, HAS_LUT, SEG, PAIR, BOTH, CHAIN>), dim3(noc * ngrp), dim3(NTHREADS), lds,
                        mhip_stream_native(), *p, (unsigned)total_pix, k64, (const int8_t *)mhip_zero_page(), noc, npt, ngrp, lg,
                        magic, make_fastdiv((unsigned)(p->out_h * p->out_w)), make_fastdiv((unsigned)p->out_w),
-                       (unsigned)persist_out_bytes(p), alt, noc0, SEG ? 0 : buf_mode(p, k64), (unsigned)in_extent_bytes(p), 0);
+                       (unsigned)persist_out_bytes(p), alt, noc0, SEG ? 0 : buf_mode(p, k64), (unsigned)in_extent_bytes(p), 0, ch);
     return mhip_check(hipGetLastError(), "conv_i8_persist launch");
 }
 
@@ -1121,6 +1198,88 @@
     return launch_pair_t<128, 32>(a, b, total_pix, k64, lg, magic, wres);
 }
 
+static bool both_shape_ok(const mhip_conv_i8_t *a, const mhip_conv_i8_t *b) {
+    if (!a || !b || !tune().persist) return false;
+    if (a->in_stride != b->in_stride || a->frames != b->frames || a->in_h != b->in_h || a->in_w != b->in_w || a->in_c != b->in_c ||
+        a->out_h != b->out_h || a->out_w != b->out_w || a->row_pad != b->row_pad || a->nseg != b->nseg || a->seg_up != b->seg_up)
+        return false;
+    for (const mhip_conv_i8_t *p : {a, b}) {
+        if (p->kh != 1 || p->kw != 1 || p->stride_h != 1 || p->stride_w != 1 || p->pad_top || p->pad_left || p->in_h != p->out_h ||
+            p->in_w != p->out_w || (p->out_c != 64 && !(p->out_c == 128 && tune().both_wide && (p->nseg > 1 || tune().both_wide > 1))) || p->oc_pad != p->out_c || p->out_c != a->out_c || p->out_pix_stride || p->out_ch_off || !p->lut || !p->lut2 ||
+            p->add || p->out_nchw || p->in_c < 64 || p->row_pad != p->in_c || !persist_eligible(p))
+            return false;
+        if (p->nseg > 1 && !seg_valid(p)) return false;
+    }
+    for (int i = 0; i < a->nseg; i++)
+        if (a->seg_c[i] != b->seg_c[i] || a->seg_stride[i] != b->seg_stride[i]) return false;
+    const long total_pix = (long)a->frames * a->out_h * a->out_w;
+    return total_pix > 0 && total_pix <= 0x7fffffffL - 256 && a->out != b->out;
+}
+extern "C" int mhip_conv_i8_both_ok(const mhip_conv_i8_t *a, const mhip_conv_i8_t *b) { return both_shape_ok(a, b) ? 1 : 0; }
+
+static void both_form(int rows, int nks, bool chain, int *bpx, int *wres) {
+    *bpx = tune().both_bpx == 128 || tune().both_bpx == 256 ? tune().both_bpx : 128;
+    *wres = tune().wres && 2 * LUTB + (chain ? CHAIN_LDS : 0) + 2 * (size_t)*bpx * BK + (size_t)nks * rows * BK <= 80 * 1024;
+}
+static bool chain_shape_ok(const mhip_conv_i8_t *a, const mhip_conv_i8_t *b, const mhip_conv_i8_t *d, int side) {
+    if (!both_shape_ok(a, b) || a->out_c != 64 || !d || (side != 1 && side != 2)) return false;
+    return d->kh == 1 && d->kw == 1 && d->stride_h == 1 && d->stride_w == 1 && !d->pad_top && !d->pad_left && d->in_c == 64 && d->out_c == 64 &&
+           d->oc_pad == 64 && d->row_pad == 64 && d->frames == a->frames && d->in_h == a->out_h && d->in_w == a->out_w && d->out_h == a->out_h &&
+           d->out_w == a->out_w && !d->out_pix_stride && !d->out_ch_off && d->lut && d->lut2 && !d->add && !d->out_nchw && d->nseg <= 1 &&
+           persist_eligible(d) && d->out != a->out && d->out != b->out;
+}
+extern "C" int mhip_conv_i8_both_chain_ok(const mhip_conv_i8_t *a, const mhip_conv_i8_t *b, const mhip_conv_i8_t *d, int side) {
+    return chain_shape_ok(a, b, d, side) ? 1 : 0;
+}
+static int both_launch(const mhip_conv_i8_t *a, const mhip_conv_i8_t *b, const conv_chain_t *ch);
+extern "C" int mhip_conv_i8_both_chain(const mhip_conv_i8_t *a, const mhip_conv_i8_t *b, const mhip_conv_i8_t *d, int side, int elide) {
+    if (!chain_shape_ok(a, b, d, side) || !d->w || !d->out) return -2;
+    const mhip_conv_i8_t *src = side == 1 ? a : b;
+    const mhip_conv_i8_t *other = side == 1 ? b : a;
+    if (!other->out) return -2;
+    if (!elide && (!src->out || d->in != src->out || d->in_stride != src->out_stride)) return -2;
+    conv_chain_t ch;
+    ch.w = d->w; ch.bias = d->bias; ch.lut2 = d->lut2; ch.out = d->out; ch.out_stride = d->out_stride;
+    ch.out_bytes = (unsigned)persist_out_bytes(d); ch.cs = d->cs; ch.side = side; ch.elide = elide ? 1 : 0;
+    return both_launch(a, b, &ch);
+}
+extern "C" int mhip_conv_i8_both(const mhip_conv_i8_t *a, const mhip_conv_i8_t *b) {
+    if (!a || !b || !a->out || !b->out) return -2;
+    return both_launch(a, b, nullptr);
+}
+static int both_launch(const mhip_conv_i8_t *a, const mhip_conv_i8_t *b, const conv_chain_t *ch) {
+    if (!both_shape_ok(a, b) || (tune().variant && !ch) || !mhip_zero_page()) return -2;
+    if (a->nseg > 1) {
+        for (int i = 0; i < a->nseg; i++)
+            if (a->seg_in[i] != b->seg_in[i]) return -2;
+    } else if (a->in != b->in) {
+        return -2;
+    }
+    const long total_pix = (long)a->frames * a->out_h * a->out_w;
+    const int k64 = (a->kh * a->row_pad + BK - 1) / BK * BK, nks = k64 / BK;
+    int lg = 0;
+    while ((1 << lg) < a->in_c) lg++;
+    int bpx, wres;
+    both_form(2 * a->out_c, nks, ch != nullptr, &bpx, &wres);
+    if (a->out_c == 128) {
+        if (ch) return -2;
+        return a->nseg > 1 ? launch_persist_t<128, 256, 2, true, true, false, true>(a, total_pix, k64, lg, 65536u, b, wres)
+                           : launch_persist_t<128, 256, 2, true, false, false, true>(a, total_pix, k64, lg, 65536u, b, wres);
+    }
+    if (ch) {
+        if (a->nseg > 1)
+            return bpx == 256 ? launch_persist_t<256, 128, 2, true, true, false, true, true>(a, total_pix, k64, lg, 65536u, b, wres, ch)
+                              : launch_persist_t<128, 128, 2, true, true, false, true, true>(a, total_pix, k64, lg, 65536u, b, wres, ch);
+        return bpx == 256 ? launch_persist_t<256, 128, 2, true, false, false, true, true>(a, total_pix, k64, lg, 65536u, b, wres, ch)
+                          : launch_persist_t<128, 128, 2, true, false, false, true, true>(a, total_pix, k64, lg, 65536u, b, wres, ch);
+    }
+    if (a->nseg > 1)
+        return bpx == 256 ? launch_persist_t<256, 128, 2, true, true, false, true>(a, total_pix, k64, lg, 65536u, b, wres)
+                          : launch_persist_t<128, 128, 2, true, true, false, true>(a, total_pix, k64, lg, 65536u, b, wres);
+    return bpx == 256 ? launch_persist_t<256, 128, 2, true, false, false, true>(a, total_pix, k64, lg, 65536u, b, wres)
+                      : launch_persist_t<128, 128, 2, true, false, false, true>(a, total_pix, k64, lg, 65536u, b, wres);
+}
+
 extern "C" int mhip_conv_i8_seg_ok(const mhip_conv_i8_t *p) {
     return p && (p->in_c % 16) == 0 && !mhip_conv_i8_small_c(p->in_c, p->kw, p->out_c) && seg_valid(p) && persist_eligible(p);
 }
diff --git a/thingino-accel_amd/csrc/hip/conv_i8_common.hpp b/thingino-accel_amd/csrc/hip/conv_i8_common.hpp
--- a/thingino-accel_amd/csrc/hip/conv_i8_common.hpp
+++ b/thingino-accel_amd/csrc/hip/conv_i8_common.hpp
@@ -140,8 +140,8 @@
                  : "v"(q0), "v"(q1), "v"(q2), "v"(q3)
                  : "memory");
 }
-template <int NV>
-__device__ __forceinline__ void requant_pack_pre(const int (&a)[NV], float cs, uint32_t (&pk)[NV / 4]) {
+template <int NV, int TAB>
+__device__ __forceinline__ void requant_pack_at(const int (&a)[NV], float cs, uint32_t (&pk)[NV / 4]) {
     const float cs2 = cs * 2.0f;
     const int klo = -256, khi = 255;
     int q[NV], v[NV];
@@ -152,15 +152,17 @@
     }
 #pragma unroll
     for (int g = 0; g < NV / 4; g++)
-        asm volatile("ds_read_i8 %0, %4 offset:768\n\tds_read_i8 %1, %5 offset:768\n\t"
-                     "ds_read_i8 %2, %6 offset:768\n\tds_read_i8 %3, %7 offset:768"
+        asm volatile("ds_read_i8 %0, %4 offset:%8\n\tds_read_i8 %1, %5 offset:%8\n\t"
+                     "ds_read_i8 %2, %6 offset:%8\n\tds_read_i8 %3, %7 offset:%8"
                      : "=&v"(v[4 * g]), "=&v"(v[4 * g + 1]), "=&v"(v[4 * g + 2]), "=&v"(v[4 * g + 3])
-                     : "v"(q[4 * g]), "v"(q[4 * g + 1]), "v"(q[4 * g + 2]), "v"(q[4 * g + 3])
+                     : "v"(q[4 * g]), "v"(q[4 * g + 1]), "v"(q[4 * g + 2]), "v"(q[4 * g + 3]), "n"(TAB + 256)
                      : "memory");
     wait_lds_values<NV>(v);
 #pragma unroll
     for (int g = 0; g < NV / 4; g++) pk[g] = pack4(v[4 * g], v[4 * g + 1], v[4 * g + 2], v[4 * g + 3]);
 }
+template <int NV>
+__device__ __forceinline__ void requant_pack_pre(const int (&a)[NV], float cs, uint32_t (&pk)[NV / 4]) { requant_pack_at<NV, 512>(a, cs, pk); }
 __device__ __forceinline__ void requant_pack_two(const int (&a)[16], float cs0, float cs1, uint32_t (&pk)[4]) {
     const float c0 = cs0 * 2.0f, c1 = cs1 * 2.0f;
     const int klo = -256, khi = 255;
@@ -188,26 +190,7 @@
 #pragma unroll
     for (int g = 0; g < 4; g++) pk[g] = pack4(v[4 * g], v[4 * g + 1], v[4 * g + 2], v[4 * g + 3]);
 }
-__device__ __forceinline__ void requant_pack_chain(const int (&a)[8], float cs, uint32_t (&pk)[2]) {
-    const float cs2 = cs * 2.0f;
-    const int klo = -256, khi = 255;
-    int q[8], v[8];
-#pragma unroll
-    for (int i = 0; i < 8; i++) {
-        const int k = (int)((float)a[i] * cs2);
-        asm("v_med3_i32 %0, %1, %2, %3" : "=v"(q[i]) : "v"(k), "v"(klo), "v"(khi));
-    }
-#pragma unroll
-    for (int g = 0; g < 2; g++)
-        asm volatile("ds_read_i8 %0, %4 offset:1792\n\tds_read_i8 %1, %5 offset:1792\n\t"
-                     "ds_read_i8 %2, %6 offset:1792\n\tds_read_i8 %3, %7 offset:1792"
-                     : "=&v"(v[4 * g]), "=&v"(v[4 * g + 1]), "=&v"(v[4 * g + 2]), "=&v"(v[4 * g + 3])
-                     : "v"(q[4 * g]), "v"(q[4 * g + 1]), "v"(q[4 * g + 2]), "v"(q[4 * g + 3])
-                     : "memory");
-    wait_lds_values<8>(v);
-#pragma unroll
-    for (int g = 0; g < 2; g++) pk[g] = pack4(v[4 * g], v[4 * g + 1], v[4 * g + 2], v[4 * g + 3]);
-}
+__device__ __forceinline__ void requant_pack_chain(const int (&a)[8], float cs, uint32_t (&pk)[2]) { requant_pack_at<8, 1536>(a, cs, pk); }
 template <int NV, bool HAS_LUT, bool SAFE, bool LUT0, bool ADD = false, bool FAST = false>
 __device__ __forceinline__ void requant_pack(const int (&a)[NV], float cs, int lo, const uint8_t *lut128, uint32_t (&pk)[NV / 4],
                                              const uint32_t *xw = nullptr, const add_args_t *ga = nullptr) {
@@ -452,6 +435,8 @@
     int rows;
     int patch_ring;
     int patch_lds_kb;
+    int both_bpx;
+    int both_wide;
 };
 const tune_t &conv_i8_tune_state();
 
diff --git a/thingino-accel_amd/csrc/host/mars_internal.h b/thingino-accel_amd/csrc/host/mars_internal.h
--- a/thingino-accel_amd/csrc/host/mars_internal.h
+++ b/thingino-accel_amd/csrc/host/mars_internal.h
@@ -67,6 +67,9 @@
     int nseg, seg_t[4], seg_c[4], seg_up;
     int chain_n, chain_out[3];
     int pair_next;
+    int pair_both;
+    int both_chain;
+    int both_elide;
     int row_pad, oc_pad, c_pad;
     int ch_off, scale_h, scale_w, bn_n;
     int out_pix_stride, out_ch_off;
@@ -102,7 +105,7 @@
 typedef struct {
     int fusion;
     unsigned no_fuse_lut : 1, no_nhwc_internal : 1, no_vconcat_q : 1, no_pair_f32 : 1, no_rec : 1, no_zero_tail : 1, no_vconcat_f32 : 1,
-        no_rowpad : 1, no_post : 1, no_split : 1, no_chain : 1;
+        no_rowpad : 1, no_post : 1, no_split : 1, no_chain : 1, no_both : 1, no_both_chain : 1;
     size_t rec_limit;
     size_t vconcat_limit;
     size_t bottleneck_limit;
@@ -119,6 +122,8 @@
     int no_post;
     int no_split;
     int no_chain;
+    int no_both;
+    int no_both_chain;
     int rec_frames;
     int rec_skipped;
     size_t rec_max_frames;
@@ -229,6 +234,9 @@
 MARS_INTERNAL void conv_i8_geometry(const mars_op_t *op, int frames, mhip_conv_i8_t *p);
 MARS_INTERNAL int conv_i8_pre_fits(const mars_op_t *op, int frames, size_t in_stride, size_t out_stride);
 MARS_INTERNAL int conv_i8_post_fits(const mars_model_ext_t *m, const mars_op_t *a, const mars_op_t *b, int frames);
+MARS_INTERNAL int conv_i8_both_fits(const mars_model_ext_t *m, const mars_op_t *a, const mars_op_t *b, int frames);
+MARS_INTERNAL int conv_i8_both_chain_fits(const mars_model_ext_t *m, const mars_op_t *a, const mars_op_t *b, const mars_op_t *d, int side, int frames);
+MARS_INTERNAL void fuse_both_chain(mars_model_ext_t *m);
 MARS_INTERNAL int conv_i8_split_fits(const mars_model_ext_t *m, const mars_op_t *a, const mars_op_t *b, const mars_op_t *c, int frames);
 MARS_INTERNAL int conv_i8_chain_fits(const mars_model_ext_t *m, const mars_op_t *a, const mars_op_t *b, const mars_op_t *c, const mars_op_t *d, int side, int frames);
 MARS_INTERNAL void plan_layer(mars_model_ext_t *m, int li);
diff --git a/thingino-accel_amd/csrc/host/mars_model.c b/thingino-accel_amd/csrc/host/mars_model.c
--- a/thingino-accel_amd/csrc/host/mars_model.c
+++ b/thingino-accel_amd/csrc/host/mars_model.c
@@ -29,6 +29,8 @@
     sw->no_post = getenv("MARS_HIP_NO_POST") != NULL;
     sw->no_split = getenv("MARS_HIP_NO_SPLIT") != NULL;
     sw->no_chain = getenv("MARS_HIP_NO_CHAIN") != NULL;
+    sw->no_both = getenv("MARS_HIP_NO_BOTH") != NULL;
+    sw->no_both_chain = getenv("MARS_HIP_NO_BOTH_CHAIN") != NULL;
     sw->rec_limit = (e = getenv("MARS_HIP_REC_LIMIT")) ? (size_t)strtoull(e, NULL, 0) : (size_t)0xfffffff0u;
     sw->vconcat_limit = (e = getenv("MARS_HIP_VCONCAT_LIMIT")) ? (size_t)strtoull(e, NULL, 0) : (size_t)0x7fffffffu;
     sw->bottleneck_limit = (e = getenv("MARS_HIP_BOTTLENECK_LIMIT")) ? (size_t)strtoull(e, NULL, 0) : 0;
@@ -168,6 +170,7 @@
         fuse_split_chain(m);
         pad_output_rows(m);
         virtual_concat_q(m);
+        fuse_both_chain(m);
     } else {
         nhwc_internal(m);
     }
@@ -207,8 +210,8 @@
     const size_t vlim = m->sw.vconcat_limit, blim = m->sw.bottleneck_limit;
     const int rec_replan = (size_t)n > m->rec_max_frames || (m->rec_skipped && n < m->rec_frames);
     m->rec_frames = n;
-    if (m->no_vconcat || m->no_bottleneck || m->no_post || m->no_split || m->no_chain || rec_replan) {
-        m->no_vconcat = m->no_bottleneck = m->no_post = m->no_split = m->no_chain = 0;
+    if (m->no_vconcat || m->no_bottleneck || m->no_post || m->no_split || m->no_chain || m->no_both || m->no_both_chain || rec_replan) {
+        m->no_vconcat = m->no_bottleneck = m->no_post = m->no_split = m->no_chain = m->no_both = m->no_both_chain = 0;
         mars_error_t e = build_plan(m);
         if (e == MARS_OK) e = upload_params(m);
         if (e != MARS_OK) return e;
@@ -268,6 +271,30 @@
             if (op->kind != OP_CONV_I8 || !op->split_next) continue;
             if (!conv_i8_split_fits(m, op, op + 1, op + 2, n)) {
                 m->no_split = 1;
+                mars_error_t e = build_plan(m);
+                if (e == MARS_OK) e = upload_params(m);
+                if (e != MARS_OK) return e;
+                break;
+            }
+        }
+    if (!m->no_both_chain)
+        for (int i = 0; i + 2 < m->n_ops; i++) {
+            const mars_op_t *op = &m->ops[i];
+            if (op->kind != OP_CONV_I8 || !op->pair_both || !op->both_chain) continue;
+            if (!conv_i8_both_chain_fits(m, op, op + 1, op + 2, op->both_chain, n)) {
+                m->no_both_chain = 1;
+                mars_error_t e = build_plan(m);
+                if (e == MARS_OK) e = upload_params(m);
+                if (e != MARS_OK) return e;
+                break;
+            }
+        }
+    if (!m->no_both)
+        for (int i = 0; i + 1 < m->n_ops; i++) {
+            const mars_op_t *op = &m->ops[i];
+            if (op->kind != OP_CONV_I8 || !op->pair_both) continue;
+            if (!conv_i8_both_fits(m, op, op + 1, n)) {
+                m->no_both = 1;
                 mars_error_t e = build_plan(m);
                 if (e == MARS_OK) e = upload_params(m);
                 if (e != MARS_OK) return e;
@@ -430,6 +457,7 @@
     if (o->split_next) ADD(" %zd", (ssize_t)o->split_w_off);
     ADD(" split_chain %d", o->split_chain);
     if (o->split_chain) ADD(" %zd", (ssize_t)o->chain_w_off);
+    ADD(" pair_both %d both_chain %d both_elide %d", o->pair_both, o->both_chain, o->both_elide);
     ADD(" pre %d", o->pre);
     if (o->pre) ADD(" %zd %zd %zd %a", (ssize_t)o->pre_w_off, (ssize_t)o->pre_b_off, (ssize_t)o->pre_lut2_off, (double)o->pre_cs);
     ADD(" macs %a bytes %a prof_kind %d", o->macs, o->bytes, o->prof_kind);
@@ -454,7 +482,7 @@
 #define FLAG(cond, ...) if (cond) k += snprintf(line + k, sizeof line - (size_t)k, __VA_ARGS__)
         FLAG(o->kind == OP_CONV_I8 || o->kind == OP_CONV_F32 || o->kind == OP_CONV_F32_VHEAD, " k%dx%d s%d c%d->%d", o->kh, o->kw, o->sw, o->in_c, o->out_c);
         FLAG(o->nchw, " relayout"); FLAG(o->out_nchw, " planar_store"); FLAG(o->lut_off != NO_OFF, " lut"); FLAG(o->add_t, " add=%d", o->add_t - 1);
-        FLAG(o->nseg, " seg=%d", o->nseg); FLAG(o->pair_next, " pair_next"); FLAG(o->post_next, " post_next"); FLAG(o->split_next, " split_next"); FLAG(o->pre, " pre"); FLAG(o->silu_f32, " silu");
+        FLAG(o->nseg, " seg=%d", o->nseg); FLAG(o->pair_next && !(o->pair_both && o->nseg), " pair_next");  FLAG(o->pair_both, " pair_both"); FLAG(o->both_chain, " both_chain=%d", o->both_chain); FLAG(o->both_elide, " both_elide"); FLAG(o->post_next, " post_next"); FLAG(o->split_next, " split_next"); FLAG(o->pre, " pre"); FLAG(o->silu_f32, " silu");
         FLAG(o->k_limit, " k_limit=%d", o->k_limit); FLAG(o->in_rec, " in_rec=%d", o->in_rec); FLAG(o->out_rec, " out_rec");
         FLAG(o->vc_shift, " view=-%d", o->vc_shift); FLAG(o->vc_n, " vcat=%dx%d", o->vc_n, o->vc_run);
         FLAG(o->rows_only, " rows_only=%d", o->rows_only); FLAG(o->out_byte_off, " out_off=%zu", o->out_byte_off); FLAG(o->chain_n, " chain=%d", o->chain_n);
@@ -480,10 +508,10 @@
     if (full) {
         const plan_switches_t *w = &m->sw;
         snprintf(line, sizeof line, "+plan n_ops %d arena_size %zu scratch_per_frame %zu blob_mirror_bytes %zu rec_max_frames %zu rec_skipped %d f32_mode %d | fusion %d"
-                 " no_fuse_lut %d no_nhwc_internal %d no_vconcat_q %d no_pair_f32 %d no_rec %d no_zero_tail %d no_vconcat_f32 %d no_rowpad %d no_post %d no_split %d no_chain %d rec_limit %zu"
+                 " no_fuse_lut %d no_nhwc_internal %d no_vconcat_q %d no_pair_f32 %d no_rec %d no_zero_tail %d no_vconcat_f32 %d no_rowpad %d no_post %d no_split %d no_chain %d no_both %d no_both_chain %d rec_limit %zu"
                  " vconcat_limit %zu bottleneck_limit %zu\n", m->n_ops, m->arena_size, m->scratch_per_frame, m->blob_mirror_bytes, m->rec_max_frames, m->rec_skipped,
                  m->plan_f32_mode, w->fusion, w->no_fuse_lut, w->no_nhwc_internal, w->no_vconcat_q, w->no_pair_f32, w->no_rec, w->no_zero_tail, w->no_vconcat_f32,
-                 w->no_rowpad, w->no_post, w->no_split, w->no_chain, w->rec_limit, w->vconcat_limit, w->bottleneck_limit);
+                 w->no_rowpad, w->no_post, w->no_split, w->no_chain, w->no_both, w->no_both_chain, w->rec_limit, w->vconcat_limit, w->bottleneck_limit);
         EMIT();
     }
 #undef EMIT
diff --git a/thingino-accel_amd/csrc/host/mars_plan.c b/thingino-accel_amd/csrc/host/mars_plan.c
--- a/thingino-accel_amd/csrc/host/mars_plan.c
+++ b/thingino-accel_amd/csrc/host/mars_plan.c
@@ -630,6 +630,48 @@
     p.post_out_stride = planned_stride(&m->mt[b->t_out]);
     p.post_out_pix_stride = b->out_pix_stride; p.post_out_ch_off = b->out_ch_off;
     return mhip_conv_i8_post_ok(&p);
+}
+
+static int both_records(const mars_model_ext_t *m, const mars_op_t *a, const mars_op_t *b, int frames, mhip_conv_i8_t p[2]) {
+    const mars_op_t *o[2] = {a, b};
+    if (a->t_out < 0 || b->t_out < 0 || a->lut2_off == NO_OFF || b->lut2_off == NO_OFF || a->nchw || b->nchw)
+        return 0;
+    for (int k = 0; k < 2; k++) {
+        conv_i8_geometry(o[k], frames, &p[k]);
+        p[k].in = (const int8_t *)m;
+        p[k].in_stride = o[k]->t_in[0] >= 0 ? planned_stride(&m->mt[o[k]->t_in[0]]) : 0;
+        p[k].out = (int8_t *)m + k; p[k].out_stride = planned_stride(&m->mt[o[k]->t_out]);
+        p[k].lut = p[k].lut2 = (const uint8_t *)m;
+        if (o[k]->add_t) p[k].add = (const int8_t *)m;
+        p[k].nseg = o[k]->nseg; p[k].seg_up = o[k]->seg_up;
+        int c0 = 0;
+        for (int q = 0; q < 4; q++) {
+            p[k].seg_c0[q] = 0x7fffffff;
+            if (q < o[k]->nseg) {
+                p[k].seg_in[q] = (const int8_t *)m;
+                p[k].seg_stride[q] = o[k]->seg_t[q] >= 0 ? planned_stride(&m->mt[o[k]->seg_t[q]]) : 0;
+                p[k].seg_c[q] = o[k]->seg_c[q];
+                p[k].seg_c0[q] = c0;
+                c0 += o[k]->seg_c[q];
+            }
+        }
+    }
+    return 1;
+}
+int conv_i8_both_fits(const mars_model_ext_t *m, const mars_op_t *a, const mars_op_t *b, int frames) {
+    mhip_conv_i8_t p[2];
+    return both_records(m, a, b, frames, p) && mhip_conv_i8_both_ok(&p[0], &p[1]);
+}
+int conv_i8_both_chain_fits(const mars_model_ext_t *m, const mars_op_t *a, const mars_op_t *b, const mars_op_t *d, int side, int frames) {
+    mhip_conv_i8_t p[2], pd;
+    if (d->t_out < 0 || d->lut2_off == NO_OFF || d->nchw || !both_records(m, a, b, frames, p)) return 0;
+    conv_i8_geometry(d, frames, &pd);
+    pd.in = (const int8_t *)m; pd.out = (int8_t *)m + 2;
+    pd.in_stride = planned_stride(&m->mt[(side == 1 ? a : b)->t_out]); pd.out_stride = planned_stride(&m->mt[d->t_out]);
+    pd.lut = pd.lut2 = (const uint8_t *)m;
+    if (d->add_t) pd.add = (const int8_t *)m;
+    pd.nseg = d->nseg;
+    return mhip_conv_i8_both_chain_ok(&p[0], &p[1], &pd, side);
 }
 
 int conv_i8_split_fits(const mars_model_ext_t *m, const mars_op_t *a, const mars_op_t *b, const mars_op_t *c, int frames) {
@@ -1212,6 +1254,50 @@
     free(readers);
 }
 
+static int both_chain_mate_ok(const mars_op_t *d, const mars_op_t *a) {
+    return d->kind == OP_CONV_I8 && d->kh == 1 && d->kw == 1 && d->sh == 1 && d->sw == 1 && !d->pt && !d->pl && d->safe && !d->nchw && !d->out_nchw && !d->add_t &&
+           !d->chain_n && !d->store_c && !d->in_byte_off && !d->out_byte_off && !d->out_pix_stride && !d->out_ch_off && d->lut_off != NO_OFF &&
+           d->lut2_off != NO_OFF && !d->nseg && !d->pre && !d->pair_next && !d->post_next && !d->split_next && d->n_in == 1 && d->in_c == 64 && d->out_c == 64 &&
+           d->oc_pad == 64 && d->row_pad == 64 && d->in_h == a->out_h && d->in_w == a->out_w && d->out_h == a->out_h && d->out_w == a->out_w;
+}
+void fuse_both_chain(mars_model_ext_t *m) {
+    if (m->sw.no_both_chain || m->no_both_chain || m->sw.no_both || m->no_both) return;
+    int *readers, *writers;
+    if (!use_counts(m, &readers, &writers)) return;
+    for (int i = 0; i + 2 < m->n_ops; i++) {
+        mars_op_t *a = &m->ops[i];
+        if (a->kind != OP_CONV_I8 || !a->pair_both || a->both_chain || a->in_byte_off || a[1].in_byte_off || a->out_byte_off || a[1].out_byte_off) continue;
+        if (i > 0 && m->ops[i - 1].split_next) continue;
+        const int O0 = a->t_out, O1 = a[1].t_out;
+        for (int j = i + 2; j < m->n_ops && j <= i + 48; j++) {
+            const mars_op_t *d = &m->ops[j];
+            if (!both_chain_mate_ok(d, a) || m->ops[j - 1].pair_next || m->ops[j - 1].post_next || m->ops[j - 1].split_next ||
+                (j >= 2 && (m->ops[j - 2].split_next || m->ops[j - 2].both_chain)) || (j >= 3 && m->ops[j - 3].split_chain))
+                continue;
+            const int side = d->t_in[0] == O0 ? 1 : (d->t_in[0] == O1 ? 2 : 0), O = d->t_out;
+            if (!side || O < 0 || O == O0 || O == O1 || writers[O] != 1 || m->mt[O].io_in || m->mt[O].is_weight || m->mt[O].pix_stride ||
+                op_reads(a, O) || op_reads(a + 1, O) || op_reads(d, O))
+                continue;
+            if (touched_between(m, i + 2, j, O, USE_READ | USE_WRITE) || touched_between(m, i + 2, j, d->t_in[0], USE_WRITE)) continue;
+            if (!conv_i8_both_chain_fits(m, a, a + 1, d, side, 1)) continue;
+            if (j > i + 2) {
+                const mars_op_t moved = *d;
+                memmove(&m->ops[i + 3], &m->ops[i + 2], sizeof(mars_op_t) * (size_t)(j - i - 2));
+                m->ops[i + 2] = moved;
+            }
+            a->both_chain = side;
+            const int S = side == 1 ? O0 : O1;
+            if (readers[S] == 1 && writers[S] == 1 && !m->mt[S].io_in && !m->mt[S].io_out && !m->mt[S].is_weight && !m->mt[S].tail_read) {
+                a->both_elide = 1;
+                m->mt[S].needed = 0;
+            }
+            break;
+        }
+        i += 1;
+    }
+    free(readers);
+}
+
 void pad_output_rows(mars_model_ext_t *m) {
     for (uint32_t i = 0; i < m->pub.header.num_tensors; i++) m->mt[i].pix_c = m->mt[i].pix_stride = 0;
     if (m->sw.no_rowpad) return;
@@ -1337,7 +1423,7 @@
            a->row_pad == b->row_pad && a->oc_pad == b->oc_pad;
 }
 static int pairable(const mars_op_t *o) {
-    return o->kind == OP_CONV_I8 && !o->nchw && !o->out_nchw && !o->add_t && !o->nseg && o->safe && o->lut_off != NO_OFF && !o->pair_next &&
+    return o->kind == OP_CONV_I8 && !o->nchw && !o->out_nchw && !o->add_t && o->safe && o->lut_off != NO_OFF && !o->pair_next &&
            (o->in_c & 15) == 0 && o->in_c > 4 && (o->out_c & 15) == 0 && !o->out_pix_stride;
 }
 static int pair_up(mars_model_ext_t *m, int i, int j) {
@@ -1359,7 +1445,12 @@
             mars_op_t *b = &m->ops[j];
             if (!pairable(b) || !same_conv_input(a, b) || b->t_out == a->t_out) continue;
             if (op_reads(b, b->t_out) || op_reads(b, a->t_out)) continue;
-            if (pair_up(m, i, j)) break;
+            const int both = !m->sw.no_both && !m->no_both && conv_i8_both_fits(m, a, b, 1);
+            if (a->nseg && !both) continue;
+            if (pair_up(m, i, j)) {
+                m->ops[i].pair_both = both;
+                break;
+            }
         }
     }
 }
@@ -1680,6 +1771,8 @@
         else if (o->add_t && !op_reads(o, o->add_t - 1)) why = "add_t is not among t_in";
         else if (o->chain_n && o->t_out != o->chain_out[o->chain_n - 1]) why = "t_out is not the chain's last stage";
         else if (o->pair_next && (i + 1 >= m->n_ops || m->ops[i + 1].kind != o->kind)) why = "pair_next without a mate of its kind";
+        else if (o->pair_both && (!o->pair_next || o->kind != OP_CONV_I8 || (o->out_c != 64 && o->out_c != 128) || m->ops[i + 1].out_c != o->out_c)) why = "pair_both without a pair of 64- or 128-channel sides";
+        else if (o->kind == OP_CONV_I8 && o->pair_next && o->nseg && !o->pair_both) why = "a side-by-side pair over a virtual concat";
         else if (o->post_next && (o->kind != OP_CONV_I8 || i + 1 >= m->n_ops || m->ops[i + 1].kind != OP_CONV_I8 || m->ops[i + 1].nseg != 2 ||
                                   m->ops[i + 1].seg_t[0] != o->t_out || !op_reads(o, m->ops[i + 1].seg_t[1])))
             why = "post_next without its 1x1 behind it, or y2 is not among t_in";
@@ -1692,6 +1785,12 @@
                                     m->ops[i + 3].t_out == m->ops[i + 1].t_out || m->ops[i + 3].t_out == m->ops[i + 2].t_out || m->ops[i + 3].t_out == o->t_out ||
                                     m->mt[m->ops[i + 3].t_out].pix_stride || o->chain_w_off == NO_OFF))
             why = "split_chain without its 1x1 behind the pair";
+        else if (o->both_chain && (!o->pair_both || i + 2 >= m->n_ops || !both_chain_mate_ok(&m->ops[i + 2], o) || (o->both_chain != 1 && o->both_chain != 2) ||
+                                   m->ops[i + 2].t_in[0] != m->ops[i + o->both_chain - 1].t_out || m->ops[i + 2].t_out < 0 ||
+                                   m->ops[i + 2].t_out == o->t_out || m->ops[i + 2].t_out == m->ops[i + 1].t_out))
+            why = "both_chain without its 1x1 behind the pair";
+        else if (o->both_elide && (!o->both_chain || m->mt[m->ops[i + o->both_chain - 1].t_out].needed || m->mt[m->ops[i + o->both_chain - 1].t_out].io_out))
+            why = "both_elide on a side that is kept";
         for (int k = 0; !why && k < o->nseg; k++)
             if (!op_reads(o, o->seg_t[k])) why = "a seg_t is not among t_in";
         for (int k = 0; !why && k < o->vc_n; k++)
diff --git a/thingino-accel_amd/csrc/host/mars_run.c b/thingino-accel_amd/csrc/host/mars_run.c
--- a/thingino-accel_amd/csrc/host/mars_run.c
+++ b/thingino-accel_amd/csrc/host/mars_run.c
@@ -337,7 +337,7 @@
             return (mars_error_t)op->err;
         }
         mars_op_t *mate = (op->pair_next || op->post_next || op->split_next) && i + 1 < m->n_ops ? &m->ops[i + 1] : NULL;
-        mars_op_t *mate2 = op->split_next && i + 2 < m->n_ops ? &m->ops[i + 2] : NULL;
+        mars_op_t *mate2 = (op->split_next || (op->pair_both && op->both_chain)) && i + 2 < m->n_ops ? &m->ops[i + 2] : NULL;
         mars_op_t *mate3 = op->split_next && op->split_chain && i + 3 < m->n_ops ? &m->ops[i + 3] : NULL;
         if (wait_tail && ((op->t_out >= 0 && (m->mt[op->t_out].io_out || m->mt[op->t_out].tail_read)) ||
                           (mate && mate->t_out >= 0 && (m->mt[mate->t_out].io_out || m->mt[mate->t_out].tail_read)) ||
@@ -384,7 +384,18 @@
             mhip_conv_i8_t pa, pb;
             conv_i8_params(m, op, &pa);
             conv_i8_params(m, mate, &pb);
-            rc = mhip_conv_i8_pair(&pa, &pb);
+            if (op->pair_both && op->both_chain) {
+                mhip_conv_i8_t pd;
+                rc = -1;
+                if (mate2) {
+                    conv_i8_params(m, mate2, &pd);
+                    rc = mhip_conv_i8_both_chain(&pa, &pb, &pd, op->both_chain, op->both_elide);
+                    if (rc == -2) rc = -1;
+                }
+                i++;
+            } else {
+                rc = op->pair_both ? mhip_conv_i8_both(&pa, &pb) : mhip_conv_i8_pair(&pa, &pb);
+            }
             if (rc == -2) {
                 rc = launch_op(m, op);
                 if (!rc) rc = launch_op(m, mate);
@@ -738,6 +749,7 @@
         if (op->post_next || (i > 0 && m->ops[i - 1].post_next)) continue;
         if (op->split_next) continue;
         if (i >= 3 && m->ops[i - 3].split_chain) continue;
+        if (i >= 2 && m->ops[i - 2].both_chain) continue;
         mhip_conv_i8_t p;
         conv_i8_params(m, op, &p);
         int codes[32];
diff --git a/thingino-accel_amd/csrc/mhip.h b/thingino-accel_amd/csrc/mhip.h
--- a/thingino-accel_amd/csrc/mhip.h
+++ b/thingino-accel_amd/csrc/mhip.h
@@ -112,6 +112,10 @@
 int mhip_conv_i8_variants(const mhip_conv_i8_t *p, int *codes, int max);
 int mhip_conv_i8_seg_ok(const mhip_conv_i8_t *p);
 int mhip_conv_i8_pair(const mhip_conv_i8_t *a, const mhip_conv_i8_t *b);
+int mhip_conv_i8_both_ok(const mhip_conv_i8_t *a, const mhip_conv_i8_t *b);
+int mhip_conv_i8_both(const mhip_conv_i8_t *a, const mhip_conv_i8_t *b);
+int mhip_conv_i8_both_chain_ok(const mhip_conv_i8_t *a, const mhip_conv_i8_t *b, const mhip_conv_i8_t *d, int side);
+int mhip_conv_i8_both_chain(const mhip_conv_i8_t *a, const mhip_conv_i8_t *b, const mhip_conv_i8_t *d, int side, int elide);
 int mhip_conv_i8_small_c(int in_c, int kw, int out_c);
 void mhip_conv_i8_pack_geom(int in_c, int kw, int out_c, int *row_pad, int *oc_pad, int *c_eff);
 int mhip_conv_i8(const mhip_conv_i8_t *p);
```

After: 61180 (median of 6 runs). 1.2% higher.
